# GeekAlexis/FastMOT

Measured on AMD Instinct MI355X. Metric: end-to-end tracker FPS @1080p/50 dets, higher is better.
Workload: dtype f16

## Files before the change

### fastmot_amd/_lib.py

```python
import ctypes as C
import os
import sys
import weakref
from pathlib import Path

import numpy as np
from types import SimpleNamespace

from .utils.nv12 import NV12Frame
from .utils.jpeg import JPEGFrame, QT_ENTRIES, max_coefficients
from .utils.source import SourceFrame
from .utils.yuv import PlanarFrame, frame_bytes
from .utils.packed import PackedFrame, row_bytes
from .utils.bayer import BayerFrame
from .utils.deep import DeepFrame, deep_frame_bytes
from .utils.devarray import DeviceArrayFrame

LIB_PATH = Path(os.environ.get('FASTMOT_LIB_PATH', Path(__file__).parent / 'libfastmot_hip.so'))

c_int_p = C.POINTER(C.c_int)
_lib = None


class FastMOTHipError(RuntimeError):
# ... 117 lines not shown
    plans = np.ascontiguousarray(plans, dtype=CROP_PLAN_DTYPE)
    lens = np.array([len(s) for s in segments], np.uint32)
    segs = np.zeros(max(sum((len(s) + 15) & ~15 for s in segments), 16), np.uint8)
    at = 0
    for s in segments:
        segs[at:at + len(s)] = np.frombuffer(s, np.uint8)
        at += (len(s) + 15) & ~15
    cap = int(plans['bound'].sum()) if capacity is None else capacity
    out = np.zeros(max(cap, 1), np.uint8)
    offsets = np.zeros(len(plans) + 1, np.uintp)
    check(load().fm_jpeg_encode_regions_assemble(_ptr(plans), C.c_int(len(plans)), C.c_int(int(quality)), _ptr(lens), _ptr(segs),
                                                 C.c_size_t(segs.size if segs_bytes is None else segs_bytes), _ptr(out), C.c_size_t(cap),
                                                 _ptr(offsets)))
    return [out[int(a):int(b)].tobytes() for a, b in zip(offsets[:-1], offsets[1:])]


def _redact_args(regions):
    regions = np.ascontiguousarray(regions, dtype=REDACT_REGION_DTYPE).reshape(-1)
    return regions, (_ptr(regions) if len(regions) else None, C.c_int(len(regions)))


def redact_check(regions, width, height):
    regions, args = _redact_args(regions)
    return load().fm_redact_check(*args, C.c_int(width), C.c_int(height))


def redact_render_host(frame, regions):
    if not isinstance(frame, np.ndarray) or frame.dtype != np.uint8 or frame.ndim != 3 or frame.shape[2] != 3 or \
            frame.strides[1:] != (3, 1) or frame.strides[0] < 3 * frame.shape[1] or not frame.flags.writeable:
        raise ValueError('frame must be a writeable uint8 HxWx3 array with packed pixels')
    regions, args = _redact_args(regions)
    check(load().fm_redact_render_host(_ptr(frame), C.c_int(frame.shape[1]), C.c_int(frame.shape[0]), C.c_size_t(frame.strides[0]), *args))
    return frame


def device_count():
    n = load().fm_device_count()
    if n < 0:
        raise FastMOTHipError(load().fm_last_error().decode())
    return n


def device_pci_bus_id(device):
    buf = C.create_string_buffer(64)
    check(load().fm_device_pci_bus_id(C.c_int(device), buf, C.c_int(64)))
    return buf.value.decode().lower()


class HipContext:

    def __init__(self, device=0):
        self._dev_pending = []
        self.lib = load()
        self._ctx = C.c_void_p()
        check(self.lib.fm_ctx_create(C.c_int(device), C.byref(self._ctx)))
        self.device = device
        self.feat_dim = 512

    def close(self):
        if getattr(self, '_ctx', None) is not None and self._ctx:
            self.lib.fm_ctx_destroy(self._ctx)
            self._ctx = C.c_void_p()
        for frame, _ in self._dev_pending:
            frame._pending = [(ref, t) for ref, t in frame._pending if ref() is not self]
        self._dev_pending = []

    def __del__(self):
        if sys.is_finalizing():
            return
        try:
            self.close()
        except Exception:
            pass

    @property
    def handle(self):
        return self._ctx

    def synchronize(self):
        check(self.lib.fm_ctx_synchronize(self._ctx))

    def set_option(self, key, value):
        check(self.lib.fm_ctx_set_option(self._ctx, key.encode(), C.c_int(int(value))))

    def trace_start(self, cap=20000):
        t0 = C.c_int64(0)
        check(self.lib.fm_trace_start(self._ctx, C.c_int(cap), C.byref(t0)))
        self._trace_cap = cap
        return t0.value

    def trace_read(self):
        cap = self._trace_cap
        tags = np.zeros(cap, np.int32)
        ms = np.zeros(cap, np.float32)
        n = C.c_int(0)
        check(self.lib.fm_trace_read(self._ctx, C.c_int(cap), _ptr(tags), _ptr(ms), C.byref(n)))
        return tags[:n.value], ms[:n.value]

    def bind_thread(self):
        check(self.lib.fm_ctx_bind_thread(self._ctx))

    def device_info(self):
        buf = C.create_string_buffer(256)
        check(self.lib.fm_device_info(self._ctx, buf, 256))
        parts = buf.value.decode().split(':')
        return {'name': parts[0], 'arch': ':'.join(parts[1:-3]), 'cus': int(parts[-3]),
                'clock_mhz': int(parts[-2]), 'hbm_bytes': int(parts[-1])}

    def kf_configure(self, dt, std_factor_acc, std_offset_acc, std_factor_det, std_factor_klt,
                     min_std_det, min_std_klt, init_pos_weight, init_vel_weight, vel_coupling,
                     vel_half_life):
        p = KFParams(dt, std_factor_acc, std_offset_acc, (C.c_double * 2)(*std_factor_det),
                     (C.c_double * 2)(*std_factor_klt), (C.c_double * 2)(*min_std_det),
                     (C.c_double * 2)(*min_std_klt), init_pos_weight, init_vel_weight, vel_coupling,
                     vel_half_life)
        check(self.lib.fm_kf_configure(self._ctx, C.byref(p)))

    def set_frame_rect(self, tlbr):
        a = _as(tlbr, np.float64, (4,))
        check(self.lib.fm_set_frame_rect(self._ctx, _ptr(a)))

    def trk_create(self, slots, det_tlbr):
        s = _as(slots, np.int32)
        b = _as(det_tlbr, np.float64, (-1, 4))
        assert len(s) == len(b)
        check(self.lib.fm_trk_create(self._ctx, C.c_int(len(s)), _ptr(s), _ptr(b)))

    def trk_step(self, slots, H, klt_tlbr, has_klt, mult):
        s = _as(slots, np.int32)
        n = len(s)
        Hm = _as(H, np.float64, (9,))
        k = _as(klt_tlbr, np.float64, (-1, 4)) if n else np.zeros((0, 4))
        hk = _as(has_klt, np.uint8)
        mu = _as(mult, np.float64)
        assert len(k) == n and len(hk) == n and len(mu) == n
        tlbr = np.empty((n, 4), np.float64)
        lost = np.empty(n, np.uint8)
        check(self.lib.fm_trk_step(self._ctx, C.c_int(n), _ptr(s), _ptr(Hm), _ptr(k), _ptr(hk),
                                   _ptr(mu), _ptr(tlbr), _ptr(lost)))
        return tlbr, lost.astype(bool)

    def trk_step_ops(self, ops, slots, H, klt_tlbr, has_klt, mult):
        s = _as(slots, np.int32)
        n = len(s)
        Hm = _as(H, np.float64, (9,))
        k = _as(klt_tlbr, np.float64, (-1, 4)) if n else np.zeros((0, 4))
        hk = _as(has_klt, np.uint8)
        mu = _as(mult, np.float64)
        tlbr = np.empty((n, 4), np.float64)
        lost = np.empty(n, np.uint8)
        check(self.lib.fm_trk_step_ops(self._ctx, C.c_int(ops), C.c_int(n), _ptr(s), _ptr(Hm), _ptr(k),
                                       _ptr(hk), _ptr(mu), _ptr(tlbr), _ptr(lost)))
        return tlbr, lost.astype(bool)

    def trk_update_det(self, slots, det_tlbr):
        s = _as(slots, np.int32)
        n = len(s)
        b = _as(det_tlbr, np.float64, (-1, 4)) if n else np.zeros((0, 4))
        assert len(b) == n
        tlbr = np.empty((n, 4), np.float64)
        lost = np.empty(n, np.uint8)
        check(self.lib.fm_trk_update_det(self._ctx, C.c_int(n), _ptr(s), _ptr(b), _ptr(tlbr), _ptr(lost)))
        return tlbr, lost.astype(bool)

    def trk_get_state(self, slots):
        s = _as(slots, np.int32)
# ... 930 lines not shown
```

### fastmot_amd/csrc/common.h

```cpp
#pragma once
#include <hip/hip_runtime.h>
#include <atomic>
#include <cstdarg>
#include <cstdint>
#include <cstdio>
#include <cstring>
#include <string>
#include <vector>
#include "../../include/fastmot_hip.h"
#ifdef FM_DIAG
#include "../../include/fastmot_hip_diag.h"
#endif

#define FM_ERR_HIP (-1)
#define FM_ERR_ARG (-2)
#define FM_ERR_STATE (-3)

void fm_set_error(const char* fmt, ...);

#define FM_HIP(call)                                                                        \
    do {                                                                                    \
        hipError_t e_ = (call);                                                             \
        if (e_ != hipSuccess) {                                                             \
            fm_set_error("%s:%d %s -> %s", __FILE__, __LINE__, #call, hipGetErrorString(e_)); \
            return FM_ERR_HIP;                                                              \
        }                                                                                   \
    } while (0)

#define FM_CHECK_ARG(cond)                                                     \
    do {                                                                       \
        if (!(cond)) {                                                         \
            fm_set_error("%s:%d bad argument: %s", __FILE__, __LINE__, #cond); \
            return FM_ERR_ARG;                                                 \
        }                                                                      \
    } while (0)

bool fm_lap_host(const double* cost, int nr, int nc, long rs, long cs, int32_t* col4row_out);
#define FM_ZERO_COPY_TRACKS (ctx->opt_zero_copy_tracks)

struct DevBuf {
    void* d = nullptr;
    void* h = nullptr;
    size_t cap = 0;
    bool pinned_mirror = true;
    int reserve(size_t bytes) {
        if (bytes <= cap) return 0;
        size_t ncap = cap ? cap : 4096;
        while (ncap < bytes) ncap *= 2;
        if (d) (void)hipFree(d);
        if (h) (void)hipHostFree(h);
        d = h = nullptr;
        cap = 0;
        FM_HIP(hipMalloc(&d, ncap));
        if (pinned_mirror) FM_HIP(hipHostMalloc(&h, ncap, hipHostMallocDefault));
        cap = ncap;
        return 0;
    }
    void release() {
        if (d) (void)hipFree(d);
        if (h) (void)hipHostFree(h);
        d = h = nullptr;
        cap = 0;
    }
    template <typename T> T* dev() { return reinterpret_cast<T*>(d); }
    template <typename T> T* host() { return reinterpret_cast<T*>(h); }
};

struct KFConst {
    double F_pos_self;
    double F_pos_other;
    double F_vel;
    double q_pp, q_pv, q_vv;
    double std_factor_acc, std_offset_acc;
    double fac_det[2], fac_klt[2], min_det[2], min_klt[2];
    double init_pos_weight, init_vel_weight;
};

struct NetState;
struct DetState;
struct ExtState;
struct FlowState;
struct EncState;
struct OvlState;
struct YuvState;
struct SsdState;
struct GalleryState;
constexpr int FM_GALLERY_CHANNELS = 2;

struct fm_ctx {
    int device = 0;
    int opt_zero_copy_tracks = 2048;
    int opt_host_lap_elems = 262144;
    int opt_use_graphs = 1;
    int opt_fused_input = 1;
    int opt_net_timing = 0;
    int opt_nms_general = 0;
    int opt_lk_variant = 0;
    void* predict_worker = nullptr;
    hipStream_t s_main = nullptr;
    hipStream_t s_det = nullptr;
    hipStream_t s_up = nullptr;
    hipStream_t s_ext = nullptr;
    hipStream_t s_ext_x[FM_MAX_EXTRA_EXTRACTORS] = {};
    hipEvent_t ev_ext_in = nullptr, ev_ext_x_done[FM_MAX_EXTRA_EXTRACTORS] = {};
    hipStream_t s_flow = nullptr;
    hipStream_t s_flow2 = nullptr;
    hipEvent_t ev_pyr = nullptr;
    bool pyr_pending = false;
    hipEvent_t ev_prep = nullptr, ev_bg = nullptr;
    hipEvent_t ev_feat = nullptr;
    hipEvent_t ev_ext_net = nullptr;
    hipEvent_t ev_ext_done = nullptr;
    hipEvent_t ev_pair = nullptr;
    bool ext_net_recorded = false;
    size_t as_in_bytes = 0;
    bool as_in_device = true;
    bool as_mirror = false;

    int slot_cap = 0;
    double* mean = nullptr;
    double* cov = nullptr;
    int feat_dim = 512;
    float* feat_sum = nullptr;
    float* feat_avg = nullptr;
    int32_t* feat_cnt = nullptr;
    KFConst kf{};
    bool kf_set = false;
    double frame_rect[4] = {0, 0, 0, 0};

    float* emb = nullptr;
    float* emb_host = nullptr;
    int emb_cap = 0;
    int emb_n = 0;

    int as_nT = 0, as_nD = 0, as_metric = 0;
    size_t as_off[6] = {0, 0, 0, 0, 0, 0};
    DevBuf as_in;
    DevBuf as_pair;
    DevBuf as_stage_in;
    DevBuf as_cost;
    DevBuf as_work;
    DevBuf as_out;
    DevBuf io0, io1;
    DevBuf occ_in, occ_out;
    DevBuf feat_in;

    int frame_w = 0, frame_h = 0, ring_size = 0;
    uint8_t* frame_cur = nullptr;
    uint8_t* frame_own = nullptr;
    uint8_t* frame_own2 = nullptr;
    uint8_t* frame_next = nullptr;
    uint8_t* frame_pinned2 = nullptr;
    hipEvent_t ev_next_upload = nullptr;
    uint8_t* frame_ahead[FM_MAX_DET_BATCH + 1] = {};
    uint8_t* frame_up[FM_MAX_DET_BATCH + 1] = {};
    uint8_t* frame_up_pinned[FM_MAX_DET_BATCH + 1] = {};
    hipEvent_t ev_up[FM_MAX_DET_BATCH + 1] = {};
    uint8_t* frame_ring = nullptr;
    uint8_t* frame_pinned = nullptr;

    DetState* det = nullptr;
    SsdState* ssd = nullptr;
    ExtState* ext = nullptr;
    NetState* det_net = nullptr;
    NetState* ext_net = nullptr;
    NetState* ext_net_x[FM_MAX_EXTRA_EXTRACTORS] = {};
    FlowState* flow = nullptr;
    EncState* enc = nullptr;
    OvlState* ovl = nullptr;
    YuvState* yuv = nullptr;
    GalleryState* gallery[2] = {nullptr, nullptr};

    std::vector<hipEvent_t> trace_ev;
    std::vector<int> trace_tag;
    std::atomic<int> trace_n{0};
    std::atomic<bool> trace_on{false};
    std::atomic<int> trace_busy{0};
    hipEvent_t trace_base = nullptr;

// ... 15 lines not shown
    };
    SrcStage frame_src[FM_MAX_DET_BATCH + 2];
    SrcStage frame_deep[FM_MAX_DET_BATCH + 2];

    hipEvent_t ev_dev_in[FM_MAX_DET_BATCH + 2] = {};
    struct DevTicket {
        uint64_t ticket = 0;
        hipEvent_t ev = nullptr;
    };
    DevTicket dev_ticket[FM_DEV_TICKETS];
    uint64_t dev_ticket_next = 1;

    int32_t* remap_xy = nullptr;
    int remap_sw = 0, remap_sh = 0;
    uint32_t remap_border = 0;
};

inline void fm_trace_mark(fm_ctx* ctx, hipStream_t s, int tag) {
    if (!ctx->trace_on.load(std::memory_order_acquire)) return;
    ctx->trace_busy.fetch_add(1);
    if (ctx->trace_on.load()) {
        const int i = ctx->trace_n.fetch_add(1);
        if (i < (int)ctx->trace_ev.size()) {
            ctx->trace_tag[i] = tag;
            (void)hipEventRecord(ctx->trace_ev[i], s);
        }
    }
    ctx->trace_busy.fetch_sub(1);
}

int fm_ensure_slots(fm_ctx* ctx, int max_slot_plus_1);
int fm_nv12_to_bgr(const uint8_t* nv12, uint8_t* bgr, int w, int h, int matrix, hipStream_t s);
inline bool fm_yuv_chroma_dims(int w, int h, int chroma, int* cw, int* ch) {
    switch (chroma) {
    case FM_YUV_420: *cw = (w + 1) / 2, *ch = (h + 1) / 2; return true;
    case FM_YUV_422: *cw = (w + 1) / 2, *ch = h; return true;
    case FM_YUV_444: *cw = w, *ch = h; return true;
    case FM_YUV_MONO: *cw = *ch = 0; return true;
    }
    return false;
}
int fm_planar_to_bgr(const uint8_t* planes, uint8_t* bgr, int w, int h, int chroma, int matrix, hipStream_t s);
inline size_t fm_packed_row_bytes(int w, int format) {
    if (format < FM_PACKED_RGB || format > FM_PACKED_YVYU) return 0;
    if (format >= FM_PACKED_YUY2) return 4 * (size_t)((w + 1) / 2);
    return (size_t)w * (format <= FM_PACKED_BGR ? 3 : 4);
}
inline bool fm_packed_matrix_ok(int matrix) {
    return matrix == FM_PACKED_BT601 || matrix == FM_PACKED_BT709 || matrix == FM_PACKED_BT601_FULL || matrix == FM_PACKED_BT709_FULL;
}
int fm_packed_to_bgr(const uint8_t* src, uint8_t* bgr, int w, int h, int format, int matrix, hipStream_t s);
inline int fm_bayer_sample_bytes(int depth) {
    return depth == 8 ? 1 : depth == 10 || depth == 12 || depth == 14 || depth == 16 ? 2 : 0;
}
inline bool fm_bayer_gain_ok(int gain) { return gain >= 1 && gain <= 4096; }
int fm_bayer_to_bgr(const uint8_t* src, uint8_t* bgr, int w, int h, int pattern, int depth, int method, int black, int gain_r, int gain_g,
                    int gain_b, hipStream_t s);
inline bool fm_deep_layout_ok(int w, int h, int chroma, int matrix, int depth, int layout) {
    int cw = 0, ch = 0;
    if (depth < 9 || depth > 16 || matrix < FM_DEEP_BT601 || matrix > FM_DEEP_BT2020 || !fm_yuv_chroma_dims(w, h, chroma, &cw, &ch)) return false;
    if (layout == FM_DEEP_SEMIPLANAR) return chroma == FM_YUV_420 && w % 2 == 0 && h % 2 == 0;
    return layout == FM_DEEP_PLANAR;
}
int fm_deep_to_bgr(const uint8_t* planes, uint8_t* bgr, int w, int h, int chroma, int matrix, int depth, int layout,
                   hipStream_t s);
int fm_device_to_bgr(const struct fm_frame_device* f, uint8_t* bgr, hipStream_t s);
inline int fm_dev_elem_bytes(int dtype) { return dtype == FM_DEV_U8 ? 1 : dtype == FM_DEV_F16 ? 2 : dtype == FM_DEV_F32 ? 4 : 0; }
inline int fm_dev_planes(int layout) { return layout == FM_DEV_HWC ? 1 : layout == FM_DEV_CHW ? 3 : layout == FM_DEV_NV12 ? 2 : 0; }
inline int fm_dev_plane_rows(const struct fm_frame_device* f, int p) { return f->layout == FM_DEV_NV12 && p == 1 ? f->height / 2 : f->height; }
inline size_t fm_dev_row_bytes(const struct fm_frame_device* f) {
    if (f->layout == FM_DEV_HWC) return (size_t)f->width * (f->format <= FM_PACKED_BGR ? 3 : 4);
    return (size_t)f->width * fm_dev_elem_bytes(f->dtype);
}
void fm_ssd_free(fm_ctx* ctx);
void fm_yuv_free(fm_ctx* ctx);
int fm_resize_bgr(const uint8_t* src, int sw, int sh, uint8_t* dst, int dw, int dh, hipStream_t s);
int fm_remap_bgr(const uint8_t* src, int sw, int sh, const int32_t* xy, uint8_t* dst, int dw, int dh, uint32_t border, hipStream_t s);
inline uint8_t*& fm_ahead_frame(fm_ctx* ctx, int k) { return k == 1 ? ctx->frame_next : ctx->frame_ahead[k]; }
inline uint8_t*& fm_ahead_buf(fm_ctx* ctx, int k) { return k == 1 ? ctx->frame_own2 : ctx->frame_up[k]; }
inline hipEvent_t& fm_ahead_event(fm_ctx* ctx, int k) { return k == 1 ? ctx->ev_next_upload : ctx->ev_up[k]; }
bool fm_host_is_pinned(const void* p, size_t bytes);
void fm_frame_staging_free(fm_ctx* ctx);
void fm_frame_dev_free(fm_ctx* ctx);
int fm_det_flush_post(fm_ctx* ctx);
int fm_jpeg_to_bgr(const uint8_t* stage, uint8_t* bgr, const struct fm_jpeg_info* info, hipStream_t s);
int fm_jpeg_layout(int width, int height, int ncomp, int hsamp0, int vsamp0, struct fm_jpeg_info* out);
size_t fm_jpeg_sample_offset(long long coef_count);
void fm_ext_invalidate_export(fm_ctx* ctx);
void fm_predict_worker_free(fm_ctx* ctx);
void fm_gallery_free(fm_ctx* ctx);
void fm_jpegenc_free(fm_ctx* ctx);
int fm_jpegenc_ensure(fm_ctx* ctx, int mcus_x, int mcus_y);
hipStream_t fm_jpegenc_stream(fm_ctx* ctx);
int fm_jpegenc_encode_device(fm_ctx* ctx, const uint8_t* src, int width, int height, int quality, uint8_t* out, size_t capacity,
                             size_t* length);
void fm_overlay_free(fm_ctx* ctx);
```

### fastmot_amd/csrc/ctx.hip

```cpp
#include "common.h"
void convd_set_cfg(int code);
#include <sched.h>
#include <cstring>
#include <cstdlib>
#include <cmath>

static thread_local char g_err[1024] = "";

void fm_set_error(const char* fmt, ...) {
    va_list ap;
    va_start(ap, fmt);
    vsnprintf(g_err, sizeof(g_err), fmt, ap);
    va_end(ap);
}

extern "C" const char* fm_last_error(void) { return g_err; }

extern "C" int fm_ctx_set_option(fm_ctx* ctx, const char* key, int value) {
    FM_CHECK_ARG(ctx && key && value >= 0);
    if (!strcmp(key, "zero_copy_tracks")) ctx->opt_zero_copy_tracks = value;
    else if (!strcmp(key, "host_lap_elems")) ctx->opt_host_lap_elems = value;
    else if (!strcmp(key, "use_graphs")) ctx->opt_use_graphs = value;
    else if (!strcmp(key, "convd_cfg")) convd_set_cfg(value);
    else if (!strcmp(key, "nms_path")) {
        ctx->opt_nms_general = value != 0;
    }
    else if (!strcmp(key, "fused_input")) ctx->opt_fused_input = value != 0;
    else if (!strcmp(key, "net_timing")) ctx->opt_net_timing = value;
    else if (!strcmp(key, "lk_variant")) {
#ifndef FM_DIAG
        if (value != 0) {
            fm_set_error("option 'lk_variant' needs a diagnostic build of the library (-DFM_DIAG)");
            return FM_ERR_ARG;
        }
#endif
        ctx->opt_lk_variant = value;
    }
    else {
        fm_set_error("unknown option '%s'", key);
        return FM_ERR_ARG;
    }
    return 0;
}

extern "C" int fm_trace_start(fm_ctx* ctx, int cap, int64_t* host_ns) {
    FM_CHECK_ARG(ctx && cap > 0 && host_ns && !ctx->trace_on.load() && ctx->trace_ev.empty());
    FM_HIP(hipDeviceSynchronize());
    std::vector<hipEvent_t> evs(cap);
    for (auto& e : evs) FM_HIP(hipEventCreate(&e));
    if (!ctx->trace_base) FM_HIP(hipEventCreate(&ctx->trace_base));
    FM_HIP(hipEventRecord(ctx->trace_base, ctx->s_main));
    FM_HIP(hipEventSynchronize(ctx->trace_base));
    timespec ts;
    clock_gettime(CLOCK_MONOTONIC, &ts);
    *host_ns = (int64_t)ts.tv_sec * 1000000000ll + ts.tv_nsec;
    ctx->trace_tag.assign(cap, 0);
    ctx->trace_n = 0;
    ctx->trace_ev = std::move(evs);
    ctx->trace_on.store(true, std::memory_order_release);
    return 0;
}

extern "C" int fm_trace_read(fm_ctx* ctx, int cap, int32_t* tags, float* ms, int* n) {
    FM_CHECK_ARG(ctx && tags && ms && n);
    ctx->trace_on.store(false, std::memory_order_seq_cst);
    while (ctx->trace_busy.load(std::memory_order_seq_cst) > 0) sched_yield();
    FM_HIP(hipDeviceSynchronize());
    std::vector<hipEvent_t> evs = std::move(ctx->trace_ev);
    ctx->trace_ev.clear();
    int k = ctx->trace_n.load();
    if (k > (int)evs.size()) k = (int)evs.size();
    if (k > cap) k = cap;
    for (int i = 0; i < k; ++i) {
        tags[i] = ctx->trace_tag[i];
        FM_HIP(hipEventElapsedTime(&ms[i], ctx->trace_base, evs[i]));
    }
    *n = k;
    for (auto& e : evs) (void)hipEventDestroy(e);
    return 0;
}

extern "C" int fm_ctx_bind_thread(fm_ctx* ctx) {
    FM_CHECK_ARG(ctx);
    FM_HIP(hipSetDevice(ctx->device));
    return 0;
}

extern "C" int fm_device_pci_bus_id(int device, char* buf, int buflen) {
    FM_CHECK_ARG(buf && buflen >= 16);
    FM_HIP(hipDeviceGetPCIBusId(buf, buflen, device));
    return 0;
}

extern "C" int fm_device_count(void) {
    int n = 0;
    FM_HIP(hipGetDeviceCount(&n));
    return n;
}

void fm_net_free(NetState* n);
void fm_det_free(DetState* d);
void fm_ext_free(ExtState* e);
void fm_flow_free(FlowState* f);

extern "C" int fm_ctx_create(int device, fm_ctx** out) {
    FM_CHECK_ARG(out != nullptr);
    int n = 0;
    FM_HIP(hipGetDeviceCount(&n));
    if (device < 0 || device >= n) {
        fm_set_error("device %d out of range (%d visible)", device, n);
        return FM_ERR_ARG;
    }
    FM_HIP(hipSetDevice(device));
    fm_ctx* ctx = new fm_ctx();
    ctx->device = device;
    if (const char* e = getenv("FASTMOT_ZERO_COPY")) ctx->opt_zero_copy_tracks = atoi(e);
    if (const char* e = getenv("FASTMOT_HOST_LAP")) ctx->opt_host_lap_elems = atoi(e);
    if (const char* e = getenv("FASTMOT_GRAPHS")) ctx->opt_use_graphs = atoi(e);
    if (const char* e = getenv("FASTMOT_FUSED_INPUT")) ctx->opt_fused_input = atoi(e) != 0;
    int prio_lo = 0, prio_hi = 0;
    FM_HIP(hipDeviceGetStreamPriorityRange(&prio_lo, &prio_hi));
    const int prio_det = prio_lo, prio_ext = prio_hi;
    FM_HIP(hipStreamCreateWithPriority(&ctx->s_main, hipStreamNonBlocking, prio_hi));
    FM_HIP(hipStreamCreateWithPriority(&ctx->s_det, hipStreamNonBlocking, prio_det));
    FM_HIP(hipStreamCreateWithPriority(&ctx->s_up, hipStreamNonBlocking, prio_lo));
    FM_HIP(hipStreamCreateWithPriority(&ctx->s_ext, hipStreamNonBlocking, prio_ext));
    FM_HIP(hipEventCreateWithFlags(&ctx->ev_ext_in, hipEventDisableTiming));
    for (int i = 0; i < FM_MAX_EXTRA_EXTRACTORS; ++i) {
        FM_HIP(hipStreamCreateWithPriority(&ctx->s_ext_x[i], hipStreamNonBlocking, prio_hi));
        FM_HIP(hipEventCreateWithFlags(&ctx->ev_ext_x_done[i], hipEventDisableTiming));
    }
    FM_HIP(hipStreamCreateWithPriority(&ctx->s_flow, hipStreamNonBlocking, prio_hi));
    FM_HIP(hipStreamCreateWithPriority(&ctx->s_flow2, hipStreamNonBlocking, prio_hi));
    FM_HIP(hipEventCreateWithFlags(&ctx->ev_pyr, hipEventDisableTiming));
    FM_HIP(hipEventCreateWithFlags(&ctx->ev_prep, hipEventDisableTiming));
    FM_HIP(hipEventCreateWithFlags(&ctx->ev_bg, hipEventDisableTiming));
    FM_HIP(hipEventCreateWithFlags(&ctx->ev_feat, hipEventDisableTiming));
    FM_HIP(hipEventCreateWithFlags(&ctx->ev_ext_net, hipEventDisableTiming));
    FM_HIP(hipEventCreateWithFlags(&ctx->ev_pair, hipEventDisableTiming));
    FM_HIP(hipEventCreateWithFlags(&ctx->ev_ext_done, hipEventDisableTiming));
    int rc = fm_ensure_slots(ctx, 1024);
    if (rc) return rc;
    *out = ctx;
    return 0;
}

extern "C" int fm_ctx_destroy(fm_ctx* ctx) {
    if (!ctx) return 0;
    (void)hipSetDevice(ctx->device);
    fm_predict_worker_free(ctx);
    fm_gallery_free(ctx);
    (void)hipDeviceSynchronize();
    if (ctx->det) fm_det_free(ctx->det);
    fm_ssd_free(ctx);
    if (ctx->ext) fm_ext_free(ctx->ext);
    for (void* p : {(void*)ctx->frame_own, (void*)ctx->frame_own2, (void*)ctx->frame_ring})
        if (p) (void)hipFree(p);
    if (ctx->frame_pinned) (void)hipHostFree(ctx->frame_pinned);
    if (ctx->frame_pinned2) (void)hipHostFree(ctx->frame_pinned2);
    for (int k = 2; k <= FM_MAX_DET_BATCH; ++k) {
        if (ctx->frame_up[k]) (void)hipFree(ctx->frame_up[k]);
        if (ctx->frame_up_pinned[k]) (void)hipHostFree(ctx->frame_up_pinned[k]);
        if (ctx->ev_up[k]) (void)hipEventDestroy(ctx->ev_up[k]);
    }
    for (hipEvent_t e : ctx->ev_jpeg)
        if (e) (void)hipEventDestroy(e);
    fm_frame_dev_free(ctx);
    fm_frame_staging_free(ctx);
    fm_overlay_free(ctx);
    fm_yuv_free(ctx);
    fm_jpegenc_free(ctx);
    if (ctx->det_net) fm_net_free(ctx->det_net);
    if (ctx->ext_net) fm_net_free(ctx->ext_net);
    for (NetState* x : ctx->ext_net_x)
        if (x) fm_net_free(x);
    if (ctx->flow) fm_flow_free(ctx->flow);
    for (void* p : {(void*)ctx->mean, (void*)ctx->cov, (void*)ctx->feat_sum, (void*)ctx->feat_avg,
                    (void*)ctx->feat_cnt, (void*)ctx->emb})
        if (p) (void)hipFree(p);
    if (ctx->emb_host) (void)hipHostFree(ctx->emb_host);
    for (DevBuf* b : {&ctx->as_in, &ctx->as_pair, &ctx->as_stage_in, &ctx->as_cost, &ctx->as_work,
                      &ctx->as_out, &ctx->io0, &ctx->io1, &ctx->feat_in, &ctx->occ_in, &ctx->occ_out})
        b->release();
    for (hipStream_t s : {ctx->s_main, ctx->s_det, ctx->s_up, ctx->s_ext, ctx->s_flow, ctx->s_flow2})
        if (s) (void)hipStreamDestroy(s);
    for (hipEvent_t e : {ctx->ev_feat, ctx->ev_ext_in, ctx->ev_pyr, ctx->ev_prep, ctx->ev_bg, ctx->ev_ext_net, ctx->ev_pair, ctx->ev_ext_done})
        if (e) (void)hipEventDestroy(e);
    for (int i = 0; i < FM_MAX_EXTRA_EXTRACTORS; ++i) {
        if (ctx->s_ext_x[i]) (void)hipStreamDestroy(ctx->s_ext_x[i]);
        if (ctx->ev_ext_x_done[i]) (void)hipEventDestroy(ctx->ev_ext_x_done[i]);
    }
    delete ctx;
    return 0;
}

extern "C" int fm_ctx_synchronize(fm_ctx* ctx) {
    FM_CHECK_ARG(ctx);
    FM_HIP(hipStreamSynchronize(ctx->s_main));
    FM_HIP(hipStreamSynchronize(ctx->s_det));
    FM_HIP(hipStreamSynchronize(ctx->s_up));
    FM_HIP(hipStreamSynchronize(ctx->s_ext));
    for (hipStream_t x : ctx->s_ext_x) FM_HIP(hipStreamSynchronize(x));
// ... 343 lines not shown
```

### fastmot_amd/csrc/detect.hip

```cpp
#include "pixel_source.h"
#include <cmath>
#include <string>
#include <vector>

struct DetState {
    fm_yolo_cfg cfg{};
    bool configured = false;
    int cap = 8192;
    static constexpr int NSLOT_UNTILED = FM_MAX_DET_BATCH + 2;
    static constexpr int NSLOT = 3 * FM_MAX_DET_BATCH;
    int nslot = NSLOT_UNTILED;
    int n_tiles = 0;
    int tile_x[FM_MAX_DET_BATCH] = {}, tile_y[FM_MAX_DET_BATCH] = {};
    int region_w = 0, region_h = 0;
    double tile_offset[FM_MAX_DET_BATCH][2] = {};
    double merge_thresh = 0.6;
    std::vector<fm_det48> tile_stage;
    std::vector<fm_det48> tile_dets;
    std::vector<int32_t> tile_ids;
    int tile_count[FM_MAX_DET_BATCH] = {};
    int tile_sum[2] = {};
    float* cand[NSLOT] = {};
    float* sorted[NSLOT] = {};
    int32_t* counters[NSLOT] = {};
    uint64_t* mask[NSLOT] = {};
    fm_det48* dets[NSLOT] = {};
    bool used[NSLOT] = {};
    hipEvent_t ev_dec[NSLOT] = {};
    int post_pending = -1;
    int post_pending_n = 0;
    bool general_post = false;
    static constexpr int GREEDY_RETRY = 1024;
    int general_passes = 0;
    int greedy_kmax = 2048, greedy_shrink = 0;
    bool sorted_valid[NSLOT] = {};
    static constexpr int PREFIX = 2048;
    fm_det48* dets_host[NSLOT] = {};
    int32_t* counters_host[NSLOT] = {};
    hipEvent_t ev_done[NSLOT] = {};
    hipStream_t s_fallback = nullptr;
    hipEvent_t ev0[NSLOT] = {}, ev1[NSLOT] = {};
    bool timed[NSLOT] = {};
    long n_passes = 0;
    int wr = 0, rd = 0, pending = 0, last = -1;
    uint8_t* label_mask = nullptr;
    float* rows_in = nullptr;
    int rows_cap = 0;
};

void fm_det_free(DetState* d) {
    if (!d) return;
    for (int i = 0; i < DetState::NSLOT; ++i) {
        for (void* q : {(void*)d->cand[i], (void*)d->sorted[i], (void*)d->counters[i], (void*)d->mask[i], (void*)d->dets[i]})
            if (q) (void)hipFree(q);
    }
    for (void* p : {(void*)d->label_mask, (void*)d->rows_in})
        if (p) (void)hipFree(p);
    if (d->s_fallback) (void)hipStreamDestroy(d->s_fallback);
    for (int i = 0; i < DetState::NSLOT; ++i) {
        if (d->dets_host[i]) (void)hipHostFree(d->dets_host[i]);
        if (d->counters_host[i]) (void)hipHostFree(d->counters_host[i]);
        for (hipEvent_t e : {d->ev_done[i], d->ev_dec[i], d->ev0[i], d->ev1[i]})
            if (e) (void)hipEventDestroy(e);
    }
    delete d;
}

namespace {

__global__ void preprocess_kernel(const StemSrc src, f16* __restrict__ inp, int in_w, int in_h, int cs) {
    const int x = blockIdx.x * blockDim.x + threadIdx.x;
    const int y = blockIdx.y, n = blockIdx.z;
    int32_t* counters = pick_sample(src.zero4, n);
    if (counters && x < 4 && y == 0) counters[x] = 0;
    if (x >= in_w || y >= in_h) return;
    float rgb[3];
    det_input_pixel(pick_sample(src.frame, n), src.fw, src.fh, x, y, pick_sample(src.roi_x, n), pick_sample(src.roi_y, n),
                    src.roi_w, src.roi_h, rgb);
    f16x8 o;
    o[0] = (f16)rgb[0]; o[1] = (f16)rgb[1]; o[2] = (f16)rgb[2];
#pragma unroll
    for (int e = 3; e < 8; ++e) o[e] = (f16)0.f;
    *reinterpret_cast<f16x8*>(inp + (((size_t)n * in_h + y) * in_w + x) * cs) = o;
}

struct HeadArgs {
    const float* data;
    int cs, gw, gh, na, base_index;
    float anchors[2 * FM_MAX_ANCHORS];
    float scale_xy;
};

__device__ __forceinline__ float sigmoid_fast(float x) { return 1.0f / (1.0f + __expf(-x)); }

struct FilterArgs {
    const uint8_t* label_mask;
    int num_classes;
    float conf_thresh;
    double size[2], offset[2];
    float* cand;
    int32_t* counters;
    int cap;
};

__device__ __forceinline__ void emit_candidate(const FilterArgs& fa, float bx, float by, float bw, float bh,
                                               float box_conf, int cls, float cls_prob, int orig) {
    if (cls < 0 || cls >= 128 || !fa.label_mask[cls]) return;
    const float score = box_conf * cls_prob;
    if (!(score >= fa.conf_thresh)) return;
    const int slot = atomicAdd(fa.counters, 1);
    if (slot >= fa.cap) {
        fa.counters[1] = 1;
        return;
    }
    float* r = fa.cand + (size_t)slot * 8;
    float x = (float)((double)bx * fa.size[0]);
    float y = (float)((double)by * fa.size[1]);
    r[2] = (float)((double)bw * fa.size[0]);
    r[3] = (float)((double)bh * fa.size[1]);
    r[0] = (float)((double)x - fa.offset[0]);
    r[1] = (float)((double)y - fa.offset[1]);
    r[4] = box_conf;
    r[5] = (float)cls;
    r[6] = cls_prob;
    r[7] = __int_as_float(orig);
}

struct HeadSet {
    HeadArgs h[FM_MAX_HEADS];
    int first_block[FM_MAX_HEADS + 1];
    float* cand[FM_MAX_DET_BATCH];
    int32_t* counters[FM_MAX_DET_BATCH];
    double off_x[FM_MAX_DET_BATCH], off_y[FM_MAX_DET_BATCH];
};

__global__ void decode_kernel(HeadSet hs, FilterArgs fa, int in_w, int in_h, int new_coords) {
    int hi = 0;
#pragma unroll
    for (int i = 1; i < FM_MAX_HEADS; ++i) hi += (int)blockIdx.x >= hs.first_block[i] ? 1 : 0;
    const HeadArgs& h = hs.h[hi];
    const int idx = ((int)blockIdx.x - hs.first_block[hi]) * blockDim.x + threadIdx.x;
    const int cells = h.gw * h.gh;
    if (idx >= cells * h.na) return;
    const int img = blockIdx.y;
    fa.cand = pick_sample(hs.cand, img);
    fa.counters = pick_sample(hs.counters, img);
    fa.offset[0] = pick_sample(hs.off_x, img);
// ... 481 lines not shown
                        else if (!(est < (float)thresh - 1e-4f)) need |= 1u << u;
                    }
                }
            }
        }
        while (need) {
            const int u = __builtin_ctz(need);
            need &= need - 1;
            const float4 c = sbox[tid + NG_T * u];
            if (diou_suppresses_call(a[0], a[1], a[2], a[3], c.x, c.y, c.z, c.w, thresh)) alive &= ~(1u << u);
        }
#pragma unroll
        for (int u = 0; u < NG_CPT; ++u) {
            const uint64_t bal = __ballot((alive >> u) & 1u);
            if (lane == 0) alive_w[wave + NG_NW * u] = bal;
        }
        __syncthreads();
        if (wave == 0) {
            uint64_t w = alive_w[lane];
            const int ws = s >> 6;
            if (lane < ws) w = 0;
            else if (lane == ws) w &= (s & 63) == 63 ? 0ull : (~0ull << ((s & 63) + 1));
            const uint64_t nz = __ballot(w != 0);
            int next = -1;
            if (nz) {
                const int fl = __builtin_ctzll(nz);
                const uint64_t ww = (uint64_t)(uint32_t)__builtin_amdgcn_readlane((int)(uint32_t)w, fl) |
                                    ((uint64_t)(uint32_t)__builtin_amdgcn_readlane((int)(uint32_t)(w >> 32), fl) << 32);
                next = fl * 64 + __builtin_ctzll(ww);
            }
            if (lane == 0) misc[0] = next;
        }
        __syncthreads();
    }
    if (tid == 0) misc[1] = 0;
    __syncthreads();
#pragma unroll
    for (int u = 0; u < NG_CPT; ++u) {
        if ((int)NG_T * u >= K) break;
        const int j = tid + NG_T * u;
        bool ok = false;
        double t0 = 0, t1 = 0, t2 = 0, t3 = 0;
        if ((kept >> u) & 1u) {
            const float4 b = box[u];
            const double xmin = b.x, ymin = b.y;
            t0 = rint(xmin); t1 = rint(ymin);
            t2 = rint(xmin + (double)b.z - 1.); t3 = rint(ymin + (double)b.w - 1.);
            const double bw = t2 - t0 + 1, bh = t3 - t1 + 1;
            const double area = (bw <= 0 || bh <= 0) ? 0. : bw * bh;
            const double ar = bw > 0 ? bh / bw : 0.;
            ok = area > 0 && area <= max_area && ar >= min_ar;
        }
        const uint64_t bal = __ballot(ok);
        if (lane == 0) misc[2 + wave] = __builtin_popcountll(bal);
        __syncthreads();
        const int base = misc[1];
        int off = base + __builtin_popcountll(bal & ((1ull << lane) - 1ull));
        for (int wv = 0; wv < wave; ++wv) off += misc[2 + wv];
        if (ok) {
            const float* r = sorted + (size_t)j * 8;
            fm_det48 d;
            d.tlbr[0] = t0; d.tlbr[1] = t1; d.tlbr[2] = t2; d.tlbr[3] = t3;
            d.label = (int64_t)r[5];
            d.conf = (double)(r[4] * r[6]);
            dets[off] = d;
            if (off < prefix) dets_host[off] = d;
        }
        __syncthreads();
        if (tid == 0) {
            int n = base;
            for (int wv = 0; wv < NG_NW; ++wv) n += misc[2 + wv];
            misc[1] = n;
        }
        __syncthreads();
    }
    if (tid == 0) {
        const int n = misc[1];
        counters[2] = n;
        counters[3] = 0;
        counters_host[0] = counters[0]; counters_host[1] = counters[1]; counters_host[2] = n; counters_host[3] = 0;
    }
}

int ensure_det(fm_ctx* ctx) {
    if (ctx->det) return 0;
    ctx->det = new DetState();
    return 0;
}

int alloc_post(DetState* d, int cap, int nslot) {
    cap = (cap + 63) & ~63;
    if (d->cand[0] && cap == d->cap && nslot == d->nslot) return 0;
    for (int i = (cap != d->cap || !d->cand[0]) ? 0 : nslot; i < DetState::NSLOT; ++i) {
        for (void* p : {(void*)d->cand[i], (void*)d->sorted[i], (void*)d->mask[i], (void*)d->dets[i]})
            if (p) (void)hipFree(p);
        if (d->dets_host[i]) (void)hipHostFree(d->dets_host[i]);
        d->dets_host[i] = nullptr;
        d->cand[i] = d->sorted[i] = nullptr; d->mask[i] = nullptr; d->dets[i] = nullptr;
    }
    for (int i = 0; i < DetState::NSLOT; ++i) d->used[i] = false;
    d->cap = cap;
    d->nslot = nslot;
    d->wr = d->rd = d->pending = 0;
    d->last = -1;
    d->post_pending = -1;
    d->post_pending_n = 0;
    for (int i = 0; i < nslot; ++i) {
        if (d->cand[i]) continue;
        FM_HIP(hipMalloc(&d->cand[i], sizeof(float) * 8 * cap));
        FM_HIP(hipMalloc(&d->sorted[i], sizeof(float) * 8 * cap));
        FM_HIP(hipMalloc(&d->mask[i], sizeof(uint64_t) * (size_t)cap * (cap / 64)));
        FM_HIP(hipMalloc(&d->dets[i], sizeof(fm_det48) * cap));
        FM_HIP(hipHostMalloc(&d->dets_host[i], sizeof(fm_det48) * cap, hipHostMallocDefault));
    }
    for (int i = 0; i < nslot; ++i) {
        if (d->counters[i]) continue;
        FM_HIP(hipMalloc(&d->counters[i], sizeof(int32_t) * 4));
        FM_HIP(hipHostMalloc(&d->counters_host[i], sizeof(int32_t) * 4, hipHostMallocDefault));
        FM_HIP(hipEventCreateWithFlags(&d->ev_done[i], hipEventDisableTiming));
        FM_HIP(hipEventCreateWithFlags(&d->ev_dec[i], hipEventDisableTiming));
        FM_HIP(hipEventCreate(&d->ev0[i]));
        FM_HIP(hipEventCreate(&d->ev1[i]));
    }
    if (!d->label_mask) FM_HIP(hipMalloc(&d->label_mask, 128));
    return 0;
}

FilterArgs filter_args(DetState* d, int slot) {
    FilterArgs fa{};
    fa.label_mask = d->label_mask;
    fa.num_classes = d->cfg.num_classes;
    fa.conf_thresh = (float)d->cfg.conf_thresh;
    const bool tiled = d->n_tiles > 1;
    fa.size[0] = d->cfg.size[0]; fa.size[1] = d->cfg.size[1];
    fa.offset[0] = tiled ? d->tile_offset[0][0] : d->cfg.offset[0]; fa.offset[1] = tiled ? d->tile_offset[0][1] : d->cfg.offset[1];
    fa.cand = d->cand[slot];
    fa.counters = d->counters[slot];
    fa.cap = d->cap;
    return fa;
}

static int launch_rank_sort(DetState* d, int slot, hipStream_t sp);
static int enqueue_general_post(fm_ctx* ctx, DetState* d, int slot, hipStream_t sp, bool sorted_already = false) {
    const int cap = d->cap;
    if (!sorted_already) {
        int rc = launch_rank_sort(d, slot, sp);
        if (rc) return rc;
    }
    fm_trace_mark(ctx, sp, 22);
    hipLaunchKernelGGL(nms_mask_kernel, dim3(std::min(NMS_MASK_GRID, (cap / 64) * (cap / 64 + 1) / 2)), dim3(256), 0, sp, d->sorted[slot],
                       d->counters[slot], cap, d->cfg.nms_thresh, d->mask[slot]);
    fm_trace_mark(ctx, sp, 23);
    hipLaunchKernelGGL(nms_scan_kernel, dim3(1), dim3(1024), sizeof(uint64_t) * (cap / 64), sp, d->sorted[slot],
                       d->counters[slot], cap, d->mask[slot], d->cfg.max_area, d->cfg.min_aspect_ratio, d->dets[slot],
                       d->dets_host[slot], cap < DetState::PREFIX ? cap : DetState::PREFIX, d->counters_host[slot]);
    FM_HIP(hipGetLastError());
    return 0;
}

static int launch_rank_sort(DetState* d, int slot, hipStream_t sp) {
    const int cap = d->cap;
    static bool configured = false;
    if (!configured) {
        FM_HIP(hipFuncSetAttribute(reinterpret_cast<const void*>(rank_sort_lds_kernel),
                                   hipFuncAttributeMaxDynamicSharedMemorySize, (int)(sizeof(uint64_t) * (16384 + 8))));
        configured = true;
    }
    if (cap <= 16384)
        hipLaunchKernelGGL(rank_sort_lds_kernel, dim3(cap / 64 + 1), dim3(256), sizeof(uint64_t) * (cap + 8), sp,
                           d->cand[slot], d->sorted[slot], d->counters[slot], cap);
    else
        hipLaunchKernelGGL(rank_sort_kernel, dim3(cap / 256 + 1), dim3(256), 0, sp, d->cand[slot], d->sorted[slot],
                           d->counters[slot], cap);
    FM_HIP(hipGetLastError());
    d->sorted_valid[slot] = true;
    return 0;
}

static int enqueue_greedy_post(fm_ctx* ctx, DetState* d, int slot, hipStream_t sp) {
    static bool configured = false;
    if (!configured) {
        FM_HIP(hipFuncSetAttribute(reinterpret_cast<const void*>(nms_greedy_kernel),
                                   hipFuncAttributeMaxDynamicSharedMemorySize, (int)ng_lds_bytes(NG_KMAX)));
        configured = true;
    }
    int rc = launch_rank_sort(d, slot, sp);
    if (rc) return rc;
    fm_trace_mark(ctx, sp, 22);
    const int kmax = d->greedy_kmax < d->cap ? d->greedy_kmax : (d->cap < NG_KMAX ? d->cap : NG_KMAX);
    hipLaunchKernelGGL(nms_greedy_kernel, dim3(1), dim3(NG_T), ng_lds_bytes(kmax), sp, d->sorted[slot], d->counters[slot],
                       d->cap, kmax, d->cfg.nms_thresh, d->cfg.max_area, d->cfg.min_aspect_ratio, d->dets[slot],
                       d->dets_host[slot], d->cap < DetState::PREFIX ? d->cap : DetState::PREFIX, d->counters_host[slot]);
    FM_HIP(hipGetLastError());
    return 0;
}

static int flush_post(fm_ctx* ctx, DetState* d) {
    const int first = d->post_pending, n = d->post_pending_n;
    if (first < 0) return 0;
    d->post_pending = -1;
    d->post_pending_n = 0;
    hipStream_t sp = ctx->s_up;
    FM_HIP(hipStreamWaitEvent(sp, d->ev_dec[first], 0));
    for (int i = 0; i < n; ++i) {
        const int slot = (first + i) % d->nslot;
        fm_trace_mark(ctx, sp, 20);
        int rc_p = (d->general_post || ctx->opt_nms_general) ? enqueue_general_post(ctx, d, slot, sp) : enqueue_greedy_post(ctx, d, slot, sp);
        if (rc_p) return rc_p;
        FM_HIP(hipEventRecord(d->ev_done[slot], sp));
        fm_trace_mark(ctx, sp, 21);
    }
    return 0;
}

int enqueue_post(fm_ctx* ctx, DetState* d, hipStream_t s, int n = 1) {
    int rc = flush_post(ctx, d);
    if (rc) return rc;
    while (d->pending + n > d->nslot) {
        const int drop = d->n_tiles > 1 ? d->n_tiles : 1;
        d->rd = (d->rd + drop) % d->nslot;
        d->pending -= drop;
    }
    const int slot = d->wr;
    FM_HIP(hipEventRecord(d->ev_dec[slot], s));
    d->post_pending = slot;
    d->post_pending_n = n;
    for (int i = 0; i < n; ++i) d->used[(slot + i) % d->nslot] = true;
    d->wr = (slot + n) % d->nslot;
    d->pending += n;
    return 0;
}

static int acquire_slots(fm_ctx* ctx, DetState* d, hipStream_t s, int n = 1) {
    if (d->post_pending >= 0 && d->post_pending_n + n > d->nslot) {
        int rc = flush_post(ctx, d);
        if (rc) return rc;
    }
    for (int i = 0; i < n; ++i) {
        const int slot = (d->wr + i) % d->nslot;
        if (d->used[slot] && hipEventQuery(d->ev_done[slot]) != hipSuccess) {
            (void)hipGetLastError();
            FM_HIP(hipStreamWaitEvent(s, d->ev_done[slot], 0));
        }
    }
    return 0;
}

int collect(fm_ctx* ctx, DetState* d, hipStream_t s, fm_det48* out, int cap_out, int* n) {
    if (d->pending == 0) {
        fm_set_error("no detector pass in flight (fm_detect_async first)");
        return FM_ERR_STATE;
    }
    const int slot = d->rd;
    int rc_f = flush_post(ctx, d);
    if (rc_f) return rc_f;
    FM_HIP(hipEventSynchronize(d->ev_done[slot]));
    if (d->counters_host[slot][3] != 0 && !d->counters_host[slot][1]) {
        const int why = d->counters_host[slot][3];
        if (!d->s_fallback) FM_HIP(hipStreamCreateWithFlags(&d->s_fallback, hipStreamNonBlocking));
        hipStream_t sp = d->s_fallback;
        int rc_g = enqueue_general_post(ctx, d, slot, sp, d->sorted_valid[slot]);
        if (rc_g) return rc_g;
        FM_HIP(hipStreamSynchronize(sp));
        if (why == 2 || d->counters_host[slot][0] > NG_KMAX) {
            d->general_post = true;
            d->general_passes = 0;
        }
    } else if (d->general_post && d->counters_host[slot][0] <= NG_KMAX * 3 / 4 && ++d->general_passes >= DetState::GREEDY_RETRY) {
        d->general_post = false;
    }
    {
        const int k = d->counters_host[slot][0];
        int want = ((k + k / 4 + 511) / 512) * 512;
        if (want < 512) want = 512;
        if (want > NG_KMAX) want = NG_KMAX;
        if (want > d->greedy_kmax) d->greedy_kmax = want;
        else if (want < d->greedy_kmax && ++d->greedy_shrink >= 64) { d->greedy_kmax = want; d->greedy_shrink = 0; }
        else if (want == d->greedy_kmax) d->greedy_shrink = 0;
    }
    d->rd = (slot + 1) % d->nslot;
    --d->pending;
    d->last = slot;
    if (d->counters_host[slot][1]) {
        fm_set_error("candidate list overflow (%d > %d): raise max_candidates", d->counters_host[slot][0], d->cap);
        return FM_ERR_STATE;
    }
    const int nd = d->counters_host[slot][2];
    if (nd > DetState::PREFIX) {
        FM_HIP(hipMemcpy(d->dets_host[slot], d->dets[slot], sizeof(fm_det48) * nd, hipMemcpyDeviceToHost));
    }
    if (nd > cap_out) {
        fm_set_error("output capacity %d < %d detections", cap_out, nd);
        return FM_ERR_ARG;
    }
    memcpy(out, d->dets_host[slot], sizeof(fm_det48) * nd);
    *n = nd;
    return 0;
}

int collect_tiles(fm_ctx* ctx, DetState* d, hipStream_t s, fm_det48* out, int cap_out, int* n) {
    const int nt = d->n_tiles;
    if (d->pending < nt) {
        fm_set_error("no detector pass in flight (fm_detect_async first)");
        return FM_ERR_STATE;
    }
    const int first = d->rd, pending = d->pending;
    d->tile_stage.resize((size_t)d->cap);
    d->tile_dets.clear();
    d->tile_ids.clear();
    d->tile_sum[0] = d->tile_sum[1] = 0;
    int rc_first = 0;
    std::string err;
    for (int t = 0; t < nt; ++t) {
        const int slot = (first + t) % d->nslot;
        int k = 0;
        d->rd = slot;
        const int rc = collect(ctx, d, s, d->tile_stage.data(), d->cap, &k);
        d->tile_count[t] = rc ? 0 : k;
        if (rc) {
            if (!rc_first) { rc_first = rc; err = fm_last_error(); }
            if (rc == FM_ERR_HIP) break;
            continue;
        }
        d->tile_sum[0] += d->counters_host[slot][0];
        d->tile_sum[1] += k;
        d->tile_dets.insert(d->tile_dets.end(), d->tile_stage.begin(), d->tile_stage.begin() + k);
        d->tile_ids.insert(d->tile_ids.end(), (size_t)k, (int32_t)t);
    }
    d->rd = (first + nt) % d->nslot;
    d->pending = pending - nt;
    d->last = first;
    if (rc_first) {
        d->tile_dets.clear();
        d->tile_ids.clear();
        for (int t = 0; t < nt; ++t) d->tile_count[t] = 0;
        fm_set_error("%s", err.c_str());
        return rc_first;
    }
    const int total = (int)d->tile_dets.size();
    if (total > cap_out) {
        d->tile_stage.resize((size_t)std::max(total, d->cap));
        int nm = 0;
        int rc = fm_detect_merge_tiles(d->tile_dets.data(), d->tile_ids.data(), total, nt, d->merge_thresh, d->tile_stage.data(), &nm);
        if (rc) return rc;
        if (nm > cap_out) {
            fm_set_error("output capacity %d < %d detections", cap_out, nm);
            return FM_ERR_ARG;
        }
        memcpy(out, d->tile_stage.data(), sizeof(fm_det48) * nm);
        *n = nm;
        return 0;
    }
    return fm_detect_merge_tiles(d->tile_dets.data(), d->tile_ids.data(), total, nt, d->merge_thresh, out, n);
}

}

int fm_det_flush_post(fm_ctx* ctx) { return ctx->det ? flush_post(ctx, ctx->det) : 0; }

extern "C" int fm_detect_configure(fm_ctx* ctx, const fm_yolo_cfg* cfg) {
    FM_CHECK_ARG(ctx && cfg);
    FM_CHECK_ARG(cfg->n_heads >= 0 && cfg->n_heads <= FM_MAX_HEADS && cfg->num_classes > 0 && cfg->num_classes <= 128);
    {
        long long rows = 0;
        for (int i = 0; i < cfg->n_heads; ++i) {
            FM_CHECK_ARG(cfg->n_anchors[i] > 0 && cfg->n_anchors[i] <= FM_MAX_ANCHORS && cfg->grid_w[i] > 0 && cfg->grid_h[i] > 0);
            rows += (long long)cfg->grid_w[i] * cfg->grid_h[i] * cfg->n_anchors[i];
        }
        FM_CHECK_ARG(rows < (1ll << FM_SORT_INDEX_BITS));
    }
    int rc = ensure_det(ctx);
    if (rc) return rc;
    DetState* d = ctx->det;
    FM_HIP(hipStreamSynchronize(ctx->s_det));
    FM_HIP(hipStreamSynchronize(ctx->s_up));
    d->post_pending = -1;
    d->post_pending_n = 0;
    d->rd = d->wr;
    d->pending = 0;
    d->cfg = *cfg;
    d->general_post = ctx->opt_nms_general != 0;
    d->n_tiles = 0;
    d->tile_dets.clear();
    d->tile_ids.clear();
    if ((rc = alloc_post(d, cfg->max_candidates > 0 ? cfg->max_candidates : 8192, DetState::NSLOT_UNTILED))) return rc;
    FM_HIP(hipMemcpy(d->label_mask, cfg->label_mask, 128, hipMemcpyHostToDevice));
    d->configured = true;
    return 0;
}

extern "C" int fm_detect_configure_tiles(fm_ctx* ctx, int n_tiles, const int32_t* origins, int region_w, int region_h,
                                         const double* offsets, double merge_thresh) {
    FM_CHECK_ARG(ctx && ctx->det && ctx->det->configured);
    FM_CHECK_ARG(n_tiles == 0 || (n_tiles >= 2 && n_tiles <= FM_MAX_DET_BATCH));
    DetState* d = ctx->det;
    if (n_tiles) {
        FM_CHECK_ARG(origins && offsets && region_w > 0 && region_h > 0 && merge_thresh >= 0. && merge_thresh <= 1.);
        for (int t = 0; t < n_tiles; ++t)
            FM_CHECK_ARG(origins[2 * t] >= 0 && origins[2 * t + 1] >= 0 && origins[2 * t] + d->cfg.in_w <= region_w &&
                         origins[2 * t + 1] + d->cfg.in_h <= region_h);
    }
    FM_HIP(hipStreamSynchronize(ctx->s_det));
    FM_HIP(hipStreamSynchronize(ctx->s_up));
    d->post_pending = -1;
    d->post_pending_n = 0;
    d->rd = d->wr;
    d->pending = 0;
    d->tile_dets.clear();
    d->tile_ids.clear();
    d->n_tiles = n_tiles;
    for (int t = 0; t < n_tiles; ++t) {
        d->tile_x[t] = origins[2 * t]; d->tile_y[t] = origins[2 * t + 1];
        d->tile_offset[t][0] = offsets[2 * t]; d->tile_offset[t][1] = offsets[2 * t + 1];
        d->tile_count[t] = 0;
    }
    if (n_tiles) {
        d->region_w = region_w; d->region_h = region_h;
        d->merge_thresh = merge_thresh;
    }
    d->last = -1;
    d->tile_sum[0] = d->tile_sum[1] = 0;
    for (int t = 0; t < FM_MAX_DET_BATCH; ++t) d->tile_count[t] = 0;
    return alloc_post(d, d->cap, n_tiles ? 3 * n_tiles : DetState::NSLOT_UNTILED);
}

static StemSrc det_source(fm_ctx* ctx, DetState* d, const uint8_t* const* frames, int n) {
    const fm_yolo_cfg& c = d->cfg;
    StemSrc src{};
    src.kind = 1; src.fw = ctx->frame_w; src.fh = ctx->frame_h;
    const bool tiled = d->n_tiles > 1;
    src.roi_w = tiled ? d->region_w : c.roi_w; src.roi_h = tiled ? d->region_h : c.roi_h;
    for (int i = 0; i < FM_MAX_DET_BATCH; ++i) {
        src.roi_x[i] = tiled && i < n ? -d->tile_x[i] : c.roi_x;
        src.roi_y[i] = tiled && i < n ? -d->tile_y[i] : c.roi_y;
    }
    for (int i = 0; i < n; ++i) {
        src.frame[i] = tiled ? frames[0] : frames[i];
        src.zero4[i] = d->counters[(d->wr + i) % d->nslot];
    }
    return src;
}

static int enqueue_preprocess(fm_ctx* ctx, DetState* d, NetState* net, const StemSrc& src, int n) {
    const fm_yolo_cfg& c = d->cfg;
    for (int i = 0; i < n; ++i) FM_CHECK_ARG(src.frame[i] != nullptr);
    FM_CHECK_ARG(c.input_tensor >= 0 && c.input_tensor < (int)net->tensors.size());
    const fm_tensor& t = net->tensors[c.input_tensor];
    FM_CHECK_ARG(t.h == c.in_h && t.w == c.in_w && !t.f32);
    hipLaunchKernelGGL(preprocess_kernel, dim3((c.in_w + 255) / 256, c.in_h, n), dim3(256), 0, ctx->s_det,
                       src, (f16*)net->bufs[c.input_tensor], c.in_w, c.in_h, t.c);
    FM_HIP(hipGetLastError());
    return 0;
}

extern "C" int fm_detect_preprocess_only(fm_ctx* ctx) {
    FM_CHECK_ARG(ctx && ctx->det && ctx->det->configured && ctx->det_net);
    const uint8_t* f = ctx->frame_cur;
    const int n = ctx->det->n_tiles > 1 ? ctx->det->n_tiles : 1;
    FM_CHECK_ARG(n <= ctx->det_net->max_batch);
    return enqueue_preprocess(ctx, ctx->det, ctx->det_net, det_source(ctx, ctx->det, &f, n), n);
}

static int detect_pass(fm_ctx* ctx, const uint8_t* const* frames, const hipEvent_t* uploads, int n);

extern "C" int fm_detect_async(fm_ctx* ctx) {
    FM_CHECK_ARG(ctx);
    const uint8_t* f = ctx->frame_cur;
    const hipEvent_t none = nullptr;
    return detect_pass(ctx, &f, &none, 1);
}

static int detect_ahead(fm_ctx* ctx, int n);

extern "C" int fm_detect_async_next(fm_ctx* ctx) {
    FM_CHECK_ARG(ctx && ctx->frame_next);
    return detect_ahead(ctx, 1);
}

extern "C" int fm_detect_async_ahead(fm_ctx* ctx, int n) {
    FM_CHECK_ARG(ctx);
    if (ctx->det && ctx->det->n_tiles > 1) {
        fm_set_error("fm_detect_async_ahead: the detector is tiled, its passes take the tiles of one frame");
        return FM_ERR_STATE;
    }
    return detect_ahead(ctx, n);
}

static int detect_ahead(fm_ctx* ctx, int n) {
    FM_CHECK_ARG(ctx && ctx->det_net && n >= 1 && n <= FM_MAX_DET_BATCH);
    if (n > ctx->det_net->max_batch) {
        fm_set_error("detector look-ahead of %d frames > the detector network's max_batch %d", n, ctx->det_net->max_batch);
        return FM_ERR_ARG;
    }
    const uint8_t* frames[FM_MAX_DET_BATCH];
    hipEvent_t uploads[FM_MAX_DET_BATCH];
    for (int k = 1; k <= n; ++k) {
        frames[k - 1] = fm_ahead_frame(ctx, k);
        if (!frames[k - 1]) {
            fm_set_error("look-ahead slot %d holds no frame (fm_frame_upload_ahead / fm_frame_ring_select_ahead)", k);
            return FM_ERR_ARG;
        }
        uploads[k - 1] = frames[k - 1] == fm_ahead_buf(ctx, k) ? fm_ahead_event(ctx, k) : nullptr;
    }
    return detect_pass(ctx, frames, uploads, n);
}

static int detect_pass(fm_ctx* ctx, const uint8_t* const* frames, const hipEvent_t* uploads, int n) {
    FM_CHECK_ARG(ctx && ctx->det && ctx->det->configured && ctx->det_net);
    DetState* d = ctx->det;
    NetState* net = ctx->det_net;
    const fm_yolo_cfg& c = d->cfg;
    const bool tiled = d->n_tiles > 1;
    const int n_frames = n;
    if (tiled) {
        FM_CHECK_ARG(n_frames == 1);
        n = d->n_tiles;
        if (n > net->max_batch) {
            fm_set_error("%d tiles > the detector network's max_batch %d", n, net->max_batch);
            return FM_ERR_ARG;
        }
    }
    FM_CHECK_ARG(n >= 1 && n <= FM_MAX_DET_BATCH && n <= net->max_batch);
    hipStream_t s = ctx->s_det;
    fm_trace_mark(ctx, s, 10);
    for (int i = 0; i < n_frames; ++i)
        if (uploads[i]) FM_HIP(hipStreamWaitEvent(s, uploads[i], 0));
    int rc = acquire_slots(ctx, d, s, n);
    if (rc) return rc;
    fm_trace_mark(ctx, s, 14);
    const StemSrc src = det_source(ctx, d, frames, n);
    const bool fused = ctx->opt_fused_input && fm_net_stem_fusable(net, c.input_tensor);
    const bool timing = ctx->opt_net_timing > 0 && d->n_passes++ % ctx->opt_net_timing == 0;
    for (int i = 0; i < n; ++i) d->timed[(d->wr + i) % d->nslot] = timing && i == 0;
    if (fused) {
        if (timing) FM_HIP(hipEventRecord(d->ev0[d->wr], s));
        fm_trace_mark(ctx, s, 11);
        if ((rc = fm_net_run_stem_from(ctx, net, src, n))) return rc;
        fm_trace_mark(ctx, s, 15);
        net->first = 1;
        rc = fm_net_run_internal(ctx, FM_NET_DETECTOR, n);
        net->first = 0;
        if (rc) return rc;
    } else {
        if ((rc = enqueue_preprocess(ctx, d, net, src, n))) return rc;
        if (timing) FM_HIP(hipEventRecord(d->ev0[d->wr], s));
        fm_trace_mark(ctx, s, 11);
        if ((rc = fm_net_run_internal(ctx, FM_NET_DETECTOR, n))) return rc;
    }
    if (timing) FM_HIP(hipEventRecord(d->ev1[d->wr], s));
    fm_trace_mark(ctx, s, 12);
    FilterArgs fa = filter_args(d, d->wr);
    HeadSet hs{};
    for (int i = 0; i < n; ++i) {
        const int slot = (d->wr + i) % d->nslot;
        hs.cand[i] = d->cand[slot];
        hs.counters[i] = d->counters[slot];
    }
    for (int i = 0; i < FM_MAX_DET_BATCH; ++i) {
        hs.off_x[i] = tiled && i < n ? d->tile_offset[i][0] : c.offset[0];
        hs.off_y[i] = tiled && i < n ? d->tile_offset[i][1] : c.offset[1];
    }
    int base = 0, blocks = 0;
    for (int i = 0; i < FM_MAX_HEADS + 1; ++i) hs.first_block[i] = 0x7fffffff;
    for (int i = 0; i < c.n_heads; ++i) {
        FM_CHECK_ARG(c.head_tensor[i] >= 0 && c.head_tensor[i] < (int)net->tensors.size());
        const fm_tensor& t = net->tensors[c.head_tensor[i]];
        FM_CHECK_ARG(t.f32 && t.h == c.grid_h[i] && t.w == c.grid_w[i] && c.n_anchors[i] <= FM_MAX_ANCHORS);
        HeadArgs& h = hs.h[i];
        h.data = (const float*)net->bufs[c.head_tensor[i]];
        h.cs = t.c; h.gw = c.grid_w[i]; h.gh = c.grid_h[i]; h.na = c.n_anchors[i];
        h.base_index = base;
        memcpy(h.anchors, c.anchors[i], sizeof(float) * 2 * FM_MAX_ANCHORS);
        h.scale_xy = c.scale_xy[i];
        const int cnt = h.gw * h.gh * h.na;
        hs.first_block[i] = blocks;
        blocks += (cnt + 255) / 256;
        base += cnt;
    }
    if (blocks) hipLaunchKernelGGL(decode_kernel, dim3(blocks, n), dim3(256), 0, s, hs, fa, c.in_w, c.in_h, c.new_coords);
    FM_HIP(hipGetLastError());
    fm_trace_mark(ctx, s, 13);
    return enqueue_post(ctx, d, s, n);
}

extern "C" int fm_detect_sync(fm_ctx* ctx, fm_det48* out, int cap, int* n) {
    FM_CHECK_ARG(ctx && ctx->det && ctx->det->configured && out && n);
    if (ctx->det->n_tiles > 1) return collect_tiles(ctx, ctx->det, ctx->s_det, out, cap, n);
    return collect(ctx, ctx->det, ctx->s_det, out, cap, n);
}

extern "C" int fm_filter_dets(fm_ctx* ctx, const float* rows, int n, fm_det48* out, int cap, int* n_out) {
    FM_CHECK_ARG(ctx && ctx->det && ctx->det->configured && n >= 0 && out && n_out);
    FM_CHECK_ARG(n < (1 << FM_SORT_INDEX_BITS));
    DetState* d = ctx->det;
    hipStream_t s = ctx->s_det;
    FM_HIP(hipStreamSynchronize(s));
    FM_HIP(hipStreamSynchronize(ctx->s_up));
    d->post_pending = -1;
    d->post_pending_n = 0;
    d->rd = d->wr;
    d->pending = 0;
    if (n > d->rows_cap) {
        if (d->rows_in) FM_HIP(hipFree(d->rows_in));
        d->rows_in = nullptr;
        FM_HIP(hipMalloc(&d->rows_in, sizeof(float) * 7 * (size_t)n));
        d->rows_cap = n;
    }
    if (n) FM_HIP(hipMemcpyAsync(d->rows_in, rows, sizeof(float) * 7 * (size_t)n, hipMemcpyHostToDevice, s));
    FM_HIP(hipMemsetAsync(d->counters[d->wr], 0, sizeof(int32_t) * 4, s));
    if (n) hipLaunchKernelGGL(rows_filter_kernel, dim3((n + 255) / 256), dim3(256), 0, s, d->rows_in, n, filter_args(d, d->wr));
    int rc = enqueue_post(ctx, d, s);
    if (rc) return rc;
    return collect(ctx, d, s, out, cap, n_out);
}

extern "C" int fm_detect_last_counts(fm_ctx* ctx, int* n_candidates, int* n_detections) {
    FM_CHECK_ARG(ctx && ctx->det && n_candidates && n_detections);
    const DetState* d = ctx->det;
    if (d->last < 0) {
        *n_candidates = *n_detections = 0;
        return 0;
    }
    if (d->n_tiles > 1) {
        *n_candidates = d->tile_sum[0];
        *n_detections = d->tile_sum[1];
        return 0;
    }
    *n_candidates = d->counters_host[d->last][0];
    *n_detections = d->counters_host[d->last][2];
    return 0;
}

extern "C" int fm_detect_last_tiles(fm_ctx* ctx, fm_det48* out, int cap, int32_t* counts, int* n_tiles) {
    FM_CHECK_ARG(ctx && ctx->det && out && counts && n_tiles);
    const DetState* d = ctx->det;
    FM_CHECK_ARG(d->n_tiles > 1 && (int)d->tile_dets.size() <= cap);
    if (!d->tile_dets.empty()) memcpy(out, d->tile_dets.data(), sizeof(fm_det48) * d->tile_dets.size());
    for (int t = 0; t < d->n_tiles; ++t) counts[t] = d->tile_count[t];
    *n_tiles = d->n_tiles;
    return 0;
}

extern "C" int fm_detect_raw_candidates(fm_ctx* ctx, float* rows, int cap, int* n) {
    FM_CHECK_ARG(ctx && ctx->det && rows && n);
    DetState* d = ctx->det;
    int rc_f = flush_post(ctx, d);
    if (rc_f) return rc_f;
    FM_HIP(hipStreamSynchronize(ctx->s_det));
    FM_HIP(hipStreamSynchronize(ctx->s_up));
    const int slot = (d->wr + d->nslot - 1) % d->nslot;
    int32_t cnt[4];
    FM_HIP(hipMemcpy(cnt, d->counters[slot], sizeof(cnt), hipMemcpyDeviceToHost));
    const int k = cnt[0] < d->cap ? cnt[0] : d->cap;
    FM_CHECK_ARG(k <= cap);
    FM_HIP(hipMemcpy(rows, d->sorted[slot], sizeof(float) * 8 * k, hipMemcpyDeviceToHost));
    *n = k;
    return 0;
}

extern "C" int fm_detect_net_ms(fm_ctx* ctx, float* ms) {
    FM_CHECK_ARG(ctx && ctx->det && ms && ctx->det->last >= 0);
    const int slot = ctx->det->last;
    if (!ctx->det->timed[slot]) { *ms = -1.f; return 0; }
    FM_HIP(hipEventSynchronize(ctx->det->ev1[slot]));
    FM_HIP(hipEventElapsedTime(ms, ctx->det->ev0[slot], ctx->det->ev1[slot]));
    return 0;
}
```

### fastmot_amd/csrc/frames.hip

```cpp
#include "pixel_source.h"
#include "remap_pixel.h"
#include <mutex>
#include <utility>
#include <vector>

namespace {
std::mutex g_host_mu;
std::vector<std::pair<const uint8_t*, size_t>> g_host_ranges;

bool is_pinned_range(const uint8_t* p, size_t bytes) {
    std::lock_guard<std::mutex> lk(g_host_mu);
    for (auto& r : g_host_ranges)
        if (p >= r.first && p + bytes <= r.first + r.second) return true;
    return false;
}
}

bool fm_host_is_pinned(const void* p, size_t bytes) { return is_pinned_range((const uint8_t*)p, bytes); }

extern "C" int fm_host_alloc(size_t bytes, void** out) {
    FM_CHECK_ARG(out && bytes > 0);
    void* p = nullptr;
    FM_HIP(hipHostMalloc(&p, bytes, hipHostMallocDefault));
    {
        std::lock_guard<std::mutex> lk(g_host_mu);
        g_host_ranges.emplace_back((const uint8_t*)p, bytes);
    }
    *out = p;
    return 0;
}

extern "C" int fm_host_free(void* p) {
    if (!p) return 0;
    {
        std::lock_guard<std::mutex> lk(g_host_mu);
        for (size_t i = 0; i < g_host_ranges.size(); ++i)
            if (g_host_ranges[i].first == (const uint8_t*)p) {
                g_host_ranges.erase(g_host_ranges.begin() + i);
                break;
            }
    }
    FM_HIP(hipHostFree(p));
    return 0;
}

static void src_stages_free(fm_ctx::SrcStage* stages, int n) {
    for (int i = 0; i < n; ++i) {
        fm_ctx::SrcStage& e = stages[i];
        if (e.bgr) (void)hipFree(e.bgr);
        if (e.dev) (void)hipFree(e.dev);
        if (e.pinned) (void)hipHostFree(e.pinned);
        if (e.ev) (void)hipEventDestroy(e.ev);
        e = fm_ctx::SrcStage{};
    }
}

static void remap_free(fm_ctx* ctx) {
    if (ctx->remap_xy) (void)hipFree(ctx->remap_xy);
    ctx->remap_xy = nullptr;
    ctx->remap_sw = ctx->remap_sh = 0;
    ctx->remap_border = 0;
}

static int remap_idle(fm_ctx* ctx) {
    FM_HIP(hipStreamSynchronize(ctx->s_det));
    FM_HIP(hipStreamSynchronize(ctx->s_ext));
    FM_HIP(hipStreamSynchronize(nullptr));
    return 0;
}

extern "C" int fm_frame_remap_set(fm_ctx* ctx, int src_w, int src_h, const int32_t* xy, const uint8_t border_bgr[3]) {
    FM_CHECK_ARG(ctx && ctx->frame_own && xy && border_bgr);
    FM_CHECK_ARG(src_w >= 1 && src_h >= 1 && src_w <= FM_SRC_MAX_DIM && src_h <= FM_SRC_MAX_DIM);
    const size_t n = (size_t)ctx->frame_w * ctx->frame_h;
    for (size_t i = 0; i < n; ++i) FM_CHECK_ARG(fm_remap_entry_ok(xy[2 * i], xy[2 * i + 1], src_w, src_h));
    int rc = remap_idle(ctx);
    if (rc) return rc;
    int32_t* dev = nullptr;
    FM_HIP(hipMalloc(&dev, n * 2 * sizeof(int32_t)));
    if (hipError_t e = hipMemcpy(dev, xy, n * 2 * sizeof(int32_t), hipMemcpyHostToDevice); e != hipSuccess) {
        (void)hipFree(dev);
        FM_HIP(e);
    }
    remap_free(ctx);
    ctx->remap_xy = dev;
    ctx->remap_sw = src_w, ctx->remap_sh = src_h;
    ctx->remap_border = (uint32_t)border_bgr[0] | (uint32_t)border_bgr[1] << 8 | (uint32_t)border_bgr[2] << 16;
    return 0;
}

extern "C" int fm_frame_remap_clear(fm_ctx* ctx) {
    FM_CHECK_ARG(ctx);
    if (!ctx->remap_xy) return 0;
    int rc = remap_idle(ctx);
    if (rc) return rc;
    remap_free(ctx);
    return 0;
}

static bool remap_takes(const fm_ctx* ctx, int w, int h) { return !ctx->remap_xy || (w == ctx->remap_sw && h == ctx->remap_sh); }

static bool src_on_size(const fm_ctx* ctx, int w, int h) { return !ctx->remap_xy && w == ctx->frame_w && h == ctx->frame_h; }
static bool src_on_size(const fm_ctx* ctx, const struct fm_frame_src* f) { return src_on_size(ctx, f->width, f->height); }

void fm_frame_staging_free(fm_ctx* ctx) {
    for (uint8_t** stage : {ctx->frame_nv12, ctx->frame_planar, ctx->frame_packed, ctx->frame_bayer, ctx->frame_jpeg})
        for (int i = 0; i < FM_MAX_DET_BATCH + 2; ++i) {
            if (stage[i]) (void)hipFree(stage[i]);
            stage[i] = nullptr;
        }
    for (uint8_t*& p : ctx->frame_jpeg_pinned) {
        if (p) (void)hipHostFree(p);
        p = nullptr;
    }
    src_stages_free(ctx->frame_src, FM_MAX_DET_BATCH + 2);
    src_stages_free(ctx->frame_deep, FM_MAX_DET_BATCH + 2);
    remap_free(ctx);
}

extern "C" int fm_frame_configure(fm_ctx* ctx, int width, int height, int ring_size) {
    FM_CHECK_ARG(ctx && width > 0 && height > 0 && ring_size >= 0);
    FM_HIP(hipDeviceSynchronize());
    for (void* p : {(void*)ctx->frame_own, (void*)ctx->frame_own2, (void*)ctx->frame_ring})
        if (p) (void)hipFree(p);
    for (void* p : {(void*)ctx->frame_pinned, (void*)ctx->frame_pinned2})
        if (p) (void)hipHostFree(p);
    ctx->frame_own = ctx->frame_own2 = ctx->frame_ring = ctx->frame_pinned = ctx->frame_pinned2 = nullptr;
    ctx->frame_next = nullptr;
    for (int k = 2; k <= FM_MAX_DET_BATCH; ++k) {
        if (ctx->frame_up[k]) (void)hipFree(ctx->frame_up[k]);
        if (ctx->frame_up_pinned[k]) (void)hipHostFree(ctx->frame_up_pinned[k]);
        ctx->frame_up[k] = ctx->frame_up_pinned[k] = ctx->frame_ahead[k] = nullptr;
    }
    fm_frame_staging_free(ctx);
    const size_t bytes = (size_t)width * height * 3;
    FM_HIP(hipMalloc(&ctx->frame_own, bytes + FM_FRAME_SLACK));
    FM_HIP(hipMalloc(&ctx->frame_own2, bytes + FM_FRAME_SLACK));
    FM_HIP(hipHostMalloc(&ctx->frame_pinned, bytes, hipHostMallocDefault));
    FM_HIP(hipHostMalloc(&ctx->frame_pinned2, bytes, hipHostMallocDefault));
    if (ring_size > 0) FM_HIP(hipMalloc(&ctx->frame_ring, bytes * ring_size + FM_FRAME_SLACK));
    ctx->frame_w = width;
    ctx->frame_h = height;
    ctx->ring_size = ring_size;
    ctx->frame_cur = ctx->frame_own;
    return 0;
}

static int src_reserve(uint8_t*& p, size_t& cap, size_t bytes, bool host, hipStream_t s) {
    if (bytes <= cap) return 0;
// ... 25 lines not shown
    uint8_t* pinned;
    hipEvent_t reuse;
    fm_ctx::SrcStage* own;
    int acquire(size_t bytes, hipStream_t s, uint8_t** out) const {
        if (own) {
            int rc = src_pinned(*own, bytes, s);
            *out = own->pinned;
            return rc;
        }
        if (reuse) FM_HIP(hipEventSynchronize(reuse));
        *out = pinned;
        return 0;
    }
    int copied(hipStream_t s) const { return own ? src_pinned_copied(*own, s) : 0; }
};

struct Plane {
    const uint8_t* ptr;
    size_t pitch, row_bytes;
    int rows;
};

enum class Direct {
    SURFACE,
    PLANES_OR_SURFACE,
    PLANES,
};

static int copy_planes(uint8_t* dev, const Plane* planes, int n, Direct direct, const Staging& staging, hipStream_t s, bool blocking) {
    size_t off[4] = {}, total = 0;
    bool packed = true, contiguous = true;
    for (int p = 0; p < n; ++p) {
        off[p] = total;
        packed = packed && planes[p].pitch == planes[p].row_bytes;
        contiguous = contiguous && planes[p].ptr == planes[0].ptr + total;
        total += planes[p].row_bytes * planes[p].rows;
    }
    off[n] = total;
    if (blocking) {
        for (int p = 0; p < n; ++p)
            FM_HIP(hipMemcpy2D(dev + off[p], planes[p].row_bytes, planes[p].ptr, planes[p].pitch, planes[p].row_bytes, planes[p].rows,
                               hipMemcpyHostToDevice));
        return 0;
    }
    bool surface = false, each = false;
    if (direct == Direct::SURFACE) {
        surface = packed && contiguous && is_pinned_range(planes[0].ptr, total);
    } else if (packed) {
        each = true;
        for (int p = 0; p < n; ++p) each = each && is_pinned_range(planes[p].ptr, off[p + 1] - off[p]);
        surface = each && contiguous && direct == Direct::PLANES_OR_SURFACE;
    }
    if (surface) {
        FM_HIP(hipMemcpyAsync(dev, planes[0].ptr, total, hipMemcpyHostToDevice, s));
    } else if (each) {
        for (int p = 0; p < n; ++p) FM_HIP(hipMemcpyAsync(dev + off[p], planes[p].ptr, off[p + 1] - off[p], hipMemcpyHostToDevice, s));
    } else {
        uint8_t* pin = nullptr;
        int rc = staging.acquire(total, s, &pin);
        if (rc) return rc;
        for (int p = 0; p < n; ++p)
            for (int r = 0; r < planes[p].rows; ++r)
                memcpy(pin + off[p] + (size_t)r * planes[p].row_bytes, planes[p].ptr + (size_t)r * planes[p].pitch, planes[p].row_bytes);
        FM_HIP(hipMemcpyAsync(dev, pin, total, hipMemcpyHostToDevice, s));
        if ((rc = staging.copied(s))) return rc;
    }
    return 0;
}

struct Target {
    int entry;
    uint8_t* dst;
    hipStream_t s;
    uint8_t* pinned;
    hipEvent_t reuse;
    bool blocking;
};

template <class Enqueue> static int into_current(fm_ctx* ctx, Enqueue enqueue) {
    FM_HIP(hipStreamSynchronize(ctx->s_det));
    FM_HIP(hipStreamSynchronize(ctx->s_ext));
    FM_HIP(hipStreamSynchronize(ctx->s_flow));
    FM_HIP(hipStreamSynchronize(ctx->s_flow2));
    int rc = enqueue(Target{0, ctx->frame_own, ctx->s_det, ctx->frame_pinned, nullptr, false});
    if (rc) return rc;
    FM_HIP(hipStreamSynchronize(ctx->s_det));
    ctx->frame_cur = ctx->frame_own;
    return 0;
}

static uint8_t*& ahead_pinned(fm_ctx* ctx, int k) { return k == 1 ? ctx->frame_pinned2 : ctx->frame_up_pinned[k]; }

template <class Enqueue> static int into_ahead(fm_ctx* ctx, int k, Enqueue enqueue) {
    const size_t bytes = (size_t)ctx->frame_w * ctx->frame_h * 3;
    if (!fm_ahead_buf(ctx, k)) {
        FM_HIP(hipMalloc(&fm_ahead_buf(ctx, k), bytes + FM_FRAME_SLACK));
        FM_HIP(hipHostMalloc(&ahead_pinned(ctx, k), bytes, hipHostMallocDefault));
    }
    uint8_t* const buf = fm_ahead_buf(ctx, k);
    hipEvent_t& ev = fm_ahead_event(ctx, k);
    hipStream_t cs = ctx->s_ext;
    fm_trace_mark(ctx, cs, 30);
    int rc = enqueue(Target{k, buf, cs, ahead_pinned(ctx, k), ev, false});
    if (rc) return rc;
    fm_trace_mark(ctx, cs, 31);
    if (!ev) FM_HIP(hipEventCreateWithFlags(&ev, hipEventDisableTiming));
    FM_HIP(hipEventRecord(ev, cs));
    if ((rc = fm_det_flush_post(ctx))) return rc;
    fm_ahead_frame(ctx, k) = buf;
    return 0;
}

template <class Enqueue> static int into_ring(fm_ctx* ctx, int index, Enqueue enqueue) {
    uint8_t* const dst = ctx->frame_ring + (size_t)ctx->frame_w * ctx->frame_h * 3 * index;
    int rc = enqueue(Target{FM_MAX_DET_BATCH + 1, dst, nullptr, nullptr, nullptr, true});
    if (rc) return rc;
    FM_HIP(hipStreamSynchronize(nullptr));
    return 0;
}

static int enqueue_bgr(fm_ctx* ctx, const Target& t, const uint8_t* bgr) {
    const size_t bytes = (size_t)ctx->frame_w * ctx->frame_h * 3;
    const uint8_t* src = bgr;
    if (!is_pinned_range(bgr, bytes)) {
        if (t.reuse) FM_HIP(hipEventSynchronize(t.reuse));
        memcpy(t.pinned, bgr, bytes);
        src = t.pinned;
    }
    FM_HIP(hipMemcpyAsync(t.dst, src, bytes, hipMemcpyHostToDevice, t.s));
    return 0;
}

extern "C" int fm_frame_upload(fm_ctx* ctx, const uint8_t* bgr) {
    FM_CHECK_ARG(ctx && bgr && ctx->frame_own);
    return into_current(ctx, [&](const Target& t) { return enqueue_bgr(ctx, t, bgr); });
}

extern "C" int fm_frame_upload_next(fm_ctx* ctx, const uint8_t* bgr) { return fm_frame_upload_ahead(ctx, 1, bgr); }

extern "C" int fm_frame_upload_ahead(fm_ctx* ctx, int k, const uint8_t* bgr) {
    FM_CHECK_ARG(ctx && bgr && ctx->frame_own2 && k >= 1 && k <= FM_MAX_DET_BATCH);
    return into_ahead(ctx, k, [&](const Target& t) { return enqueue_bgr(ctx, t, bgr); });
}

extern "C" int fm_frame_ring_select_next(fm_ctx* ctx, int index) { return fm_frame_ring_select_ahead(ctx, 1, index); }

extern "C" int fm_frame_ring_select_ahead(fm_ctx* ctx, int k, int index) {
    FM_CHECK_ARG(ctx && index >= 0 && index < ctx->ring_size && k >= 1 && k <= FM_MAX_DET_BATCH);
    fm_ahead_frame(ctx, k) = ctx->frame_ring + (size_t)ctx->frame_w * ctx->frame_h * 3 * index;
    return 0;
}

extern "C" int fm_frame_promote_next(fm_ctx* ctx) {
    FM_CHECK_ARG(ctx && ctx->frame_next);
    if (ctx->frame_next == ctx->frame_own2) {
        FM_HIP(hipStreamSynchronize(ctx->s_ext));
        FM_HIP(hipStreamSynchronize(ctx->s_flow));
        FM_HIP(hipStreamSynchronize(ctx->s_flow2));
        if (hipEventQuery(ctx->ev_next_upload) != hipSuccess) {
            (void)hipGetLastError();
            FM_HIP(hipStreamWaitEvent(ctx->s_ext, ctx->ev_next_upload, 0));
            FM_HIP(hipStreamWaitEvent(ctx->s_flow, ctx->ev_next_upload, 0));
            FM_HIP(hipStreamWaitEvent(ctx->s_flow2, ctx->ev_next_upload, 0));
            FM_HIP(hipStreamWaitEvent(ctx->s_main, ctx->ev_next_upload, 0));
        }
        std::swap(ctx->frame_own, ctx->frame_own2);
        std::swap(ctx->frame_pinned, ctx->frame_pinned2);
        ctx->frame_cur = ctx->frame_own;
    } else {
        ctx->frame_cur = ctx->frame_next;
    }
    ctx->frame_next = nullptr;
    for (int k = 2; k <= FM_MAX_DET_BATCH; ++k) {
        uint8_t* f = ctx->frame_ahead[k];
        if (f && f == ctx->frame_up[k]) {
            std::swap(fm_ahead_buf(ctx, k - 1), fm_ahead_buf(ctx, k));
            std::swap(ahead_pinned(ctx, k - 1), ahead_pinned(ctx, k));
            std::swap(fm_ahead_event(ctx, k - 1), fm_ahead_event(ctx, k));
        }
        fm_ahead_frame(ctx, k - 1) = f;
        ctx->frame_ahead[k] = nullptr;
    }
    return 0;
}

extern "C" int fm_frame_ring_store(fm_ctx* ctx, int index, const uint8_t* bgr) {
    FM_CHECK_ARG(ctx && bgr && index >= 0 && index < ctx->ring_size);
    const size_t bytes = (size_t)ctx->frame_w * ctx->frame_h * 3;
    FM_HIP(hipMemcpy(ctx->frame_ring + bytes * index, bgr, bytes, hipMemcpyHostToDevice));
    return 0;
}
// ... 557 lines not shown
```

### fastmot_amd/csrc/net.h

```cpp
#pragma once
#include "common.h"
#include <hip/hip_fp16.h>

typedef _Float16 f16;
typedef f16 f16x8 __attribute__((ext_vector_type(8)));
typedef f16 f16x4 __attribute__((ext_vector_type(4)));
typedef float f32x16 __attribute__((ext_vector_type(16)));
typedef float f32x4 __attribute__((ext_vector_type(4)));

enum { ACT_LINEAR = 0, ACT_LEAKY = 1, ACT_MISH = 2, ACT_RELU = 3, ACT_LOGISTIC = 4, ACT_SWISH = 5, ACT_RELU6 = 6 };
enum { RES_NONE = 0, RES_AFTER_ACT = 1, RES_BEFORE_ACT = 2 };

struct ConvParams {
    const f16* in;  int in_cs, in_coff;
    const f16* w;
    const float* bias;
    f16* out;       int out_cs, out_coff;
    float* out32;
    const f16* res; int res_cs, res_coff;
    int N, H, W, Cin, Ho, Wo, Cout, KH, KW, stride, pad;
    int K, Kpad, P;
    int cout_store;
    int act, res_mode;
    int grid_p, grid_c, grid_z, weight_major;
    int pad_dx;
    int up;
    int batch_inv;
};

int launch_conv(const ConvParams& p, float* ws, size_t ws_floats, hipStream_t s);

struct NetState {
    int which = 0, max_batch = 0;
    std::vector<fm_tensor> tensors;
    std::vector<void*> bufs;
    std::vector<fm_layer> layers;
    char* weights = nullptr;
    size_t weight_bytes = 0;
    float* gates = nullptr;
    int n_gates = 0, gate_c = 0;
    hipStream_t stream = nullptr;
    char* arena = nullptr;
    float* ws = nullptr;
    size_t ws_floats = 0;
    std::vector<std::pair<long, hipGraphExec_t>> graphs;
    bool use_graphs = true;
    int emb_offset = 0;
    int batch_offset = 0;
    int first = 0;
};

NetState* fm_net_get(fm_ctx* ctx, int which);
int fm_net_run_internal(fm_ctx* ctx, int which, int batch);

__device__ __forceinline__ void unpack8(const uint4& v, float* f) {
    const f16x8 h = *reinterpret_cast<const f16x8*>(&v);
#pragma unroll
    for (int e = 0; e < 8; ++e) f[e] = (float)h[e];
}
__device__ __forceinline__ uint4 pack8(const float* f) {
    f16x8 h;
#pragma unroll
    for (int e = 0; e < 8; ++e) h[e] = (f16)f[e];
    return *reinterpret_cast<const uint4*>(&h);
}

__device__ __forceinline__ int idiv_small(int i, int d, float inv) {
    (void)d;
    return (int)(((float)i + 0.5f) * inv);
}

template <int HI>
__device__ __forceinline__ float fma_mix_h(uint32_t packed, float k, float acc) {
    float d;
    if constexpr (HI) asm("v_fma_mix_f32 %0, %1, %2, %3 op_sel:[1,0,0] op_sel_hi:[1,0,0]" : "=v"(d) : "v"(packed), "v"(k), "v"(acc));
    else asm("v_fma_mix_f32 %0, %1, %2, %3 op_sel:[0,0,0] op_sel_hi:[1,0,0]" : "=v"(d) : "v"(packed), "v"(k), "v"(acc));
    return d;
}
template <int HI>
__device__ __forceinline__ float fma_mix_hh(uint32_t packed, uint32_t kpacked, float acc) {
    float d;
    if constexpr (HI) asm("v_fma_mix_f32 %0, %1, %2, %3 op_sel:[1,1,0] op_sel_hi:[1,1,0]" : "=v"(d) : "v"(packed), "v"(kpacked), "v"(acc));
    else asm("v_fma_mix_f32 %0, %1, %2, %3 op_sel:[0,0,0] op_sel_hi:[1,1,0]" : "=v"(d) : "v"(packed), "v"(kpacked), "v"(acc));
    return d;
}
template <int N>
__device__ __forceinline__ void fma_mix_nh(const uint32_t* raw, const uint32_t* k, float* acc) {
#pragma unroll
    for (int e = 0; e < N; e += 2) {
        acc[e] = fma_mix_hh<0>(raw[e >> 1], k[e >> 1], acc[e]);
        acc[e + 1] = fma_mix_hh<1>(raw[e >> 1], k[e >> 1], acc[e + 1]);
    }
}
template <int N>
__device__ __forceinline__ void fma_mix_n(const uint32_t* raw, const float* k, float* acc) {
#pragma unroll
    for (int e = 0; e < N; e += 2) {
        acc[e] = fma_mix_h<0>(raw[e >> 1], k[e], acc[e]);
        acc[e + 1] = fma_mix_h<1>(raw[e >> 1], k[e + 1], acc[e + 1]);
    }
}

__device__ __forceinline__ void store_out(const ConvParams& p, long pix, int co, f16x4 o) {
    if (p.up == 2) {
        const int hw = p.Ho * p.Wo, rem = (int)(pix % hw);
        const size_t o00 = ((size_t)(pix / hw) * 2 * p.Ho + 2 * (rem / p.Wo)) * (2 * p.Wo) + 2 * (rem % p.Wo);
        f16* dst = p.out + o00 * p.out_cs + p.out_coff + co;
        *reinterpret_cast<f16x4*>(dst) = o;
        *reinterpret_cast<f16x4*>(dst + p.out_cs) = o;
        *reinterpret_cast<f16x4*>(dst + (size_t)2 * p.Wo * p.out_cs) = o;
        *reinterpret_cast<f16x4*>(dst + (size_t)(2 * p.Wo + 1) * p.out_cs) = o;
    } else {
        *reinterpret_cast<f16x4*>(p.out + (size_t)pix * p.out_cs + p.out_coff + co) = o;
    }
}

__device__ __forceinline__ float act_rcp(float x) { return __builtin_amdgcn_rcpf(x); }
__device__ __forceinline__ float act_leaky(float x) { return x > 0.f ? x : 0.1f * x; }
__device__ __forceinline__ float act_relu(float x) { return x > 0.f ? x : 0.f; }
__device__ __forceinline__ float act_relu6(float x) { return fminf(fmaxf(x, 0.f), 6.f); }
__device__ __forceinline__ float act_mish(float x) {
    const float n = __expf(x);
    const float t = n * (n + 2.f);
    return x > 20.f ? x : x * (t * act_rcp(t + 2.f));
}
__device__ __forceinline__ float act_logistic(float x) { return act_rcp(1.f + __expf(-x)); }
__device__ __forceinline__ float act_swish(float x) { return x * act_rcp(1.f + __expf(-x)); }

__device__ __forceinline__ float apply_act(float x, int act) {
    switch (act) {
        case ACT_LEAKY: return act_leaky(x);
        case ACT_MISH: return act_mish(x);
        case ACT_RELU: return act_relu(x);
// ... 38 lines not shown
```

### fastmot_amd/csrc/net.hip

```cpp
#include "pixel_source.h"
#include <algorithm>
#include <memory>

int launch_dwconv3(const f16* in, int in_cs, int in_coff, f16* out, int out_cs, int out_coff, const f16* w,
                   const float* bias, int N, int H, int W, int C, int act, hipStream_t s);
int launch_dwconv(const f16* in, int in_cs, int in_coff, f16* out, int out_cs, int out_coff, const f16* w,
                  const float* bias, int N, int H, int W, int Ho, int Wo, int C, int stride, int act, hipStream_t s);
bool sepconv_supported(int cin, int cout, int stride);
int launch_sepconv(const f16* in, int in_cs, int in_coff, f16* out, int out_cs, int out_coff, const f16* wdw,
                   const float* bdw, const f16* wpw, const float* bpw, int N, int H, int W, int Ho, int Wo, int cin,
                   int cout, int stride, int act1, int act2, long p_choice, hipStream_t s);
int launch_liteconv(int G, const f16* const* in, const int* in_cs, const int* in_coff, f16* out, int out_cs,
                    int out_coff, const f16* wpw, int kpad, const f16* wdw, const float* bias, int N, int H,
                    int W, int C, int act, float* gap_out, hipStream_t s);
void liteconv_tiling(int C, int W, int H, int* th, int* tw, int* tiles_x, int* tiles_y);
int launch_litechain(const f16* in, int in_cs, int in_coff, f16* out, int out_cs, int out_coff, const f16* wpw,
                     int kpad, const f16* wdw, const float* bias, int N, int H, int W, int C, int act,
                     float* const* gap, hipStream_t s);
int launch_gated_sum(int nstreams, const f16* const* in, const int* in_cs, const int* in_coff, int N, int HW,
                     int C, int hid, const f16* w1, const float* b1, const f16* w2, const float* b2, f16* out,
                     int out_cs, int out_coff, const float* const* part, int tiles, hipStream_t s);
constexpr int GATE_SLOT_TILES = 32;
int launch_pair11(const f16* xa, int xa_cs, int xa_coff, const f16* xc, int xc_cs, int xc_coff, f16* out, int out_cs,
                  int out_coff, const f16* w1, const float* b1, const f16* w2, const float* b2, long P, int cout, int act1,
                  int act2, hipStream_t s, long p_choice);
bool pair11_supported(int cin, int mid, int extra, int cout);
int launch_ostail(const f16* in, int in_cs, int in_coff, const f16* ph, const float* pf, int N, float* out, float* raw_out,
                  float* mirror, hipStream_t s);
bool ostail_supported(int in_h, int in_w, int cin, int mid, int cout, int feat, int n_halfs, int n_floats);
int launch_stemconv(const f16* in, int in_cs, int in_coff, f16* out, int out_cs, int out_coff, const f16* w,
                    const float* bias, int N, int H, int W, int Ho, int Wo, int k, int stride, int pad, int cout,
                    int act, hipStream_t s);
int launch_spp(const f16* in, int in_cs, int in_coff, f16* out, int out_cs, int out_coff, int N, int H, int W,
               int C, hipStream_t s);
int launch_pool(const f16* in, int in_cs, int in_coff, f16* out, int out_cs, int out_coff, int N, int H,
                int W, int C, int Ho, int Wo, int k, int stride, int pad, int avg, hipStream_t s);
int launch_upsample2(const f16* in, int in_cs, int in_coff, f16* out, int out_cs, int out_coff, int N, int H,
                     int W, int C, hipStream_t s);
int launch_conv_streamed(const ConvParams& p, hipStream_t s);
int launch_convd(const ConvParams& p, hipStream_t s);
bool resblock_supported(int C, int M);
int launch_resblock(const f16* x, int x_cs, int x_coff, f16* out, int out_cs, int out_coff, const f16* w1,
                    const float* b1, const f16* w2, const float* b2, int N, int H, int W, int C, int M, int act1,
                    int act2, hipStream_t s);
int launch_add(const f16* a, int a_cs, int a_coff, const f16* b, int b_cs, int b_coff, f16* out, int out_cs,
               int out_coff, long npix, int C, hipStream_t s);
int launch_copy(const f16* in, int in_cs, int in_coff, f16* out, int out_cs, int out_coff, long npix, int C,
                hipStream_t s);
int launch_gate(const f16* in, int in_cs, int in_coff, int N, int HW, int C, int hid, const f16* w1,
                const float* b1, const f16* w2, const float* b2, float* gate, hipStream_t s);
int launch_gate_sum(int nstreams, const f16* const* in, const int* in_cs, const int* in_coff,
                    const float* const* gate, f16* out, int out_cs, int out_coff, int N, int HW, int C,
                    hipStream_t s);
int launch_head(const f16* in, int in_cs, int in_coff, int N, int HW, int C, int D, const f16* w,
                const float* b, float* out, float* raw_out, hipStream_t s, float* mirror = nullptr);
int launch_poolhead(const f16* in, int in_cs, int in_coff, int N, int HW, int C, int D, const float* scale, const float* shift,
                    const f16* w, const float* b, int relu, float* out, float* mirror, hipStream_t s);
int fm_emb_reserve(fm_ctx* ctx, int n);


void fm_net_free(NetState* n) {
    if (!n) return;
    for (size_t i = 0; i < n->bufs.size(); ++i)
        if (n->bufs[i] && n->tensors[i].offset < 0) (void)hipFree(n->bufs[i]);
    if (n->arena) (void)hipFree(n->arena);
    if (n->weights) (void)hipFree(n->weights);
    if (n->gates) (void)hipFree(n->gates);
    if (n->ws) (void)hipFree(n->ws);
    for (auto& g : n->graphs) (void)hipGraphExecDestroy(g.second);
    delete n;
}

static NetState*& net_slot(fm_ctx* ctx, int which) {
    return which == FM_NET_DETECTOR ? ctx->det_net : which == FM_NET_EXTRACTOR ? ctx->ext_net
                                                    : ctx->ext_net_x[which - FM_NET_EXTRACTOR_B];
}
NetState* fm_net_get(fm_ctx* ctx, int which) { return net_slot(ctx, which); }
int fm_net_run_internal(fm_ctx* ctx, int which, int batch) { return fm_net_run(ctx, which, batch); }

void fm_net_drop_graphs(NetState* net) {
    if (!net) return;
    (void)hipStreamSynchronize(net->stream);
    for (auto& g : net->graphs) (void)hipGraphExecDestroy(g.second);
    net->graphs.clear();
}

static size_t elem_size(const fm_tensor& t) { return t.f32 ? 4 : 2; }

extern "C" int fm_net_destroy(fm_ctx* ctx, int which) {
    FM_CHECK_ARG(ctx && (which >= 0 && which < FM_NET_EXTRACTOR_B + FM_MAX_EXTRA_EXTRACTORS));
    NetState*& slot = net_slot(ctx, which);
    if (slot) {
        FM_HIP(hipStreamSynchronize(slot->stream));
        fm_net_free(slot);
        slot = nullptr;
    }
    return 0;
}

extern "C" int fm_net_create(fm_ctx* ctx, int which, int max_batch, int n_tensors, const fm_tensor* tensors,
                             int n_layers, const fm_layer* layers, const void* weights, size_t weight_bytes,
                             int n_gates, int gate_channels, size_t arena_bytes) {
    FM_CHECK_ARG(ctx && (which >= 0 && which < FM_NET_EXTRACTOR_B + FM_MAX_EXTRA_EXTRACTORS) && max_batch > 0 && n_tensors > 0 && n_layers > 0);
    FM_CHECK_ARG(tensors && layers && weights && weight_bytes > 0);
    int rc = fm_net_destroy(ctx, which);
    if (rc) return rc;
    std::unique_ptr<NetState, void (*)(NetState*)> net(new NetState(), fm_net_free);
    net->which = which;
    net->max_batch = max_batch;
    net->stream = which == FM_NET_DETECTOR ? ctx->s_det : which == FM_NET_EXTRACTOR ? ctx->s_ext
                                                        : ctx->s_ext_x[which - FM_NET_EXTRACTOR_B];
    net->tensors.assign(tensors, tensors + n_tensors);
    net->layers.assign(layers, layers + n_layers);
    if (arena_bytes) {
        FM_HIP(hipMalloc(&net->arena, arena_bytes));
        FM_HIP(hipMemset(net->arena, 0, arena_bytes));
    }
    for (const fm_tensor& t : net->tensors) {
        FM_CHECK_ARG(t.h > 0 && t.w > 0 && t.c > 0 && t.c % 8 == 0);
        void* b = nullptr;
        const size_t bytes = (size_t)max_batch * t.h * t.w * t.c * elem_size(t);
        if (t.offset >= 0) {
            FM_CHECK_ARG(t.offset % 256 == 0 && (size_t)t.offset + bytes <= arena_bytes);
            b = net->arena + t.offset;
        } else {
            FM_HIP(hipMalloc(&b, bytes));
            FM_HIP(hipMemset(b, 0, bytes));
        }
        net->bufs.push_back(b);
    }
    for (const fm_layer& L : net->layers) {
        FM_CHECK_ARG(L.out >= 0 && L.out < n_tensors && L.n_in >= 1 && L.n_in <= 4);
        for (int i = 0; i < L.n_in; ++i) FM_CHECK_ARG(L.in[i] >= 0 && L.in[i] < n_tensors);
        FM_CHECK_ARG(L.res_mode == FM_RES_NONE || (L.res >= 0 && L.res < n_tensors));
        FM_CHECK_ARG(L.w_off >= 0 && (size_t)L.w_off <= weight_bytes && L.w_off % 16 == 0 && L.b_off % 16 == 0);
        if (L.op == FM_OP_OSTAIL)
            FM_CHECK_ARG(L.stride > 0 && L.pad > 0 && L.b_off >= 0 && (size_t)L.w_off + (size_t)L.stride * 2 <= weight_bytes &&
                         (size_t)L.b_off + (size_t)L.pad * 4 <= weight_bytes);
    }
    FM_HIP(hipMalloc(&net->weights, weight_bytes));
    FM_HIP(hipMemcpy(net->weights, weights, weight_bytes, hipMemcpyHostToDevice));
    net->weight_bytes = weight_bytes;
    net->n_gates = n_gates;
    net->gate_c = gate_channels;
    net->ws_floats = ((size_t)16 << 20) * (which == FM_NET_DETECTOR ? (size_t)std::min(max_batch, FM_MAX_DET_BATCH) : 1);
    FM_HIP(hipMalloc(&net->ws, net->ws_floats * sizeof(float)));
    if (n_gates > 0) {
        FM_CHECK_ARG(gate_channels > 0);
        FM_HIP(hipMalloc(&net->gates, sizeof(float) * (size_t)n_gates * max_batch * gate_channels * GATE_SLOT_TILES));
    }
    if (which != FM_NET_DETECTOR) {
        FM_HIP(hipStreamSynchronize(ctx->s_main));
        if ((rc = fm_emb_reserve(ctx, max_batch))) return rc;
    }
    net_slot(ctx, which) = net.release();
    return 0;
}

static int run_layer(fm_ctx* ctx, NetState* net, const fm_layer& L, int B) {
    const fm_tensor& ti = net->tensors[L.in[0]];
    const fm_tensor& to = net->tensors[L.out];
    hipStream_t s = net->stream;
    float* ws = net->ws;
    const f16* in0 = (const f16*)net->bufs[L.in[0]];
    f16* out = (f16*)net->bufs[L.out];
    switch (L.op) {
        case FM_OP_CONV:
        case FM_OP_CONVS:
        case FM_OP_CONVD: {
            ConvParams p{};
            p.in = in0; p.in_cs = ti.c; p.in_coff = L.in_coff[0];
            p.w = (const f16*)(net->weights + L.w_off);
            p.bias = (const float*)(net->weights + L.b_off);
            p.out = to.f32 ? nullptr : out;
            p.out32 = to.f32 ? (float*)net->bufs[L.out] : nullptr;
            p.out_cs = to.c; p.out_coff = L.out_coff;
            if (L.res_mode != FM_RES_NONE) {
                p.res = (const f16*)net->bufs[L.res];
                p.res_cs = net->tensors[L.res].c;
                p.res_coff = L.res_coff;
            }
            p.up = L.up == 2 ? 2 : 1;
            FM_CHECK_ARG(L.up <= 2 && (p.up == 1 || (!to.f32 && to.h % 2 == 0 && to.w % 2 == 0)));
            p.N = B; p.H = ti.h; p.W = ti.w; p.Cin = L.cin; p.Ho = to.h / p.up; p.Wo = to.w / p.up; p.Cout = L.cout;
            p.KH = p.KW = L.k; p.stride = L.stride; p.pad = L.pad;
            p.K = L.k * L.k * L.cin; p.Kpad = (p.K + 63) & ~63; p.P = B * p.Ho * p.Wo;
            p.cout_store = (L.cout + 7) & ~7;
            p.act = L.act; p.res_mode = L.res_mode;
            p.batch_inv = net->which == FM_NET_DETECTOR ? 1 : 0;
            {
                const int pad_x = L.gate[0] >= 0 && L.op != FM_OP_CONVD ? L.gate[0] : L.pad;
                const bool same2 = L.k == 3 && L.stride == 2 && L.op != FM_OP_CONVD;
                FM_CHECK_ARG(pad_x <= L.k / 2 && (pad_x == L.pad || same2));
                FM_CHECK_ARG((ti.h + 2 * L.pad - L.k) / L.stride + 1 == p.Ho || (same2 && L.pad == 0 && ti.h % 2 == 0 && p.Ho == ti.h / 2));
                FM_CHECK_ARG((ti.w + 2 * pad_x - L.k) / L.stride + 1 == p.Wo || (same2 && pad_x == 0 && ti.w % 2 == 0 && p.Wo == ti.w / 2));
                p.pad_dx = pad_x - L.pad;
            }
            FM_CHECK_ARG(L.out_coff + p.cout_store <= to.c && L.in_coff[0] + L.cin <= ti.c);
            if (L.op == FM_OP_CONVS) return launch_conv_streamed(p, s);
            if (L.op == FM_OP_CONVD) return launch_convd(p, s);
            return launch_conv(p, ws, net->ws_floats, s);
        }
        case FM_OP_DWCONV3:
            return launch_dwconv3(in0, ti.c, L.in_coff[0], out, to.c, L.out_coff,
                                  (const f16*)(net->weights + L.w_off), (const float*)(net->weights + L.b_off),
                                  B, ti.h, ti.w, L.cin, L.act, s);
        case FM_OP_DWCONV:
            FM_CHECK_ARG(!to.f32 && L.k == 3 && L.in_coff[0] + L.cin <= ti.c && L.out_coff + L.cin <= to.c);
            return launch_dwconv(in0, ti.c, L.in_coff[0], out, to.c, L.out_coff, (const f16*)(net->weights + L.w_off),
                                 (const float*)(net->weights + L.b_off), B, ti.h, ti.w, to.h, to.w, L.cin, L.stride, L.act, s);
        case FM_OP_SEPCONV:
            FM_CHECK_ARG(!to.f32 && L.k == 3 && sepconv_supported(L.cin, L.cout, L.stride) && L.in_coff[0] + L.cin <= ti.c &&
                         L.out_coff + L.cout <= to.c && L.gate[0] >= 0);
            FM_CHECK_ARG(L.w2_off >= 0 && L.w2_off % 16 == 0 && L.b2_off >= 0 && L.b2_off % 16 == 0 &&
                         (size_t)L.w_off + (size_t)9 * L.cin * 2 <= net->weight_bytes && (size_t)L.b_off + (size_t)L.cin * 4 <= net->weight_bytes &&
                         (size_t)L.w2_off + (size_t)((L.cout + 31) / 32) * ((L.cin + 15) / 16) * 1024 <= net->weight_bytes &&
                         (size_t)L.b2_off + (size_t)((L.cout + 31) / 32) * 128 <= net->weight_bytes);
            return launch_sepconv(in0, ti.c, L.in_coff[0], out, to.c, L.out_coff, (const f16*)(net->weights + L.w_off),
                                  (const float*)(net->weights + L.b_off), (const f16*)(net->weights + L.w2_off),
                                  (const float*)(net->weights + L.b2_off), B, ti.h, ti.w, to.h, to.w, L.cin, L.cout, L.stride,
                                  L.gate[0], L.act, net->which == FM_NET_DETECTOR ? (long)to.h * to.w : (long)B * to.h * to.w, s);
        case FM_OP_LITECONV: {
            FM_CHECK_ARG(L.cin == ((L.cout + 7) & ~7) && L.n_in >= 1 && L.n_in <= 4);
            FM_CHECK_ARG(L.out_coff + L.n_in * L.cin <= to.c);
            const f16* ins[4];
            int cs[4], co[4];
            for (int i = 0; i < L.n_in; ++i) {
                const fm_tensor& tg = net->tensors[L.in[i]];
                FM_CHECK_ARG(tg.h == to.h && tg.w == to.w && L.in_coff[i] + L.cin <= tg.c);
                ins[i] = (const f16*)net->bufs[L.in[i]];
                cs[i] = tg.c;
                co[i] = L.in_coff[i];
            }
            float* gap_out = nullptr;
            if (L.gate[0] >= 0) {
                int th, tw, tx, ty;
                liteconv_tiling(L.cin, ti.w, ti.h, &th, &tw, &tx, &ty);
                FM_CHECK_ARG(L.gate[0] < net->n_gates && L.cin <= net->gate_c && tx * ty <= GATE_SLOT_TILES);
                gap_out = net->gates + (size_t)L.gate[0] * net->max_batch * net->gate_c * GATE_SLOT_TILES;
            }
            return launch_liteconv(L.n_in, ins, cs, co, out, to.c, L.out_coff,
                                   (const f16*)(net->weights + L.w_off), (L.cin + 63) & ~63,
                                   (const f16*)(net->weights + L.w2_off), (const float*)(net->weights + L.b_off),
                                   B, ti.h, ti.w, L.cin, L.act, gap_out, s);
        }
        case FM_OP_LITECHAIN: {
            FM_CHECK_ARG(L.cin == ((L.cout + 7) & ~7) && to.h == ti.h && to.w == ti.w && L.in_coff[0] + L.cin <= ti.c &&
                         L.out_coff + 4 * L.cin <= to.c);
            int th, tw, tx, ty;
            liteconv_tiling(L.cin, ti.w, ti.h, &th, &tw, &tx, &ty);
            FM_CHECK_ARG(L.cin <= net->gate_c && tx * ty <= GATE_SLOT_TILES);
            float* gaps[4];
            for (int i = 0; i < 4; ++i) {
                FM_CHECK_ARG(L.gate[i] >= 0 && L.gate[i] < net->n_gates);
                gaps[i] = net->gates + (size_t)L.gate[i] * net->max_batch * net->gate_c * GATE_SLOT_TILES;
            }
            return launch_litechain(in0, ti.c, L.in_coff[0], out, to.c, L.out_coff,
                                    (const f16*)(net->weights + L.w_off), (L.cin + 63) & ~63,
                                    (const f16*)(net->weights + L.w2_off), (const float*)(net->weights + L.b_off),
                                    B, ti.h, ti.w, L.cin, L.act, gaps, s);
        }
        case FM_OP_GATED_SUM: {
            const f16* ins[4];
            int cs[4], co[4];
            FM_CHECK_ARG(L.n_in >= 1 && L.n_in <= 4);
            for (int i = 0; i < L.n_in; ++i) {
                ins[i] = (const f16*)net->bufs[L.in[i]];
                cs[i] = net->tensors[L.in[i]].c;
                co[i] = L.in_coff[i];
            }
            const float* parts[4] = {nullptr, nullptr, nullptr, nullptr};
            int tiles = 0;
            if (L.gate[0] >= 0) {
                int th, tw, tx, ty;
                liteconv_tiling(L.cin, ti.w, ti.h, &th, &tw, &tx, &ty);
                tiles = tx * ty;
                for (int i = 0; i < L.n_in; ++i) {
                    FM_CHECK_ARG(L.gate[i] >= 0 && L.gate[i] < net->n_gates);
                    parts[i] = net->gates + (size_t)L.gate[i] * net->max_batch * net->gate_c * GATE_SLOT_TILES;
                }
            }
            return launch_gated_sum(L.n_in, ins, cs, co, B, ti.h * ti.w, L.cin, L.hid,
                                    (const f16*)(net->weights + L.w_off), (const float*)(net->weights + L.b_off),
                                    (const f16*)(net->weights + L.w2_off), (const float*)(net->weights + L.b2_off),
// ... 29 lines not shown
        case FM_OP_MAXPOOL:
        case FM_OP_AVGPOOL:
            return launch_pool(in0, ti.c, L.in_coff[0], out, to.c, L.out_coff, B, ti.h, ti.w, L.cin, to.h, to.w,
                               L.k, L.stride, L.pad, L.op == FM_OP_AVGPOOL, s);
        case FM_OP_UPSAMPLE2:
            FM_CHECK_ARG(to.h == 2 * ti.h && to.w == 2 * ti.w);
            return launch_upsample2(in0, ti.c, L.in_coff[0], out, to.c, L.out_coff, B, ti.h, ti.w, L.cin, s);
        case FM_OP_RESBLOCK:
            FM_CHECK_ARG(!to.f32 && to.h == ti.h && to.w == ti.w && L.cin == L.cout &&
                         L.in_coff[0] + L.cin <= ti.c && L.out_coff + L.cout <= to.c);
            return launch_resblock(in0, ti.c, L.in_coff[0], out, to.c, L.out_coff,
                                   (const f16*)(net->weights + L.w_off), (const float*)(net->weights + L.b_off),
                                   (const f16*)(net->weights + L.w2_off), (const float*)(net->weights + L.b2_off),
                                   B, ti.h, ti.w, L.cin, L.hid, L.act, L.act, s);
        case FM_OP_ADD: {
            FM_CHECK_ARG(L.n_in == 2);
            const fm_tensor& tb = net->tensors[L.in[1]];
            FM_CHECK_ARG(tb.h == ti.h && tb.w == ti.w && to.h == ti.h && to.w == ti.w);
            return launch_add(in0, ti.c, L.in_coff[0], (const f16*)net->bufs[L.in[1]], tb.c, L.in_coff[1], out, to.c,
                              L.out_coff, (long)B * ti.h * ti.w, L.cin, s);
        }
        case FM_OP_COPY:
            return launch_copy(in0, ti.c, L.in_coff[0], out, to.c, L.out_coff, (long)B * ti.h * ti.w, L.cin, s);
        case FM_OP_GATE:
            FM_CHECK_ARG(L.gate[0] >= 0 && L.gate[0] < net->n_gates && L.cin <= net->gate_c);
            return launch_gate(in0, ti.c, L.in_coff[0], B, ti.h * ti.w, L.cin, L.hid,
                               (const f16*)(net->weights + L.w_off), (const float*)(net->weights + L.b_off),
                               (const f16*)(net->weights + L.w2_off), (const float*)(net->weights + L.b2_off),
                               net->gates + (size_t)L.gate[0] * net->max_batch * net->gate_c * GATE_SLOT_TILES, s);
        case FM_OP_GATE_SUM: {
            const f16* ins[4];
            int cs[4], co[4];
            const float* gs[4];
            for (int i = 0; i < L.n_in; ++i) {
                ins[i] = (const f16*)net->bufs[L.in[i]];
                cs[i] = net->tensors[L.in[i]].c;
                co[i] = L.in_coff[i];
                FM_CHECK_ARG(L.gate[i] >= 0 && L.gate[i] < net->n_gates);
                gs[i] = net->gates + (size_t)L.gate[i] * net->max_batch * net->gate_c * GATE_SLOT_TILES;
            }
            return launch_gate_sum(L.n_in, ins, cs, co, gs, out, to.c, L.out_coff, B, ti.h * ti.w, L.cin, s);
        }
        case FM_OP_HEAD:
            FM_CHECK_ARG(L.cout == ctx->feat_dim && net->emb_offset + B <= ctx->emb_cap);
            return launch_head(in0, ti.c, L.in_coff[0], B, ti.h * ti.w, L.cin, L.cout,
                               (const f16*)(net->weights + L.w_off), (const float*)(net->weights + L.b_off),
                               ctx->emb + (size_t)net->emb_offset * ctx->feat_dim, nullptr, s,
                               ctx->emb_host ? ctx->emb_host + (size_t)net->emb_offset * ctx->feat_dim : nullptr);
        case FM_OP_OSTAIL:
            FM_CHECK_ARG(L.cout == ctx->feat_dim && net->emb_offset + B <= ctx->emb_cap && L.in_coff[0] + L.cin <= ti.c &&
                         ostail_supported(ti.h, ti.w, L.cin, L.hid, L.k, L.cout, L.stride, L.pad));
            return launch_ostail(in0, ti.c, L.in_coff[0], (const f16*)(net->weights + L.w_off),
                                 (const float*)(net->weights + L.b_off), B, ctx->emb + (size_t)net->emb_offset * ctx->feat_dim,
                                 nullptr, ctx->emb_host ? ctx->emb_host + (size_t)net->emb_offset * ctx->feat_dim : nullptr, s);
        case FM_OP_POOLHEAD: {
            const bool neck = L.gate[0] > 0, fc = L.gate[1] > 0;
            const size_t wb = net->weight_bytes;
            FM_CHECK_ARG(L.cout == ctx->feat_dim && net->emb_offset + B <= ctx->emb_cap && !ti.f32 && L.cin > 0 && L.cout > 0 &&
                         L.in_coff[0] + L.cin <= ti.c && (fc || L.cout == L.cin));
            FM_CHECK_ARG(!fc || (L.b_off >= 0 && (size_t)L.w_off + (size_t)L.cout * L.cin * 2 <= wb && (size_t)L.b_off + (size_t)L.cout * 4 <= wb));
            FM_CHECK_ARG(!neck || (L.w2_off >= 0 && L.b2_off >= 0 && L.w2_off % 16 == 0 && L.b2_off % 16 == 0 &&
                                   (size_t)L.w2_off + (size_t)L.cin * 4 <= wb && (size_t)L.b2_off + (size_t)L.cin * 4 <= wb));
            return launch_poolhead(in0, ti.c, L.in_coff[0], B, ti.h * ti.w, L.cin, L.cout,
                                   neck ? (const float*)(net->weights + L.w2_off) : nullptr,
                                   neck ? (const float*)(net->weights + L.b2_off) : nullptr,
                                   fc ? (const f16*)(net->weights + L.w_off) : nullptr,
                                   fc ? (const float*)(net->weights + L.b_off) : nullptr, L.act == FM_ACT_RELU,
                                   ctx->emb + (size_t)net->emb_offset * ctx->feat_dim,
                                   ctx->emb_host ? ctx->emb_host + (size_t)net->emb_offset * ctx->feat_dim : nullptr, s);
        }
        default:
            fm_set_error("unknown layer op %d", L.op);
            return FM_ERR_ARG;
    }
}

bool fm_net_writes_mirror(const NetState* net) {
    if (!net || net->layers.empty()) return false;
    const int op = net->layers.back().op;
    return op == FM_OP_HEAD || op == FM_OP_OSTAIL || op == FM_OP_POOLHEAD;
}

static int run_layers_eager(fm_ctx* ctx, NetState* net, int batch) {
    for (size_t i = (size_t)net->first; i < net->layers.size(); ++i) {
        int rc = run_layer(ctx, net, net->layers[i], batch);
        if (rc) return rc;
    }
    return 0;
}

bool fm_net_stem_fusable(const NetState* net, int input_tensor) {
    if (!net || net->layers.empty()) return false;
    const fm_layer& L = net->layers[0];
    if ((L.op != FM_OP_STEMCONV && L.op != FM_OP_STEM2 && L.op != FM_OP_STEMPOOL) || L.n_in != 1 || L.in[0] != input_tensor || L.in_coff[0] != 0) return false;
    for (size_t i = 1; i < net->layers.size(); ++i) {
        const fm_layer& M = net->layers[i];
        for (int k = 0; k < M.n_in; ++k)
            if (M.in[k] == input_tensor) return false;
        if (M.res_mode != FM_RES_NONE && M.res == input_tensor) return false;
        if (M.out == input_tensor) return false;
    }
    return true;
}

int launch_stem2_layer(const fm_layer& L, const StemSrc& src, const NetState* net, int batch, hipStream_t s) {
    const fm_tensor& ti = net->tensors[L.in[0]];
    const fm_tensor& to = net->tensors[L.out];
    const bool three = L.gate[1] > 0;
    const int cout2 = three ? L.gate[1] : L.cout, act2 = three ? L.gate[2] : L.act;
    FM_CHECK_ARG(!to.f32 && L.hid == 32 && stem2_supported(L.hid, cout2) && L.in_coff[0] == 0 && L.out_coff + L.cout <= to.c);
    FM_CHECK_ARG(!three || stem3_supported(cout2, L.cout));
    const char* w2 = net->weights + L.w2_off;
    const char* b2 = net->weights + L.b2_off;
    return launch_stem2(src, (const f16*)net->bufs[L.in[0]], ti.c, (f16*)net->bufs[L.out], to.c, L.out_coff,
                        (const f16*)(net->weights + L.w_off), (const float*)(net->weights + L.b_off), (const f16*)w2,
                        (const float*)b2, batch, ti.h, ti.w, to.h / 1, to.w / 1, cout2, L.gate[0], act2, s, three ? L.cout : 0,
                        three ? (const f16*)(w2 + (size_t)cout2 * 288 * 2) : nullptr,
                        three ? (const float*)(b2 + (size_t)cout2 * 4) : nullptr, L.act);
}

int launch_stempool_layer(const fm_layer& L, const StemSrc& src, const NetState* net, int batch, hipStream_t s) {
    const fm_tensor& ti = net->tensors[L.in[0]];
    const fm_tensor& to = net->tensors[L.out];
    FM_CHECK_ARG(!ti.f32 && !to.f32 && L.k == 7 && L.stride == 2 && L.pad == 3 && L.act == FM_ACT_RELU && L.in_coff[0] == 0 &&
                 (L.gate[0] == 0 || L.gate[0] == 1) && stempool_supported(L.cout, L.gate[0]) && L.out_coff + ((L.cout + 7) & ~7) <= to.c);
    FM_CHECK_ARG(L.b_off >= 0 && (size_t)L.w_off + (size_t)((L.cout + 31) & ~31) * 208 * 2 <= net->weight_bytes &&
                 (size_t)L.b_off + (size_t)((L.cout + 31) & ~31) * 4 <= net->weight_bytes);
    const int hc = (ti.h + 6 - 7) / 2 + 1, wc = (ti.w + 6 - 7) / 2 + 1;
    return launch_stempool_src(src, (const f16*)net->bufs[L.in[0]], ti.c, 0, (f16*)net->bufs[L.out], to.c, L.out_coff,
                               (const f16*)(net->weights + L.w_off), (const float*)(net->weights + L.b_off), batch, ti.h, ti.w,
                               hc, wc, to.h, to.w, L.gate[0], L.cout, s);
}

int fm_net_run_stem_from(fm_ctx* ctx, NetState* net, const StemSrc& src, int batch) {
    FM_CHECK_ARG(ctx && net && !net->layers.empty() && batch >= 1 && batch <= net->max_batch);
    const fm_layer& L = net->layers[0];
    FM_CHECK_ARG(L.op == FM_OP_STEMCONV || L.op == FM_OP_STEM2 || L.op == FM_OP_STEMPOOL);
    const fm_tensor& ti = net->tensors[L.in[0]];
    const fm_tensor& to = net->tensors[L.out];
    if (L.op == FM_OP_STEM2) {
        FM_CHECK_ARG(src.kind != 2);
        return launch_stem2_layer(L, src, net, batch, net->stream);
    }
    if (L.op == FM_OP_STEMPOOL) {
        FM_CHECK_ARG(src.kind == 2);
        return launch_stempool_layer(L, src, net, batch, net->stream);
    }
    return launch_stemconv_src(src, (const f16*)net->bufs[L.in[0]], ti.c, 0, (f16*)net->bufs[L.out], to.c, L.out_coff,
                               (const f16*)(net->weights + L.w_off), (const float*)(net->weights + L.b_off), batch, ti.h,
                               ti.w, to.h, to.w, L.k, L.stride, L.pad, L.cout, L.act, net->stream);
}

extern "C" int fm_net_run(fm_ctx* ctx, int which, int batch) {
    FM_CHECK_ARG(ctx && (which >= 0 && which < FM_NET_EXTRACTOR_B + FM_MAX_EXTRA_EXTRACTORS));
    NetState* net = net_slot(ctx, which);
    FM_CHECK_ARG(net != nullptr && batch >= 0 && batch <= net->max_batch);
    if (batch == 0) return 0;
    if (!net->use_graphs || !ctx->opt_use_graphs) return run_layers_eager(ctx, net, batch);
    const long key = (((long)batch << 32) | (unsigned)net->emb_offset) ^ ((long)net->first << 60);
    for (auto& g : net->graphs)
        if (g.first == key) {
            FM_HIP(hipGraphLaunch(g.second, net->stream));
            return 0;
        }
    int rc = run_layers_eager(ctx, net, batch);
    if (rc) return rc;
    FM_HIP(hipStreamSynchronize(net->stream));
    hipGraph_t graph = nullptr;
    hipGraphExec_t exec = nullptr;
    if (hipStreamBeginCapture(net->stream, hipStreamCaptureModeThreadLocal) != hipSuccess) {
        (void)hipGetLastError();
        net->use_graphs = false;
        return 0;
    }
    rc = run_layers_eager(ctx, net, batch);
    const hipError_t ec = hipStreamEndCapture(net->stream, &graph);
    if (rc != 0 || ec != hipSuccess || graph == nullptr ||
        hipGraphInstantiate(&exec, graph, nullptr, nullptr, 0) != hipSuccess) {
        (void)hipGetLastError();
        if (graph) (void)hipGraphDestroy(graph);
        net->use_graphs = false;
        return rc;
    }
    (void)hipGraphDestroy(graph);
    net->graphs.emplace_back(key, exec);
    return 0;
}

extern "C" int fm_net_tensor_write(fm_ctx* ctx, int which, int tensor, const void* host, size_t bytes) {
    FM_CHECK_ARG(ctx && (which >= 0 && which < FM_NET_EXTRACTOR_B + FM_MAX_EXTRA_EXTRACTORS) && host);
    NetState* net = net_slot(ctx, which);
    FM_CHECK_ARG(net && tensor >= 0 && tensor < (int)net->tensors.size());
    const fm_tensor& t = net->tensors[tensor];
    FM_CHECK_ARG(bytes <= (size_t)net->max_batch * t.h * t.w * t.c * elem_size(t));
    FM_HIP(hipStreamSynchronize(net->stream));
    FM_HIP(hipMemcpy(net->bufs[tensor], host, bytes, hipMemcpyHostToDevice));
    return 0;
}

extern "C" int fm_net_tensor_read(fm_ctx* ctx, int which, int tensor, void* host, size_t bytes) {
    FM_CHECK_ARG(ctx && (which >= 0 && which < FM_NET_EXTRACTOR_B + FM_MAX_EXTRA_EXTRACTORS) && host);
    NetState* net = net_slot(ctx, which);
    FM_CHECK_ARG(net && tensor >= 0 && tensor < (int)net->tensors.size());
    const fm_tensor& t = net->tensors[tensor];
    FM_CHECK_ARG(bytes <= (size_t)net->max_batch * t.h * t.w * t.c * elem_size(t));
    FM_HIP(hipStreamSynchronize(net->stream));
    FM_HIP(hipMemcpy(host, net->bufs[tensor], bytes, hipMemcpyDeviceToHost));
    return 0;
}

extern "C" int fm_net_read_embeddings(fm_ctx* ctx, int n, float* host) {
    FM_CHECK_ARG(ctx && n >= 0 && n <= ctx->emb_cap);
    if (n == 0) return 0;
    FM_CHECK_ARG(host);
    FM_HIP(hipStreamSynchronize(ctx->s_ext));
    FM_HIP(hipMemcpy(host, ctx->emb, sizeof(float) * (size_t)n * ctx->feat_dim, hipMemcpyDeviceToHost));
    ctx->emb_n = n;
    return 0;
}

extern "C" int fm_net_read_embeddings_mirror(fm_ctx* ctx, int n, float* host) {
    FM_CHECK_ARG(ctx && n >= 0 && n <= ctx->emb_cap);
    if (n == 0) return 0;
    FM_CHECK_ARG(host && ctx->emb_host);
    FM_HIP(hipStreamSynchronize(ctx->s_ext));
    memcpy(host, ctx->emb_host, sizeof(float) * (size_t)n * ctx->feat_dim);
    return 0;
}

static void layer_cost(const NetState* net, const fm_layer& L, int B, double* flops, double* bytes) {
    const fm_tensor& ti = net->tensors[L.in[0]];
    const fm_tensor& to = net->tensors[L.out];
    const double pin = (double)B * ti.h * ti.w, pout = (double)B * to.h * to.w;
    *flops = 0;
    *bytes = 0;
    switch (L.op) {
        case FM_OP_CONV:
        case FM_OP_CONVS:
        case FM_OP_CONVD:
            *flops = 2.0 * L.k * L.k * L.cin * L.cout * pout;
            *bytes = pin * L.cin * 2 + pout * L.cout * (to.f32 ? 4 : 2) + (double)L.k * L.k * L.cin * L.cout * 2 +
                     (L.res_mode != FM_RES_NONE ? pout * L.cout * 2 : 0);
            break;
        case FM_OP_DWCONV3:
            *flops = 2.0 * 9 * L.cin * pout;
            *bytes = (pin + pout) * L.cin * 2;
            break;
        case FM_OP_DWCONV:
            *flops = 2.0 * 9 * L.cin * pout;
            *bytes = (pin + pout) * L.cin * 2;
            break;
        case FM_OP_SEPCONV:
            *flops = 2.0 * (9 + L.cout) * L.cin * pout;
            *bytes = pin * L.cin * 2 + pout * L.cout * 2 + (double)(L.cin + 9) * L.cout * 2;
            break;
        case FM_OP_LITECONV:
            *flops = 2.0 * (L.cin + 9) * L.cout * pout * L.n_in;
            *bytes = ((pin + pout) * L.cin * 2 + (double)L.cin * L.cout * 2) * L.n_in;
            break;
        case FM_OP_LITECHAIN:
            *flops = 2.0 * (L.cin + 9) * L.cout * pout * 10;
            *bytes = (pin + 4 * pout) * L.cin * 2 + 10.0 * L.cin * L.cout * 2;
            break;
        case FM_OP_GATED_SUM: *bytes = (pin * L.n_in + pout) * L.cin * 2; break;
        case FM_OP_STEMCONV:
            *flops = 2.0 * L.k * L.k * 3 * L.cout * pout;
            *bytes = pin * 8 + pout * L.cout * 2;
            break;
        case FM_OP_PAIR11:
            *flops = 2.0 * L.cin * L.hid * pout + 2.0 * (L.hid + L.cin) * L.cout * pout;
            *bytes = (pin * L.cin + pout * L.hid + (double)L.cin * L.hid) * 2 + (pout * (L.hid + L.cin) + pout * L.cout + (double)(L.hid + L.cin) * L.cout) * 2;
            break;
        case FM_OP_STEM2:
            *flops = 2.0 * 9 * 3 * L.hid * pin + 2.0 * 9 * L.hid * (L.gate[1] > 0 ? L.gate[1] : L.cout) * pout +
                     (L.gate[1] > 0 ? 2.0 * L.gate[1] * L.cout * pout : 0.);
            *bytes = pin * 8 + pout * L.cout * 2 + 9.0 * L.hid * (L.gate[1] > 0 ? L.gate[1] : L.cout) * 2;
            break;
        case FM_OP_RESBLOCK:
            *flops = 2.0 * 10 * L.cin * L.hid * pout;
            *bytes = (pin + pout) * L.cin * 2 + 10.0 * L.cin * L.hid * 2;
            break;
        case FM_OP_SPP: *bytes = (pin + 3 * pout) * L.cin * 2; break;
        case FM_OP_GATE: *bytes = pin * L.cin * 2; break;
        case FM_OP_GATE_SUM: *bytes = (pin * L.n_in + pout) * L.cin * 2; break;
        case FM_OP_OSTAIL: {
            const double px = 128.0 * B, m = L.hid, c = L.k, lite = 10.0 * (m + 9) * m;
            *flops = 2.0 * px * (L.cin * m + lite + (m + L.cin) * c + c * m + lite + m * c + c * c) + 2.0 * c * L.cout * B;
            *bytes = pin * L.cin * 2 + ((double)L.stride) * 2 + (double)B * L.cout * 4;
            break;
// ... 107 lines not shown
```

### fastmot_amd/detector.py

```python
from collections import defaultdict
from pathlib import Path
import abc
import configparser

import numpy as np

from . import _lib, models
from .engine import HipNet, NET_DETECTOR
from .runtime import get_context
from .utils.setorder import IntSet

DET_DTYPE = _lib.DET_DTYPE


class DeviceFrame:

    def __init__(self, index):
        self.index = index




def bind_frame(ctx, frame, size, begin_step=False):
    if getattr(ctx, 'frame_size', None) != tuple(size):
        ctx.frame_configure(size[0], size[1], getattr(ctx, 'ring_size', 0))
    if not begin_step and getattr(ctx, 'in_step', False) and getattr(ctx, 'bound_frame', None) is frame:
        return
    if getattr(ctx, 'next_frame', None) is frame:
        ctx.frame_promote_next()
        ahead = getattr(ctx, 'ahead_frames', None) or []
        ctx.next_frame, ctx.ahead_frames = (ahead[0], ahead[1:]) if ahead else (None, [])
        ctx.bound_frame = frame
        return
    ctx.next_frame = None
    ctx.ahead_frames = []
    if isinstance(frame, DeviceFrame):
        ctx.frame_ring_select(frame.index)
    else:
        ctx.frame_upload(frame)
    ctx.bound_frame = frame


def prefetch_frame(ctx, frame, size):
    if getattr(ctx, 'frame_size', None) != tuple(size):
        ctx.frame_configure(size[0], size[1], getattr(ctx, 'ring_size', 0))
    if isinstance(frame, DeviceFrame):
        ctx.frame_ring_select_next(frame.index)
    else:
        ctx.frame_upload_next(frame)
    ctx.next_frame = frame
    ctx.ahead_frames = []


def prefetch_frames(ctx, frames, size):
    if getattr(ctx, 'frame_size', None) != tuple(size):
        ctx.frame_configure(size[0], size[1], getattr(ctx, 'ring_size', 0))
    for k, frame in enumerate(frames, 1):
        if isinstance(frame, DeviceFrame):
            ctx.frame_ring_select_ahead(k, frame.index)
        else:
            ctx.frame_upload_ahead(k, frame)
    ctx.next_frame, ctx.ahead_frames = frames[0], list(frames[1:])


def generate_tiles(tile_wh, tiling_grid, tile_overlap):
    tile_wh = np.array(tile_wh, float)
    grid = np.array(tiling_grid)
    step = (1 - tile_overlap) * tile_wh
    region = np.rint((grid - 1) * step + tile_wh).astype(int)
    tiles = []
    for row in range(grid[1]):
        for col in range(grid[0]):
            x, y = float(col * step[0]), float(row * step[1])
            tiles.append([round(x, 0), round(y, 0), round(x + tile_wh[0] - 1., 0), round(y + tile_wh[1] - 1., 0)])
    return np.array(tiles), tuple(region)


def tile_box_transforms(size, tile_wh, tiles, region):
    scale = np.array(size, float) / np.array(region, float)
    upscaled_sz = np.array(tile_wh, float) * scale
    offsets = [-(np.array(t[:2], float) * scale) for t in tiles]
    return upscaled_sz, offsets


def check_tiling(tiling_grid, max_batch=1, detector_lookahead=1):
    cols, rows = (int(v) for v in tiling_grid)
# ... 153 lines not shown
        box = np.array(dets.tlbr, float)
        bw, bh = box[:, 2] - box[:, 0] + 1, box[:, 3] - box[:, 1] + 1
        area = np.where((bw <= 0) | (bh <= 0), 0., bw * bh)
        iw = np.minimum(box[:, None, 2], box[None, :, 2]) - np.maximum(box[:, None, 0], box[None, :, 0]) + 1
        ih = np.minimum(box[:, None, 3], box[None, :, 3]) - np.maximum(box[:, None, 1], box[None, :, 1]) + 1
        with np.errstate(divide='ignore', invalid='ignore'):
            iom = np.where((iw <= 0) | (ih <= 0), 0., iw * ih / np.minimum(area[:, None], area[None, :]))
        linkable = (tile_ids[:, None] != tile_ids[None, :]) & (dets.label[:, None] == dets.label[None, :]) & (iom >= thresh)
        links = []
        for i in range(n):
            best = np.zeros(num_tile)
            mine = []
            for j in np.flatnonzero(linkable[i]):
                if iom[i, j] > best[tile_ids[j]]:
                    best[tile_ids[j]] = iom[i, j]
                    mine.append(int(j))
            links.append(mine)
        seen = np.zeros(n, bool)
        keep = IntSet(n)
        out = dets.copy().view(np.recarray)
        for i in range(n):
            if not links[i] or seen[i]:
                continue
            seen[i] = True
            todo, group = [i], []
            while todo:
                for j in links[todo.pop()]:
                    if not seen[j]:
                        seen[j] = True
                        group.append(j)
                        todo.append(j)
            for k in group:
                out.tlbr[i] = np.concatenate([np.minimum(out.tlbr[i, :2], out.tlbr[k, :2]),
                                              np.maximum(out.tlbr[i, 2:], out.tlbr[k, 2:])])
                out.conf[i] = max(out.conf[i], out.conf[k])
                keep.discard(k)
        out = out[np.array(list(keep), np.int64)]
        return out[np.argsort(out.label)].view(np.recarray)


class YOLODetector(Detector):
    def __init__(self, size,
                 class_ids,
                 model='YOLOv4',
                 conf_thresh=0.25,
                 nms_thresh=0.5,
                 max_area=800000,
                 min_aspect_ratio=1.2,
                 weights=None,
                 max_candidates=8192,
                 reuse_buffers=True,
                 max_batch=1,
                 tiling_grid=(1, 1),
                 tile_overlap=0.25,
                 merge_thresh=0.6):
        super().__init__(size)
        self.n_tiles = check_tiling(tiling_grid, max_batch)
        assert 0 <= tile_overlap <= 1
        assert 0 <= merge_thresh <= 1
        self.tiling_grid, self.tile_overlap, self.merge_thresh = tuple(int(v) for v in tiling_grid), tile_overlap, merge_thresh
        self.model = models.YOLO.get_model(model)
        assert 0 <= conf_thresh <= 1
        self.conf_thresh = conf_thresh
        assert 0 <= nms_thresh <= 1
        self.nms_thresh = nms_thresh
        assert max_area >= 0
        self.max_area = max_area
        assert min_aspect_ratio >= 0
        self.min_aspect_ratio = min_aspect_ratio

        self.label_mask = np.zeros(self.model.NUM_CLASSES, dtype=np.bool_)
        try:
            self.label_mask[tuple(class_ids),] = True
        except IndexError as err:
            raise ValueError('Unsupported class IDs') from err

        if not 1 <= max_batch <= _lib.FM_MAX_DET_BATCH:
            raise ValueError(f'max_batch must be 1..{_lib.FM_MAX_DET_BATCH}')
        self.max_batch = max_batch
        self.ctx = get_context()
        self._announced = []
        self.graph, self.heads = self.model.build_graph(weights)
        self.backend = HipNet(self.ctx, NET_DETECTOR, self.graph, max(max_batch, self.n_tiles), reuse_buffers=reuse_buffers)
        self.roi, self.upscaled_sz, self.bbox_offset = self._create_letterbox()
        self.tiles = self.tiling_region_sz = self.tile_bbox_offsets = None
        self.last_tile_detections = None
        if self.n_tiles > 1:
            tile_wh = self.model.INPUT_SHAPE[:0:-1]
            self.tiles, self.tiling_region_sz = generate_tiles(tile_wh, self.tiling_grid, self.tile_overlap)
            self.upscaled_sz, self.tile_bbox_offsets = tile_box_transforms(self.size, tile_wh, self.tiles,
                                                                           self.tiling_region_sz)
            self.bbox_offset = self.tile_bbox_offsets[0]
        self._configure(max_candidates)

    def _create_letterbox(self):
        src_size = np.array(self.size)
        dst_size = np.array(self.model.INPUT_SHAPE[:0:-1])
        if self.model.LETTERBOX:
            scale_factor = min(dst_size / src_size)
            scaled_size = np.rint(src_size * scale_factor).astype(int)
            img_offset = ((dst_size - scaled_size) / 2).astype(int)
            roi = (int(img_offset[0]), int(img_offset[1]), int(scaled_size[0]), int(scaled_size[1]))
            upscaled_sz = np.rint(dst_size / scale_factor).astype(int)
            bbox_offset = (upscaled_sz - src_size) / 2
        else:
            roi = (0, 0, int(dst_size[0]), int(dst_size[1]))
            upscaled_sz = src_size
            bbox_offset = np.zeros(2)
        return roi, upscaled_sz, bbox_offset

    def _configure(self, max_candidates):
        m = self.model
        cfg = _lib.YoloCfg()
        cfg.in_w, cfg.in_h = m.INPUT_SHAPE[2], m.INPUT_SHAPE[1]
        cfg.roi_x, cfg.roi_y, cfg.roi_w, cfg.roi_h = self.roi
        cfg.input_tensor = self.graph.input.tid
        cfg.n_heads = len(self.heads)
        for i, head in enumerate(self.heads):
            cfg.head_tensor[i] = head.tid
            cfg.grid_w[i] = m.INPUT_SHAPE[2] // m.LAYER_FACTORS[i]
            cfg.grid_h[i] = m.INPUT_SHAPE[1] // m.LAYER_FACTORS[i]
            cfg.n_anchors[i] = len(m.ANCHORS[i]) // 2
            for j, a in enumerate(m.ANCHORS[i]):
                cfg.anchors[i][j] = a
            cfg.scale_xy[i] = m.SCALES[i]
        cfg.num_classes = m.NUM_CLASSES
        cfg.new_coords = int(m.NEW_COORDS)
        for i, v in enumerate(self.label_mask):
            cfg.label_mask[i] = int(v)
        cfg.conf_thresh, cfg.nms_thresh = self.conf_thresh, self.nms_thresh
        cfg.max_area, cfg.min_aspect_ratio = self.max_area, self.min_aspect_ratio
        cfg.size[0], cfg.size[1] = float(self.upscaled_sz[0]), float(self.upscaled_sz[1])
        cfg.offset[0], cfg.offset[1] = float(self.bbox_offset[0]), float(self.bbox_offset[1])
        cfg.max_candidates = max_candidates
        self._cfg = cfg
        self.ctx.detect_configure(cfg)
        if self.n_tiles > 1:
            self.ctx.detect_configure_tiles(self.tiles[:, :2], self.tiling_region_sz, self.tile_bbox_offsets,
                                            self.merge_thresh)

    def detect_async(self, frame):
        if self._announced and self._announced[0] is frame and frame is not None:
            self._announced.pop(0)
            bind_frame(self.ctx, frame, self.size)
            return
        self._drop_announced()
        bind_frame(self.ctx, frame, self.size)
        self.ctx.detect_async()

    def _drop_announced(self):
        announced, self._announced = self._announced, []
        for _ in announced:
            self.ctx.detect_sync()

    def prefetch(self, frame):
        prefetch_frame(self.ctx, frame, self.size)
        self.ctx.detect_async_next()
        self._announced = [frame]

    def prefetch_batch(self, frames):
        frames = list(frames)
        if len(frames) == 1:
            return self.prefetch(frames[0])
        if self.n_tiles > 1:
            raise ValueError('a tiled detector takes one frame per network pass')
        if not 1 <= len(frames) <= self.max_batch:
# ... 88 lines not shown
```

### fastmot_amd/models/yolo.py

```python
import os
from pathlib import Path

import numpy as np

from . import scaled_yolov4
from .darknet import DarknetWeights, darknet_graph
from .graph import Graph, fold_bn, missing_weights


class YOLO:
    __registry = {}

    PLUGIN_PATH = Path(__file__).parents[1] / 'libfastmot_hip.so'
    ENGINE_PATH = None
    MODEL_PATH = None
    NUM_CLASSES = None
    LETTERBOX = False
    NEW_COORDS = False
    INPUT_SHAPE = None
    LAYER_FACTORS = None
    SCALES = None
    ANCHORS = None
    TOPOLOGY = 'yolov4'
    BUILTIN_CFG = None

    def __init_subclass__(cls, **kwargs):
        super().__init_subclass__(**kwargs)
        cls.__registry[cls.__name__] = cls

    @classmethod
    def get_model(cls, name):
        return cls.__registry[name]

    @classmethod
    def cfg_path(cls):
        return cls.MODEL_PATH.with_suffix('.cfg') if cls.MODEL_PATH is not None else None

    @classmethod
    def weight_file(cls):
        if cls.MODEL_PATH is None:
            return None
        base = Path(cls.MODEL_PATH)
        for cand in (base, base.with_suffix('.weights')):
            if cand.is_file():
                return cand
        return None

    @classmethod
    def build_graph(cls, weights=None):
        real = None
        onnx_model = None
        if weights is None:
            path = cls.weight_file()
            if path is None:
                weights = missing_weights(cls, seed=0)
            elif path.suffix == '.onnx':
                from .onnx_reader import OnnxDarknetWeights
                weights = real = OnnxDarknetWeights(path)
                onnx_model = weights.model
            else:
                weights = real = DarknetWeights(path)
        cfg = cls.cfg_path()
        text = None
        if cfg is not None and cfg.is_file():
            text, origin = cfg.read_text(), str(cfg)
        elif onnx_model is not None:
            from .onnx_reader import darknet_cfg_from_onnx
            text, origin = darknet_cfg_from_onnx(onnx_model, cls), f'the node list of {cls.MODEL_PATH}'
            shape = onnx_model.data_inputs[0][1]
            if tuple(shape[1:]) != tuple(cls.INPUT_SHAPE):
                raise ValueError(f'{cls.MODEL_PATH}: input {tuple(shape[1:])} != {cls.__name__}.INPUT_SHAPE {cls.INPUT_SHAPE}')
        if text is not None:
            g, heads, meta = darknet_graph(text, weights, in_hw=cls.INPUT_SHAPE[1:])
            if meta.get('classes') != cls.NUM_CLASSES or len(heads) != len(cls.LAYER_FACTORS) or \
                    meta.get('strides') != list(cls.LAYER_FACTORS) or meta.get('new_coords') != cls.NEW_COORDS:
                raise ValueError(f'{origin} does not describe {cls.__name__}: {meta}')
        elif cls.TOPOLOGY == 'yolov4':
            assert len(cls.LAYER_FACTORS) == len(cls.SCALES) == len(cls.ANCHORS)
            g, heads = yolov4_graph(cls, weights)
        elif cls.BUILTIN_CFG is not None:
            text = getattr(scaled_yolov4, cls.BUILTIN_CFG)(cls.INPUT_SHAPE[2], cls.INPUT_SHAPE[1], cls.NUM_CLASSES)
            g, heads, meta = darknet_graph(text, weights, in_hw=cls.INPUT_SHAPE[1:])
            assert meta['strides'] == list(cls.LAYER_FACTORS) and meta['new_coords'] == cls.NEW_COORDS
        else:
            raise NotImplementedError(f'{cls.__name__}: no built-in layer table; put the Darknet cfg at {cfg}')
        if real is not None and real.remaining() != 0:
            raise ValueError(f'{cls.weight_file()}: {real.remaining()} '
                             f'{"layers" if onnx_model is not None else "bytes"} left after loading {cls.__name__}')
        return g, heads


def yolov4_graph(model, weights):
    _, H, W = model.INPUT_SHAPE
    assert H % 32 == 0 and W % 32 == 0
    g = Graph(weights, (H, W), 3)
    n = [0]

    def name():
        n[0] += 1
        return f'conv{n[0]}'

    def conv(x, cout, k=1, stride=1, act='mish', **kw):
        return g.conv(name(), x, cout, k, stride, act, **kw)

    merge_siblings = os.environ.get('FASTMOT_CSP_MERGE', '1') != '0'
    if not merge_siblings:
        g.use_stem3 = False
# ... 48 lines not shown
    d4 = g.new(t4.h, t4.w, 512)
    n4 = five(u4, 256, dst=d4.slice(256, 256))

    u3 = g.new(t3.h, t3.w, 256)
    conv(n4, 128, 1, dst=u3.slice(128, 128), up=2, **lk)
    conv(t3, 128, 1, dst=u3.slice(0, 128), **lk)
    n3 = five(u3, 128)

    n_out = (5 + model.NUM_CLASSES) * (len(model.ANCHORS[0]) // 2)
    head_act = 'logistic' if model.NEW_COORDS else 'linear'
    heads = []
    x = conv(n3, 256, 3, **lk)
    heads.append(conv(x, n_out, 1, act=head_act, bn=False, f32_out=True))

    conv(n3, 256, 3, 2, dst=d4.slice(0, 256), **lk)
    m4 = five(d4, 256)
    x = conv(m4, 512, 3, **lk)
    heads.append(conv(x, n_out, 1, act=head_act, bn=False, f32_out=True))

    conv(m4, 512, 3, 2, dst=d5.slice(0, 512), **lk)
    m5 = five(d5, 512)
    x = conv(m5, 1024, 3, **lk)
    heads.append(conv(x, n_out, 1, act=head_act, bn=False, f32_out=True))
    g.outputs = heads
    return g, heads


class YOLOv4(YOLO):
    ENGINE_PATH = Path(__file__).parent / 'yolov4_crowdhuman.hipnet'
    MODEL_PATH = Path(__file__).parent / 'yolov4_crowdhuman.onnx'
    NUM_CLASSES = 2
    INPUT_SHAPE = (3, 512, 512)
    LAYER_FACTORS = [8, 16, 32]
    SCALES = [1.2, 1.1, 1.05]
    ANCHORS = [[11, 22, 24, 60, 37, 116],
               [54, 186, 69, 268, 89, 369],
               [126, 491, 194, 314, 278, 520]]


class YOLOv4_608(YOLO):
    ENGINE_PATH = Path(__file__).parent / 'yolov4_608.hipnet'
    MODEL_PATH = Path(__file__).parent / 'yolov4.onnx'
    NUM_CLASSES = 80
    INPUT_SHAPE = (3, 608, 608)
    LAYER_FACTORS = [8, 16, 32]
    SCALES = [1.2, 1.1, 1.05]
    ANCHORS = [[12, 16, 19, 36, 40, 28],
               [36, 75, 76, 55, 72, 146],
               [142, 110, 192, 243, 459, 401]]


_COCO_ANCHORS = [[12, 16, 19, 36, 40, 28], [36, 75, 76, 55, 72, 146], [142, 110, 192, 243, 459, 401]]


def _scaled(name, input_shape, factors, anchors, scales=2.0, builtin=None):
    return type(name, (YOLO,), dict(
        BUILTIN_CFG=builtin,
        ENGINE_PATH=Path(__file__).parent / f'{_file_name(name)}.hipnet',
        MODEL_PATH=Path(__file__).parent / f'{_file_name(name)}.onnx',
        NUM_CLASSES=1, LETTERBOX=True, NEW_COORDS=True, INPUT_SHAPE=input_shape, LAYER_FACTORS=factors,
        SCALES=[scales] * len(factors), ANCHORS=anchors, TOPOLOGY='darknet-cfg', __module__=__name__))


def _file_name(name):
    return {'YOLOv4CSP': 'yolov4-csp', 'YOLOv4xMish': 'yolov4x-mish', 'YOLOv4CSPSwish': 'yolov4-csp-swish',
            'YOLOv4CSPxSwish': 'yolov4-csp-x-swish', 'YOLOv4P5': 'yolov4-p5', 'YOLOv4P6': 'yolov4-p6'}[name]


YOLOv4CSP = _scaled('YOLOv4CSP', (3, 640, 640), [8, 16, 32], _COCO_ANCHORS, builtin='yolov4_csp_cfg')
YOLOv4xMish = _scaled('YOLOv4xMish', (3, 640, 640), [8, 16, 32], _COCO_ANCHORS)
YOLOv4CSPSwish = _scaled('YOLOv4CSPSwish', (3, 640, 640), [8, 16, 32], _COCO_ANCHORS)
YOLOv4CSPxSwish = _scaled('YOLOv4CSPxSwish', (3, 640, 640), [8, 16, 32], _COCO_ANCHORS)
YOLOv4P5 = _scaled('YOLOv4P5', (3, 896, 896), [8, 16, 32],
                   [[13, 17, 31, 25, 24, 51, 61, 45], [48, 102, 119, 96, 97, 189, 217, 184],
                    [171, 384, 324, 451, 616, 618, 800, 800]])
YOLOv4P6 = _scaled('YOLOv4P6', (3, 1280, 1280), [8, 16, 32, 64],
                   [[13, 17, 31, 25, 24, 51, 61, 45], [61, 45, 48, 102, 119, 96, 97, 189],
                    [97, 189, 217, 184, 171, 384, 324, 451], [324, 451, 545, 357, 616, 618, 1024, 1024]],
                   builtin='yolov4_p6_cfg')


class YOLOv4CSP_640(YOLOv4CSP):
    NUM_CLASSES = 80


class YOLOv4P6_1280(YOLOv4P6):
    NUM_CLASSES = 80


class YOLOv4Tiny(YOLO):
    ENGINE_PATH = Path(__file__).parent / 'yolov4-tiny.hipnet'
    MODEL_PATH = Path(__file__).parent / 'yolov4-tiny.onnx'
    NUM_CLASSES = 1
    INPUT_SHAPE = (3, 416, 416)
    LAYER_FACTORS = [32, 16]
    SCALES = [1.05, 1.05]
    ANCHORS = [[81, 82, 135, 169, 344, 319], [23, 27, 37, 58, 81, 82]]
    TOPOLOGY = 'darknet-cfg'


class YOLOv3(YOLO):
    ENGINE_PATH = Path(__file__).parent / 'yolov3.hipnet'
    MODEL_PATH = Path(__file__).parent / 'yolov3.onnx'
    NUM_CLASSES = 1
    INPUT_SHAPE = (3, 416, 416)
    LAYER_FACTORS = [32, 16, 8]
    SCALES = [1., 1.]
    ANCHORS = [[116, 90, 156, 198, 373, 326], [30, 61, 62, 45, 59, 119], [10, 13, 16, 30, 33, 23]]
    TOPOLOGY = 'darknet-cfg'


class YOLOv3SPP(YOLOv3):
    ENGINE_PATH = Path(__file__).parent / 'yolov3-spp.hipnet'
    MODEL_PATH = Path(__file__).parent / 'yolov3-spp.onnx'
    INPUT_SHAPE = (3, 608, 608)


class YOLOv3Tiny(YOLO):
    ENGINE_PATH = Path(__file__).parent / 'yolov3-tiny.hipnet'
    MODEL_PATH = Path(__file__).parent / 'yolov3-tiny.onnx'
    NUM_CLASSES = 1
    INPUT_SHAPE = (3, 416, 416)
    LAYER_FACTORS = [32, 16]
    SCALES = [1., 1.]
    ANCHORS = [[81, 82, 135, 169, 344, 319], [10, 14, 23, 27, 37, 58]]
    TOPOLOGY = 'darknet-cfg'
```

### include/fastmot_hip.h

```cpp
#ifndef FASTMOT_HIP_H
#define FASTMOT_HIP_H

#include <stddef.h>
#include <stdint.h>

#ifdef __cplusplus
extern "C" {
#endif

typedef struct fm_ctx fm_ctx;

int fm_ctx_create(int device, fm_ctx** out);
int fm_ctx_destroy(fm_ctx* ctx);
const char* fm_last_error(void);
int fm_device_count(void);
int fm_device_pci_bus_id(int device, char* buf, int buflen);
int fm_ctx_synchronize(fm_ctx* ctx);
int fm_ctx_bind_thread(fm_ctx* ctx);
int fm_ctx_set_option(fm_ctx* ctx, const char* key, int value);
int fm_trace_start(fm_ctx* ctx, int cap, int64_t* host_ns);
int fm_trace_read(fm_ctx* ctx, int cap, int32_t* tags, float* ms, int* n);
int fm_device_info(fm_ctx* ctx, char* buf, int buflen);

typedef struct fm_kf_params {
    double dt;
    double std_factor_acc, std_offset_acc;
    double std_factor_det[2], std_factor_klt[2];
    double min_std_det[2], min_std_klt[2];
    double init_pos_weight, init_vel_weight;
    double vel_coupling, vel_half_life;
} fm_kf_params;

int fm_kf_configure(fm_ctx* ctx, const fm_kf_params* p);
int fm_set_frame_rect(fm_ctx* ctx, const double tlbr[4]);

int fm_trk_create(fm_ctx* ctx, int n, const int32_t* slots, const double* det_tlbr);

int fm_trk_step(fm_ctx* ctx, int n, const int32_t* slots, const double* H,
                const double* klt_tlbr, const uint8_t* has_klt, const double* mult,
                double* tlbr_out, uint8_t* lost_out);

enum { FM_KF_WARP = 1, FM_KF_PREDICT = 2, FM_KF_UPDATE_KLT = 4 };
int fm_trk_step_ops(fm_ctx* ctx, int ops, int n, const int32_t* slots, const double* H,
                    const double* klt_tlbr, const uint8_t* has_klt, const double* mult,
                    double* tlbr_out, uint8_t* lost_out);

int fm_trk_update_det(fm_ctx* ctx, int n, const int32_t* slots, const double* det_tlbr,
                      double* tlbr_out, uint8_t* lost_out);

int fm_trk_get_state(fm_ctx* ctx, int n, const int32_t* slots, double* mean, double* cov);
int fm_trk_set_state(fm_ctx* ctx, int n, const int32_t* slots, const double* mean, const double* cov);
int fm_trk_copy_state(fm_ctx* ctx, int dst_slot, int src_slot);

int fm_feat_configure(fm_ctx* ctx, int dim);
int fm_emb_upload(fm_ctx* ctx, int n, const float* emb);
int fm_feat_update(fm_ctx* ctx, int n, const int32_t* slots, const int32_t* emb_rows);
int fm_feat_merge(fm_ctx* ctx, int dst_slot, int src_slot);
int fm_feat_reset(fm_ctx* ctx, int n, const int32_t* slots);
int fm_feat_get(fm_ctx* ctx, int slot, float* sum, float* avg, int32_t* count);
int fm_feat_read(fm_ctx* ctx, int n, const int32_t* slots, float* avg_out, int32_t* count_out);
int fm_feat_write(fm_ctx* ctx, int n, const int32_t* slots, const float* avg, const int32_t* count);

enum { FM_METRIC_EUCLIDEAN = 0, FM_METRIC_COSINE = 1 };

int fm_find_occluded(fm_ctx* ctx, int n, const double* tlbr, double thresh, uint8_t* out);

int fm_assoc_prepare(fm_ctx* ctx, int metric,
                     int nT, const int32_t* slots, const double* trk_tlbr, const int64_t* trk_label,
                     int nD, const double* det_tlbr, const int64_t* det_label,
                     const uint8_t* det_occluded, const uint8_t* trk_feat_f32);

int fm_assoc_get_pairwise(fm_ctx* ctx, double* feat, double* maha, double* iou);

enum {
    FM_STAGE_MATCHING = 0,
    FM_STAGE_IOU      = 1,
    FM_STAGE_REID     = 2
};

int fm_assoc_stage(fm_ctx* ctx, int stage, int solver,
                   int nr, const int32_t* rows, int nc, const int32_t* cols,
                   double motion_weight, double max_cost, double fill_val,
                   const int64_t* row_label_override,
                   int32_t* m_rows, int32_t* m_cols, uint8_t* match_gated, int* n_match,
                   double* cost_out);

int fm_assoc_prepare2(fm_ctx* ctx, int metric,
                      int nT, const int32_t* slots, const double* trk_tlbr, const int64_t* trk_label,
                      int nD, const double* det_tlbr, const int64_t* det_label,
                      const uint8_t* det_occluded, const uint8_t* trk_feat_f32, int after_extractor, int* host_cascade);

#define FM_CASCADE_HEADER 16
typedef struct fm_cascade_in {
    int32_t n_groups;
    int32_t n_unconf, n_hist;
    int32_t reserved;
    const int32_t* group_off;
    const int32_t* conf_rows;
    const uint8_t* conf_active;
    const int32_t* unconf_rows;
    const int32_t* hist_rows;
    const int64_t* hist_labels;
// ... 465 lines not shown
```

Measured before the change: 1006.

## Run detector front layers ahead on a side stream with double-buffered activations

Splits the detector network at layer K and runs the stem plus the first K high-resolution layers for the look-ahead frame on the upload (or extractor) stream, into double-buffered activation sets, while the previous detection's tail may still be running. The main detector stream then waits on an event and runs only the remaining layers. The post-processing flush is also deferred so it overlaps with this front work. This adds memory for two activation copies, separate graph keys per buffer set and extra syncs on reset paths, and it is skipped for models whose FRONT_LAYERS is 0.

```diff
diff --git a/fastmot_amd/_lib.py b/fastmot_amd/_lib.py
--- a/fastmot_amd/_lib.py
+++ b/fastmot_amd/_lib.py
@@ -223,6 +223,16 @@
 
     def set_option(self, key, value):
         check(self.lib.fm_ctx_set_option(self._ctx, key.encode(), C.c_int(int(value))))
+
+    def get_option(self, key):
+        v = C.c_int(0)
+        check(self.lib.fm_ctx_get_option(self._ctx, key.encode(), C.byref(v)))
+        return v.value
+
+    def front_info(self):
+        k, b, n = C.c_int(0), C.c_longlong(0), C.c_longlong(0)
+        check(self.lib.fm_net_front_info(self._ctx, C.byref(k), C.byref(b), C.byref(n)))
+        return k.value, b.value, n.value
 
     def trace_start(self, cap=20000):
         t0 = C.c_int64(0)
diff --git a/fastmot_amd/csrc/common.h b/fastmot_amd/csrc/common.h
--- a/fastmot_amd/csrc/common.h
+++ b/fastmot_amd/csrc/common.h
@@ -95,6 +95,10 @@
     int opt_fused_input = 1;
     int opt_net_timing = 0;
     int opt_nms_general = 0;
+    int opt_det_front_ahead = 1;
+    int opt_det_front_layers = -1;
+    int opt_det_front_stream = 0;
+    bool det_flush_deferred = false;
     int opt_lk_variant = 0;
     void* predict_worker = nullptr;
     hipStream_t s_main = nullptr;
@@ -276,6 +280,8 @@
 bool fm_host_is_pinned(const void* p, size_t bytes);
 void fm_frame_staging_free(fm_ctx* ctx);
 void fm_frame_dev_free(fm_ctx* ctx);
+hipStream_t fm_det_front_stream(fm_ctx* ctx);
+bool fm_det_defers_flush(fm_ctx* ctx);
 int fm_det_flush_post(fm_ctx* ctx);
 int fm_jpeg_to_bgr(const uint8_t* stage, uint8_t* bgr, const struct fm_jpeg_info* info, hipStream_t s);
 int fm_jpeg_layout(int width, int height, int ncomp, int hsamp0, int vsamp0, struct fm_jpeg_info* out);
diff --git a/fastmot_amd/csrc/ctx.hip b/fastmot_amd/csrc/ctx.hip
--- a/fastmot_amd/csrc/ctx.hip
+++ b/fastmot_amd/csrc/ctx.hip
@@ -1,3 +1,4 @@
+#include <algorithm>
 #include "common.h"
 void convd_set_cfg(int code);
 #include <sched.h>
@@ -17,7 +18,7 @@
 extern "C" const char* fm_last_error(void) { return g_err; }
 
 extern "C" int fm_ctx_set_option(fm_ctx* ctx, const char* key, int value) {
-    FM_CHECK_ARG(ctx && key && value >= 0);
+    FM_CHECK_ARG(ctx && key && (value >= 0 || (value == -1 && !strcmp(key, "det_front_layers"))));
     if (!strcmp(key, "zero_copy_tracks")) ctx->opt_zero_copy_tracks = value;
     else if (!strcmp(key, "host_lap_elems")) ctx->opt_host_lap_elems = value;
     else if (!strcmp(key, "use_graphs")) ctx->opt_use_graphs = value;
@@ -27,6 +28,11 @@
     }
     else if (!strcmp(key, "fused_input")) ctx->opt_fused_input = value != 0;
     else if (!strcmp(key, "net_timing")) ctx->opt_net_timing = value;
+    else if (!strcmp(key, "det_front_ahead") || !strcmp(key, "det_front_stream")) {
+        FM_CHECK_ARG(value <= (key[10] == 'a' ? 2 : 1));
+        (key[10] == 'a' ? ctx->opt_det_front_ahead : ctx->opt_det_front_stream) = value;
+    }
+    else if (!strcmp(key, "det_front_layers")) ctx->opt_det_front_layers = value;
     else if (!strcmp(key, "lk_variant")) {
 #ifndef FM_DIAG
         if (value != 0) {
@@ -38,6 +44,18 @@
     }
     else {
         fm_set_error("unknown option '%s'", key);
+        return FM_ERR_ARG;
+    }
+    return 0;
+}
+
+extern "C" int fm_ctx_get_option(fm_ctx* ctx, const char* key, int* value) {
+    FM_CHECK_ARG(ctx && key && value);
+    if (!strcmp(key, "det_front_ahead")) *value = ctx->opt_det_front_ahead;
+    else if (!strcmp(key, "det_front_layers")) *value = ctx->opt_det_front_layers;
+    else if (!strcmp(key, "det_front_stream")) *value = ctx->opt_det_front_stream;
+    else {
+        fm_set_error("option '%s' cannot be read", key);
         return FM_ERR_ARG;
     }
     return 0;
@@ -118,6 +136,8 @@
     if (const char* e = getenv("FASTMOT_HOST_LAP")) ctx->opt_host_lap_elems = atoi(e);
     if (const char* e = getenv("FASTMOT_GRAPHS")) ctx->opt_use_graphs = atoi(e);
     if (const char* e = getenv("FASTMOT_FUSED_INPUT")) ctx->opt_fused_input = atoi(e) != 0;
+    if (const char* e = getenv("FASTMOT_FRONT_AHEAD")) ctx->opt_det_front_ahead = std::min(std::max(atoi(e), 0), 2);
+    if (const char* e = getenv("FASTMOT_FRONT_STREAM")) ctx->opt_det_front_stream = atoi(e) == 1;
     int prio_lo = 0, prio_hi = 0;
     FM_HIP(hipDeviceGetStreamPriorityRange(&prio_lo, &prio_hi));
     const int prio_det = prio_lo, prio_ext = prio_hi;
diff --git a/fastmot_amd/csrc/detect.hip b/fastmot_amd/csrc/detect.hip
--- a/fastmot_amd/csrc/detect.hip
+++ b/fastmot_amd/csrc/detect.hip
@@ -41,6 +41,10 @@
     hipStream_t s_fallback = nullptr;
     hipEvent_t ev0[NSLOT] = {}, ev1[NSLOT] = {};
     bool timed[NSLOT] = {};
+    hipEvent_t evf0[NSLOT] = {}, evf1[NSLOT] = {};
+    bool timed_front[NSLOT] = {};
+    hipEvent_t ev_front[2] = {};
+    int set_slot[2] = {-1, -1};
     long n_passes = 0;
     int wr = 0, rd = 0, pending = 0, last = -1;
     uint8_t* label_mask = nullptr;
@@ -60,9 +64,11 @@
     for (int i = 0; i < DetState::NSLOT; ++i) {
         if (d->dets_host[i]) (void)hipHostFree(d->dets_host[i]);
         if (d->counters_host[i]) (void)hipHostFree(d->counters_host[i]);
-        for (hipEvent_t e : {d->ev_done[i], d->ev_dec[i], d->ev0[i], d->ev1[i]})
+        for (hipEvent_t e : {d->ev_done[i], d->ev_dec[i], d->ev0[i], d->ev1[i], d->evf0[i], d->evf1[i]})
             if (e) (void)hipEventDestroy(e);
     }
+    for (hipEvent_t e : d->ev_front)
+        if (e) (void)hipEventDestroy(e);
     delete d;
 }
 
@@ -710,6 +716,13 @@
     }
 }
 
+}
+bool fm_det_defers_flush(fm_ctx* ctx) {
+    return ctx->det && ctx->det_net && ctx->det_net->front_k > 0 && ctx->opt_det_front_ahead && ctx->opt_det_front_layers &&
+           ctx->opt_det_front_stream == 0;
+}
+namespace {
+
 int ensure_det(fm_ctx* ctx) {
     if (ctx->det) return 0;
     ctx->det = new DetState();
@@ -733,6 +746,7 @@
     d->last = -1;
     d->post_pending = -1;
     d->post_pending_n = 0;
+    d->set_slot[0] = d->set_slot[1] = -1;
     for (int i = 0; i < nslot; ++i) {
         if (d->cand[i]) continue;
         FM_HIP(hipMalloc(&d->cand[i], sizeof(float) * 8 * cap));
@@ -749,7 +763,11 @@
         FM_HIP(hipEventCreateWithFlags(&d->ev_dec[i], hipEventDisableTiming));
         FM_HIP(hipEventCreate(&d->ev0[i]));
         FM_HIP(hipEventCreate(&d->ev1[i]));
-    }
+        FM_HIP(hipEventCreate(&d->evf0[i]));
+        FM_HIP(hipEventCreate(&d->evf1[i]));
+    }
+    for (hipEvent_t& e : d->ev_front)
+        if (!e) FM_HIP(hipEventCreateWithFlags(&e, hipEventDisableTiming));
     if (!d->label_mask) FM_HIP(hipMalloc(&d->label_mask, 128));
     return 0;
 }
@@ -880,8 +898,13 @@
         return FM_ERR_STATE;
     }
     const int slot = d->rd;
-    int rc_f = flush_post(ctx, d);
-    if (rc_f) return rc_f;
+    bool later = d->post_pending >= 0 && (slot - d->post_pending + d->nslot) % d->nslot >= d->post_pending_n && fm_det_defers_flush(ctx);
+    if (later && hipEventQuery(d->ev_dec[d->post_pending]) == hipSuccess) later = false;
+    (void)hipGetLastError();
+    if (!later) {
+        int rc_f = flush_post(ctx, d);
+        if (rc_f) return rc_f;
+    }
     FM_HIP(hipEventSynchronize(d->ev_done[slot]));
     if (d->counters_host[slot][3] != 0 && !d->counters_host[slot][1]) {
         const int why = d->counters_host[slot][3];
@@ -985,6 +1008,7 @@
 }
 
 int fm_det_flush_post(fm_ctx* ctx) { return ctx->det ? flush_post(ctx, ctx->det) : 0; }
+hipStream_t fm_det_front_stream(fm_ctx* ctx) { return ctx->det_net ? ctx->det_net->front_stream : nullptr; }
 
 extern "C" int fm_detect_configure(fm_ctx* ctx, const fm_yolo_cfg* cfg) {
     FM_CHECK_ARG(ctx && cfg);
@@ -1002,6 +1026,8 @@
     DetState* d = ctx->det;
     FM_HIP(hipStreamSynchronize(ctx->s_det));
     FM_HIP(hipStreamSynchronize(ctx->s_up));
+    if (int rc_n = fm_net_sync(ctx->det_net)) return rc_n;
+    d->set_slot[0] = d->set_slot[1] = -1;
     d->post_pending = -1;
     d->post_pending_n = 0;
     d->rd = d->wr;
@@ -1030,6 +1056,8 @@
     }
     FM_HIP(hipStreamSynchronize(ctx->s_det));
     FM_HIP(hipStreamSynchronize(ctx->s_up));
+    if (int rc_n = fm_net_sync(ctx->det_net)) return rc_n;
+    d->set_slot[0] = d->set_slot[1] = -1;
     d->post_pending = -1;
     d->post_pending_n = 0;
     d->rd = d->wr;
@@ -1089,13 +1117,13 @@
     return enqueue_preprocess(ctx, ctx->det, ctx->det_net, det_source(ctx, ctx->det, &f, n), n);
 }
 
-static int detect_pass(fm_ctx* ctx, const uint8_t* const* frames, const hipEvent_t* uploads, int n);
+static int detect_pass(fm_ctx* ctx, const uint8_t* const* frames, const hipEvent_t* uploads, int n, bool look_ahead);
 
 extern "C" int fm_detect_async(fm_ctx* ctx) {
     FM_CHECK_ARG(ctx);
     const uint8_t* f = ctx->frame_cur;
     const hipEvent_t none = nullptr;
-    return detect_pass(ctx, &f, &none, 1);
+    return detect_pass(ctx, &f, &none, 1, false);
 }
 
 static int detect_ahead(fm_ctx* ctx, int n);
@@ -1130,10 +1158,10 @@
         }
         uploads[k - 1] = frames[k - 1] == fm_ahead_buf(ctx, k) ? fm_ahead_event(ctx, k) : nullptr;
     }
-    return detect_pass(ctx, frames, uploads, n);
-}
-
-static int detect_pass(fm_ctx* ctx, const uint8_t* const* frames, const hipEvent_t* uploads, int n) {
+    return detect_pass(ctx, frames, uploads, n, true);
+}
+
+static int detect_pass(fm_ctx* ctx, const uint8_t* const* frames, const hipEvent_t* uploads, int n, bool look_ahead) {
     FM_CHECK_ARG(ctx && ctx->det && ctx->det->configured && ctx->det_net);
     DetState* d = ctx->det;
     NetState* net = ctx->det_net;
@@ -1150,31 +1178,96 @@
     }
     FM_CHECK_ARG(n >= 1 && n <= FM_MAX_DET_BATCH && n <= net->max_batch);
     hipStream_t s = ctx->s_det;
+    int rc = 0;
+    const bool fused = ctx->opt_fused_input && fm_net_stem_fusable(net, c.input_tensor);
+    int K = 0;
+    if (ctx->det_flush_deferred && !(look_ahead && fused && n == 1 && !tiled)) {
+        ctx->det_flush_deferred = false;
+        if ((rc = flush_post(ctx, d))) return rc;
+    }
+    if (look_ahead && fused && n == 1 && !tiled && ctx->opt_det_front_ahead && ctx->opt_det_front_layers) {
+        bool busy = ctx->opt_det_front_ahead == 2;
+        if (!busy && d->pending > 0 && hipEventQuery(d->ev_dec[(d->wr + d->nslot - 1) % d->nslot]) != hipSuccess) {
+            (void)hipGetLastError();
+            busy = true;
+        }
+        if (busy && (rc = fm_net_front_prepare(ctx, net, ctx->opt_det_front_layers, &K))) return rc;
+    }
+    if (ctx->det_flush_deferred && !K) {
+        ctx->det_flush_deferred = false;
+        if ((rc = flush_post(ctx, d))) return rc;
+    }
+    const bool timing = ctx->opt_net_timing > 0 && d->n_passes++ % ctx->opt_net_timing == 0;
+    for (int i = 0; i < n; ++i) {
+        d->timed[(d->wr + i) % d->nslot] = timing && i == 0;
+        d->timed_front[(d->wr + i) % d->nslot] = timing && i == 0 && K > 0;
+    }
+    struct Restore {
+        NetState* net;
+        ~Restore() { net->first = net->last = 0; fm_net_select(net, nullptr, net->set); }
+    } restore{net};
     fm_trace_mark(ctx, s, 10);
-    for (int i = 0; i < n_frames; ++i)
-        if (uploads[i]) FM_HIP(hipStreamWaitEvent(s, uploads[i], 0));
-    int rc = acquire_slots(ctx, d, s, n);
-    if (rc) return rc;
-    fm_trace_mark(ctx, s, 14);
-    const StemSrc src = det_source(ctx, d, frames, n);
-    const bool fused = ctx->opt_fused_input && fm_net_stem_fusable(net, c.input_tensor);
-    const bool timing = ctx->opt_net_timing > 0 && d->n_passes++ % ctx->opt_net_timing == 0;
-    for (int i = 0; i < n; ++i) d->timed[(d->wr + i) % d->nslot] = timing && i == 0;
-    if (fused) {
+    if (K > 0) {
+        hipStream_t se = ctx->opt_det_front_stream == 1 ? ctx->s_ext : ctx->s_up;
+        const int set = net->set ^ 1;
+        if (net->front_stream && net->front_stream != se) FM_HIP(hipStreamSynchronize(net->front_stream));
+        net->front_stream = se;
+        ++net->front_passes;
+        if (uploads[0] && se != ctx->s_ext) FM_HIP(hipStreamWaitEvent(se, uploads[0], 0));
+        if ((rc = acquire_slots(ctx, d, se, 1))) return rc;
+        if (d->set_slot[set] >= 0 && hipEventQuery(d->ev_dec[d->set_slot[set]]) != hipSuccess) {
+            (void)hipGetLastError();
+            FM_HIP(hipStreamWaitEvent(se, d->ev_dec[d->set_slot[set]], 0));
+        }
+        const StemSrc src = det_source(ctx, d, frames, n);
+        fm_net_select(net, se, set);
+        if (timing) FM_HIP(hipEventRecord(d->evf0[d->wr], se));
+        fm_trace_mark(ctx, se, 11);
+        if ((rc = fm_net_run_stem_from(ctx, net, src, n))) return rc;
+        fm_trace_mark(ctx, se, 15);
+        if (K > 1) {
+            net->first = 1;
+            net->last = K;
+            if ((rc = fm_net_run_internal(ctx, FM_NET_DETECTOR, n))) return rc;
+        }
+        if (timing) FM_HIP(hipEventRecord(d->evf1[d->wr], se));
+        fm_trace_mark(ctx, se, 16);
+        FM_HIP(hipEventRecord(d->ev_front[set], se));
+        if (ctx->det_flush_deferred) {
+            ctx->det_flush_deferred = false;
+            if ((rc = flush_post(ctx, d))) return rc;
+        }
+        fm_net_select(net, nullptr, set);
+        FM_HIP(hipStreamWaitEvent(s, d->ev_front[set], 0));
+        fm_trace_mark(ctx, s, 14);
         if (timing) FM_HIP(hipEventRecord(d->ev0[d->wr], s));
-        fm_trace_mark(ctx, s, 11);
-        if ((rc = fm_net_run_stem_from(ctx, net, src, n))) return rc;
-        fm_trace_mark(ctx, s, 15);
-        net->first = 1;
-        rc = fm_net_run_internal(ctx, FM_NET_DETECTOR, n);
+        net->first = K;
+        net->last = 0;
+        if ((rc = fm_net_run_internal(ctx, FM_NET_DETECTOR, n))) return rc;
         net->first = 0;
-        if (rc) return rc;
     } else {
-        if ((rc = enqueue_preprocess(ctx, d, net, src, n))) return rc;
-        if (timing) FM_HIP(hipEventRecord(d->ev0[d->wr], s));
-        fm_trace_mark(ctx, s, 11);
-        if ((rc = fm_net_run_internal(ctx, FM_NET_DETECTOR, n))) return rc;
-    }
+        for (int i = 0; i < n_frames; ++i)
+            if (uploads[i]) FM_HIP(hipStreamWaitEvent(s, uploads[i], 0));
+        if ((rc = acquire_slots(ctx, d, s, n))) return rc;
+        fm_trace_mark(ctx, s, 14);
+        const StemSrc src = det_source(ctx, d, frames, n);
+        if (fused) {
+            if (timing) FM_HIP(hipEventRecord(d->ev0[d->wr], s));
+            fm_trace_mark(ctx, s, 11);
+            if ((rc = fm_net_run_stem_from(ctx, net, src, n))) return rc;
+            fm_trace_mark(ctx, s, 15);
+            net->first = 1;
+            rc = fm_net_run_internal(ctx, FM_NET_DETECTOR, n);
+            net->first = 0;
+            if (rc) return rc;
+        } else {
+            if ((rc = enqueue_preprocess(ctx, d, net, src, n))) return rc;
+            if (timing) FM_HIP(hipEventRecord(d->ev0[d->wr], s));
+            fm_trace_mark(ctx, s, 11);
+            if ((rc = fm_net_run_internal(ctx, FM_NET_DETECTOR, n))) return rc;
+        }
+    }
+    d->set_slot[net->set] = d->wr;
     if (timing) FM_HIP(hipEventRecord(d->ev1[d->wr], s));
     fm_trace_mark(ctx, s, 12);
     FilterArgs fa = filter_args(d, d->wr);
@@ -1224,6 +1317,8 @@
     hipStream_t s = ctx->s_det;
     FM_HIP(hipStreamSynchronize(s));
     FM_HIP(hipStreamSynchronize(ctx->s_up));
+    if (int rc_n = fm_net_sync(ctx->det_net)) return rc_n;
+    d->set_slot[0] = d->set_slot[1] = -1;
     d->post_pending = -1;
     d->post_pending_n = 0;
     d->rd = d->wr;
@@ -1276,6 +1371,7 @@
     if (rc_f) return rc_f;
     FM_HIP(hipStreamSynchronize(ctx->s_det));
     FM_HIP(hipStreamSynchronize(ctx->s_up));
+    if (int rc_n = fm_net_sync(ctx->det_net)) return rc_n;
     const int slot = (d->wr + d->nslot - 1) % d->nslot;
     int32_t cnt[4];
     FM_HIP(hipMemcpy(cnt, d->counters[slot], sizeof(cnt), hipMemcpyDeviceToHost));
@@ -1292,5 +1388,10 @@
     if (!ctx->det->timed[slot]) { *ms = -1.f; return 0; }
     FM_HIP(hipEventSynchronize(ctx->det->ev1[slot]));
     FM_HIP(hipEventElapsedTime(ms, ctx->det->ev0[slot], ctx->det->ev1[slot]));
-    return 0;
-}
+    if (ctx->det->timed_front[slot]) {
+        float front = 0.f;
+        FM_HIP(hipEventElapsedTime(&front, ctx->det->evf0[slot], ctx->det->evf1[slot]));
+        *ms += front;
+    }
+    return 0;
+}
diff --git a/fastmot_amd/csrc/frames.hip b/fastmot_amd/csrc/frames.hip
--- a/fastmot_amd/csrc/frames.hip
+++ b/fastmot_amd/csrc/frames.hip
@@ -65,6 +65,7 @@
 static int remap_idle(fm_ctx* ctx) {
     FM_HIP(hipStreamSynchronize(ctx->s_det));
     FM_HIP(hipStreamSynchronize(ctx->s_ext));
+    if (fm_det_front_stream(ctx)) FM_HIP(hipStreamSynchronize(fm_det_front_stream(ctx)));
     FM_HIP(hipStreamSynchronize(nullptr));
     return 0;
 }
@@ -256,6 +257,7 @@
     FM_HIP(hipStreamSynchronize(ctx->s_ext));
     FM_HIP(hipStreamSynchronize(ctx->s_flow));
     FM_HIP(hipStreamSynchronize(ctx->s_flow2));
+    if (fm_det_front_stream(ctx)) FM_HIP(hipStreamSynchronize(fm_det_front_stream(ctx)));
     int rc = enqueue(Target{0, ctx->frame_own, ctx->s_det, ctx->frame_pinned, nullptr, false});
     if (rc) return rc;
     FM_HIP(hipStreamSynchronize(ctx->s_det));
@@ -280,7 +282,9 @@
     fm_trace_mark(ctx, cs, 31);
     if (!ev) FM_HIP(hipEventCreateWithFlags(&ev, hipEventDisableTiming));
     FM_HIP(hipEventRecord(ev, cs));
-    if ((rc = fm_det_flush_post(ctx))) return rc;
+    if (k == 1 && fm_det_defers_flush(ctx))
+        ctx->det_flush_deferred = true;
+    else if ((rc = fm_det_flush_post(ctx))) return rc;
     fm_ahead_frame(ctx, k) = buf;
     return 0;
 }
diff --git a/fastmot_amd/csrc/net.h b/fastmot_amd/csrc/net.h
--- a/fastmot_amd/csrc/net.h
+++ b/fastmot_amd/csrc/net.h
@@ -43,12 +43,33 @@
     char* arena = nullptr;
     float* ws = nullptr;
     size_t ws_floats = 0;
-    std::vector<std::pair<long, hipGraphExec_t>> graphs;
+    struct GraphKey {
+        long batch_emb;
+        int first, last, set;
+        bool operator==(const GraphKey& o) const { return batch_emb == o.batch_emb && first == o.first && last == o.last && set == o.set; }
+    };
+    std::vector<std::pair<GraphKey, hipGraphExec_t>> graphs;
     bool use_graphs = true;
     int emb_offset = 0;
     int batch_offset = 0;
     int first = 0;
+    int last = 0;
+    int front_k = 0;
+    int front_req = 0;
+    int set = 0;
+    std::vector<void*> bufs_b;
+    std::vector<char> in_front;
+    std::vector<void*> front_owned;
+    float* ws_b = nullptr;
+    size_t front_bytes = 0;
+    hipStream_t home = nullptr;
+    hipStream_t front_stream = nullptr;
+    long front_passes = 0;
 };
+
+int fm_net_front_prepare(fm_ctx* ctx, NetState* net, int request, int* k);
+void fm_net_select(NetState* net, hipStream_t s, int set);
+int fm_net_sync(NetState* net);
 
 NetState* fm_net_get(fm_ctx* ctx, int which);
 int fm_net_run_internal(fm_ctx* ctx, int which, int batch);
diff --git a/fastmot_amd/csrc/net.hip b/fastmot_amd/csrc/net.hip
--- a/fastmot_amd/csrc/net.hip
+++ b/fastmot_amd/csrc/net.hip
@@ -62,27 +62,127 @@
 void fm_net_free(NetState* n) {
     if (!n) return;
     for (size_t i = 0; i < n->bufs.size(); ++i)
-        if (n->bufs[i] && n->tensors[i].offset < 0) (void)hipFree(n->bufs[i]);
+        if (n->bufs[i] && n->tensors[i].offset < 0 && !(i < n->in_front.size() && n->in_front[i])) (void)hipFree(n->bufs[i]);
+    for (void* p : n->front_owned) (void)hipFree(p);
     if (n->arena) (void)hipFree(n->arena);
     if (n->weights) (void)hipFree(n->weights);
     if (n->gates) (void)hipFree(n->gates);
     if (n->ws) (void)hipFree(n->ws);
+    if (n->ws_b) (void)hipFree(n->ws_b);
     for (auto& g : n->graphs) (void)hipGraphExecDestroy(g.second);
     delete n;
+}
+
+int fm_net_sync(NetState* net) {
+    if (!net) return 0;
+    if (net->front_stream) FM_HIP(hipStreamSynchronize(net->front_stream));
+    FM_HIP(hipStreamSynchronize(net->home ? net->home : net->stream));
+    return 0;
+}
+
+void fm_net_select(NetState* net, hipStream_t s, int set) {
+    net->stream = s ? s : net->home;
+    if (set != net->set && !net->bufs_b.empty()) {
+        net->bufs.swap(net->bufs_b);
+        net->set = set;
+    }
 }
 
 static NetState*& net_slot(fm_ctx* ctx, int which) {
     return which == FM_NET_DETECTOR ? ctx->det_net : which == FM_NET_EXTRACTOR ? ctx->ext_net
                                                     : ctx->ext_net_x[which - FM_NET_EXTRACTOR_B];
 }
+extern "C" int fm_net_front_info(fm_ctx* ctx, int* k, long long* bytes, long long* passes) {
+    FM_CHECK_ARG(ctx && k && bytes && passes);
+    const NetState* net = ctx->det_net;
+    *k = net ? net->front_k : 0;
+    *bytes = net ? (long long)net->front_bytes : 0;
+    *passes = net ? (long long)net->front_passes : 0;
+    return 0;
+}
 NetState* fm_net_get(fm_ctx* ctx, int which) { return net_slot(ctx, which); }
 int fm_net_run_internal(fm_ctx* ctx, int which, int batch) { return fm_net_run(ctx, which, batch); }
 
 void fm_net_drop_graphs(NetState* net) {
     if (!net) return;
-    (void)hipStreamSynchronize(net->stream);
+    (void)fm_net_sync(net);
     for (auto& g : net->graphs) (void)hipGraphExecDestroy(g.second);
     net->graphs.clear();
+}
+
+static size_t elem_size(const fm_tensor& t);
+
+constexpr size_t FRONT_BUDGET = (size_t)512 << 20;
+constexpr size_t FRONT_WS_FLOATS = (size_t)16 << 20;
+int fm_net_front_prepare(fm_ctx* ctx, NetState* net, int request, int* k) {
+    FM_CHECK_ARG(ctx && net && k && request != 0);
+    if (net->front_req == request) { *k = net->front_k; return 0; }
+    const int nl = (int)net->layers.size(), nt = (int)net->tensors.size();
+    const int input = net->layers[0].in[0];
+    int K = 0;
+    if (request > 0) K = std::min(request, nl - 1);
+    else
+        while (K < nl - 1 && (long)net->tensors[net->layers[K].out].h * net->tensors[net->layers[K].out].w >= 8192) ++K;
+    auto plain = [](int op) {
+        switch (op) {
+            case FM_OP_CONV: case FM_OP_CONVS: case FM_OP_CONVD: case FM_OP_DWCONV3: case FM_OP_DWCONV: case FM_OP_SEPCONV:
+            case FM_OP_STEMCONV: case FM_OP_STEM2: case FM_OP_STEMPOOL: case FM_OP_PAIR11: case FM_OP_SPP: case FM_OP_MAXPOOL:
+            case FM_OP_AVGPOOL: case FM_OP_UPSAMPLE2: case FM_OP_RESBLOCK: case FM_OP_ADD: case FM_OP_COPY: return true;
+            default: return false;
+        }
+    };
+    std::vector<char> want;
+    size_t bytes = 0;
+    for (;; --K) {
+        want.assign(nt, 0);
+        bytes = net->ws_b ? 0 : FRONT_WS_FLOATS * sizeof(float);
+        bool ok = true;
+        for (int i = 0; i < K && ok; ++i) {
+            const fm_layer& L = net->layers[i];
+            ok = plain(L.op);
+            want[L.out] = 1;
+            for (int j = 0; j < L.n_in; ++j) want[L.in[j]] = 1;
+            if (L.res_mode != FM_RES_NONE) want[L.res] = 1;
+        }
+        want[input] = 0;
+        for (int t = 0; t < nt; ++t)
+            if (want[t] && !(t < (int)net->in_front.size() && net->in_front[t])) {
+                const fm_tensor& T = net->tensors[t];
+                bytes += 2 * (((size_t)net->max_batch * T.h * T.w * T.c * elem_size(T) + 255) & ~(size_t)255);
+            }
+        if (K == 0 || (ok && net->front_bytes + bytes <= FRONT_BUDGET)) break;
+    }
+    net->front_req = request;
+    net->front_k = K;
+    *k = K;
+    if (K == 0) return 0;
+    fm_net_drop_graphs(net);
+    if (net->in_front.empty()) {
+        net->in_front.assign(nt, 0);
+        net->bufs_b = net->bufs;
+    }
+    if (!net->ws_b) {
+        FM_HIP(hipMalloc(&net->ws_b, FRONT_WS_FLOATS * sizeof(float)));
+        net->front_bytes += FRONT_WS_FLOATS * sizeof(float);
+    }
+    for (int t = 0; t < nt; ++t) {
+        if (!want[t] || net->in_front[t]) continue;
+        const fm_tensor& T = net->tensors[t];
+        const size_t b = (size_t)net->max_batch * T.h * T.w * T.c * elem_size(T);
+        void* two[2] = {nullptr, nullptr};
+        for (void*& p : two) {
+            FM_HIP(hipMalloc(&p, b));
+            net->front_owned.push_back(p);
+            FM_HIP(hipMemset(p, 0, b));
+        }
+        if (T.offset < 0) FM_HIP(hipFree(net->bufs[t]));
+        net->bufs[t] = two[0];
+        net->bufs_b[t] = two[1];
+        net->in_front[t] = 1;
+        net->front_bytes += 2 * ((b + 255) & ~(size_t)255);
+    }
+    FM_HIP(hipStreamSynchronize(nullptr));
+    return 0;
 }
 
 static size_t elem_size(const fm_tensor& t) { return t.f32 ? 4 : 2; }
@@ -91,7 +191,8 @@
     FM_CHECK_ARG(ctx && (which >= 0 && which < FM_NET_EXTRACTOR_B + FM_MAX_EXTRA_EXTRACTORS));
     NetState*& slot = net_slot(ctx, which);
     if (slot) {
-        FM_HIP(hipStreamSynchronize(slot->stream));
+        int rc = fm_net_sync(slot);
+        if (rc) return rc;
         fm_net_free(slot);
         slot = nullptr;
     }
@@ -110,6 +211,7 @@
     net->max_batch = max_batch;
     net->stream = which == FM_NET_DETECTOR ? ctx->s_det : which == FM_NET_EXTRACTOR ? ctx->s_ext
                                                         : ctx->s_ext_x[which - FM_NET_EXTRACTOR_B];
+    net->home = net->stream;
     net->tensors.assign(tensors, tensors + n_tensors);
     net->layers.assign(layers, layers + n_layers);
     if (arena_bytes) {
@@ -161,7 +263,9 @@
     const fm_tensor& ti = net->tensors[L.in[0]];
     const fm_tensor& to = net->tensors[L.out];
     hipStream_t s = net->stream;
-    float* ws = net->ws;
+    const bool away = s != net->home && net->ws_b;
+    float* ws = away ? net->ws_b : net->ws;
+    const size_t ws_floats = away ? FRONT_WS_FLOATS : net->ws_floats;
     const f16* in0 = (const f16*)net->bufs[L.in[0]];
     f16* out = (f16*)net->bufs[L.out];
     switch (L.op) {
@@ -199,7 +303,7 @@
             FM_CHECK_ARG(L.out_coff + p.cout_store <= to.c && L.in_coff[0] + L.cin <= ti.c);
             if (L.op == FM_OP_CONVS) return launch_conv_streamed(p, s);
             if (L.op == FM_OP_CONVD) return launch_convd(p, s);
-            return launch_conv(p, ws, net->ws_floats, s);
+            return launch_conv(p, ws, ws_floats, s);
         }
         case FM_OP_DWCONV3:
             return launch_dwconv3(in0, ti.c, L.in_coff[0], out, to.c, L.out_coff,
@@ -395,7 +499,8 @@
 }
 
 static int run_layers_eager(fm_ctx* ctx, NetState* net, int batch) {
-    for (size_t i = (size_t)net->first; i < net->layers.size(); ++i) {
+    const size_t end = net->last > 0 ? (size_t)net->last : net->layers.size();
+    for (size_t i = (size_t)net->first; i < end; ++i) {
         int rc = run_layer(ctx, net, net->layers[i], batch);
         if (rc) return rc;
     }
@@ -470,7 +575,7 @@
     FM_CHECK_ARG(net != nullptr && batch >= 0 && batch <= net->max_batch);
     if (batch == 0) return 0;
     if (!net->use_graphs || !ctx->opt_use_graphs) return run_layers_eager(ctx, net, batch);
-    const long key = (((long)batch << 32) | (unsigned)net->emb_offset) ^ ((long)net->first << 60);
+    const NetState::GraphKey key{((long)batch << 32) | (unsigned)net->emb_offset, net->first, net->last, net->set};
     for (auto& g : net->graphs)
         if (g.first == key) {
             FM_HIP(hipGraphLaunch(g.second, net->stream));
@@ -506,8 +611,11 @@
     FM_CHECK_ARG(net && tensor >= 0 && tensor < (int)net->tensors.size());
     const fm_tensor& t = net->tensors[tensor];
     FM_CHECK_ARG(bytes <= (size_t)net->max_batch * t.h * t.w * t.c * elem_size(t));
-    FM_HIP(hipStreamSynchronize(net->stream));
+    int rc = fm_net_sync(net);
+    if (rc) return rc;
     FM_HIP(hipMemcpy(net->bufs[tensor], host, bytes, hipMemcpyHostToDevice));
+    if (!net->bufs_b.empty() && net->bufs_b[tensor] != net->bufs[tensor])
+        FM_HIP(hipMemcpy(net->bufs_b[tensor], host, bytes, hipMemcpyHostToDevice));
     return 0;
 }
 
@@ -517,7 +625,8 @@
     FM_CHECK_ARG(net && tensor >= 0 && tensor < (int)net->tensors.size());
     const fm_tensor& t = net->tensors[tensor];
     FM_CHECK_ARG(bytes <= (size_t)net->max_batch * t.h * t.w * t.c * elem_size(t));
-    FM_HIP(hipStreamSynchronize(net->stream));
+    int rc = fm_net_sync(net);
+    if (rc) return rc;
     FM_HIP(hipMemcpy(host, net->bufs[tensor], bytes, hipMemcpyDeviceToHost));
     return 0;
 }
diff --git a/fastmot_amd/detector.py b/fastmot_amd/detector.py
--- a/fastmot_amd/detector.py
+++ b/fastmot_amd/detector.py
@@ -2,6 +2,7 @@
 from pathlib import Path
 import abc
 import configparser
+import os
 
 import numpy as np
 
@@ -321,6 +322,7 @@
         self._announced = []
         self.graph, self.heads = self.model.build_graph(weights)
         self.backend = HipNet(self.ctx, NET_DETECTOR, self.graph, max(max_batch, self.n_tiles), reuse_buffers=reuse_buffers)
+        self.ctx.set_option('det_front_layers', int(os.environ.get('FASTMOT_FRONT_LAYERS', self.model.FRONT_LAYERS)))
         self.roi, self.upscaled_sz, self.bbox_offset = self._create_letterbox()
         self.tiles = self.tiling_region_sz = self.tile_bbox_offsets = None
         self.last_tile_detections = None
diff --git a/fastmot_amd/models/yolo.py b/fastmot_amd/models/yolo.py
--- a/fastmot_amd/models/yolo.py
+++ b/fastmot_amd/models/yolo.py
@@ -23,6 +23,7 @@
     ANCHORS = None
     TOPOLOGY = 'yolov4'
     BUILTIN_CFG = None
+    FRONT_LAYERS = -1
 
     def __init_subclass__(cls, **kwargs):
         super().__init_subclass__(**kwargs)
@@ -237,10 +238,12 @@
 
 class YOLOv4CSP_640(YOLOv4CSP):
     NUM_CLASSES = 80
+    FRONT_LAYERS = 0
 
 
 class YOLOv4P6_1280(YOLOv4P6):
     NUM_CLASSES = 80
+    FRONT_LAYERS = 0
 
 
 class YOLOv4Tiny(YOLO):
diff --git a/include/fastmot_hip.h b/include/fastmot_hip.h
--- a/include/fastmot_hip.h
+++ b/include/fastmot_hip.h
@@ -18,6 +18,8 @@
 int fm_ctx_synchronize(fm_ctx* ctx);
 int fm_ctx_bind_thread(fm_ctx* ctx);
 int fm_ctx_set_option(fm_ctx* ctx, const char* key, int value);
+int fm_ctx_get_option(fm_ctx* ctx, const char* key, int* value);
+int fm_net_front_info(fm_ctx* ctx, int* k, long long* bytes, long long* passes);
 int fm_trace_start(fm_ctx* ctx, int cap, int64_t* host_ns);
 int fm_trace_read(fm_ctx* ctx, int cap, int32_t* tags, float* ms, int* n);
 int fm_device_info(fm_ctx* ctx, char* buf, int buflen);
```

Measured after the change: 1076 (median of 6 runs). 7.0% higher.
